# SinOncology/BreakID

Hardware: AMD Instinct MI355X
Metric: M reads/s clustered+split-scanned (higher is better)
Workload: dtype int32/u8 (+f64 sd replay)

## Files before the change

breakid_amd/csrc/api.hip:

```cpp
#include <algorithm>
#include <cmath>
#include <limits>
#include <cstring>
#include <numeric>

#include "bk_common.h"
#include "prims.h"
#include "stream.h"
#include "join.h"
#include "cluster.h"
#include "bp.h"
#include "normal.h"
#include "genotype.h"
#include "clip.h"
#include "junction.h"
#include "evidence.h"
#include "unique.h"
#include "consensus.h"
#include "jfit.h"
#include "locsim.h"
#include "coverage.h"
#include "frame.h"
#include "exclude.h"
#include "ahc.h"
#include "lanes.h"
#include "bgzf_gpu.h"

namespace
{
thread_local std::string g_init_error;

uint64_t fnv64(const std::string &s)
{
  uint64_t h = 0xCBF29CE484222325ull;
  for (unsigned char c : s)
  {
    h ^= c;
    h *= 0x100000001B3ull;
  }
  return h;
}
std::string chrom_id_to_name(int tid)
{
  if (tid == 23) return "chrY";
  if (tid == 22) return "chrX";
  if (tid >= 0 && tid < 22) return "chr" + std::to_string(tid + 1);
  return "";
}

struct StageTimer
{
  std::string name;
  hipEvent_t a = nullptr, b = nullptr;
  uint64_t bytes = 0;
  uint64_t touched = 0;
};
}

struct bk_ctx
{
  int device = 0;
  hipStream_t st = nullptr;
  bool own_stream = true;
  std::string err;
  int nt = 0;
  std::vector<uint32_t> tlen;
  std::vector<std::string> tname;
  std::vector<int32_t> hdr_id_host;
  DevBuf d_tprefix, d_nhash, d_nid, d_own, d_hdr;
  NameTableDev names{};

  bk_soa rec{};
  DevBuf col[13];
  DevBuf d_side;
  DevBuf xcol[13];
  bool have_records = false;
  bool streamed = false;

  DevBuf d_counters, d_sd, d_cand, d_split_raw, d_split, d_sa_list;
  StreamCounters hc{};
  SdState hsd{};
  bool stream_done = false, splits_sorted = false;
  int mapq_min = 20;
  int stream_mapq = -1;
  uint64_t cand_cap = 0, split_cap = 0, sa_cap = 0;
  uint64_t rec_base = 0;
  std::vector<uint64_t> route_counts;
  JoinBufs jb2;
  const Cand *ext_cand = nullptr;
  const bk_split *ext_split = nullptr;
  bk_cluster *ext_clusters = nullptr;
  std::vector<uint8_t> own_groups;
  const Cand *cand_ptr() const { return ext_cand ? ext_cand : d_cand.get<Cand>(); }
  const bk_split *split_raw_ptr() const { return ext_split ? ext_split : d_split_raw.get<bk_split>(); }
  bk_cluster *clusters_ptr() const { return ext_clusters ? ext_clusters : d_clusters.get<bk_cluster>(); }
  SdBufs sdb;
  double mean = 0, sd = 0;
  bool stats_done = false;

  JoinBufs jb;
  JoinResult jr;
  std::vector<uint32_t> gkey_host, glex_host, lex_to_num;
  std::vector<uint64_t> gstart_host;
  DevBuf d_glex, d_lex_to_num;

  ClusterStage stage;
  bool clustered = false;

  BpBufs bb;
  DevBuf d_clusters;
  uint64_t n_clusters = 0;

  bool joined = false, bp_done = false, shard = false;
  double join_w = 0;
  NormalBufs nb;
  std::vector<struct bk_normal_support> f_normal;
  RefBufs rb;
  std::vector<struct bk_ref_support> f_ref;
  ClipBufs cb;
  std::vector<struct bk_clip_support> f_clip;
  DevBuf d_bd_tid, d_bd_pos, d_bd_out, d_bd_samp;
  std::vector<uint32_t> f_base_depth;
  ClipReadBufs crb;
  std::vector<uint32_t> f_cr_counts;
  std::vector<struct bk_clip_read> f_cr_rows;
  std::vector<uint64_t> f_cr_off;
  JunctionBufs jnb;
  std::vector<struct bk_junction> f_junction;
  bool summary_map = false;
  EvidenceBufs evb;
  std::vector<struct bk_evidence> f_evidence;
  std::vector<uint64_t> f_ev_off;
  UniqueBufs uqb;
  std::vector<struct bk_unique_support> f_unique;
  std::vector<uint64_t> f_uq_first;
  ConsensusBufs cnb;
  std::vector<struct bk_consensus> f_cons;
  std::vector<uint8_t> f_cons_bases;
  std::vector<uint32_t> f_cons_depth;
  JfitBufs jfb;
  std::vector<struct bk_junction_fit> f_jfit;
  LocsimBufs lsb;
  std::vector<struct bk_locus_sim> f_locsim;
  CovBufs cvb;
  std::vector<struct bk_window_cov> f_wincov;
  FrameBufs frb;
  std::vector<struct bk_frame_call> f_frame;

  prims::RadixBufs dbg_radix;
  DevBuf dbg_in, dbg_out, dbg_vals;

  std::vector<bk_pair> f_pairs[3];
  std::vector<uint64_t> f_off[3];
  std::vector<bk_split> f_splits;
  std::vector<bk_cluster> f_clusters;
  std::vector<int32_t> f_gkeys;
  std::vector<bk_group_stat> f_gstats;

  bool timing = false;
  std::vector<StageTimer> timers;
  Timing tout;

  void tick(const char *name, uint64_t bytes, bool begin, uint64_t touched = 0)
  {
    if (!timing) return;
    if (begin)
    {
      StageTimer t;
      t.name = name;
      t.bytes = bytes;
      t.touched = touched;
      HIP_CHECK(hipEventCreate(&t.a));
      HIP_CHECK(hipEventCreate(&t.b));
      HIP_CHECK(hipEventRecord(t.a, st));
      timers.push_back(t);
    }
    else
      HIP_CHECK(hipEventRecord(timers.back().b, st));
  }
};

static RecView rec_view(const bk_ctx *ctx)
{
  RecView r;
  r.n = ctx->rec.n;
  r.tid = ctx->rec.tid; r.pos = ctx->rec.pos; r.flag = ctx->rec.flag; r.mapq = ctx->rec.mapq;
  r.cigar_off = ctx->rec.cigar_off; r.cigar = ctx->rec.cigar;
  r.isize = ctx->rec.isize; r.aux_off = ctx->rec.aux_off;
  return r;
}

namespace
{
struct Scope
{
  bk_ctx *c;
  Scope(bk_ctx *c, const char *name, uint64_t bytes = 0, uint64_t touched = 0) : c(c) { c->tick(name, bytes, true, touched); }
  ~Scope()
  {
    try
    {
      c->tick("", 0, false);
    }
    catch (...)
    {
    }
  }
};

template <class F> int guarded(bk_ctx *ctx, F &&f)
{
  if (!ctx) return BK_ERR_ARG;
  try
  {
    HIP_CHECK(hipSetDevice(ctx->device));
    f();
    return BK_OK;
  }
  catch (const bk_error &e)
  {
    ctx->err = e.msg;
    return e.code;
  }
  catch (const std::exception &e)
  {
    ctx->err = e.what();
    return BK_ERR_HIP;
  }
}

template <class T> void rows_to_host(bk_ctx *ctx, const T *d_rows, uint64_t n, std::vector<T> &out)
{
  out.resize(n);
  if (n) HIP_CHECK(hipMemcpyAsync(out.data(), d_rows, n * sizeof(T), hipMemcpyDeviceToHost, ctx->st));
  HIP_CHECK(hipStreamSynchronize(ctx->st));
}

void build_name_tables(bk_ctx *c)
{
  const int nt = c->nt;
  std::map<std::string, int> ids;
  for (int i = 0; i < nt; ++i)
    if (!ids.count(c->tname[i])) ids[c->tname[i]] = i;
  if (!ids.count("")) ids[""] = nt;
  if (!ids.count("*")) ids["*"] = nt + 1;
  for (int t = 0; t < 24; ++t)
  {
    std::string s = chrom_id_to_name(t);
    if (!ids.count(s)) ids[s] = nt + 2 + t;
  }
  uint32_t cap = 64;
  while (cap < ids.size() * 4) cap <<= 1;
  std::vector<uint64_t> hash(cap, 0);
  std::vector<int32_t> idv(cap, -1);
  for (auto &kv : ids)
  {
    uint64_t h = fnv64(kv.first);
    if (h == 0) h = 1;
    uint32_t slot = (uint32_t) h & (cap - 1);
    while (hash[slot] != 0 && hash[slot] != h) slot = (slot + 1) & (cap - 1);
    if (hash[slot] == 0)
    {
      hash[slot] = h;
      idv[slot] = kv.second;
    }
  }
  std::vector<int32_t> own(std::max(nt, 1));
  for (int t = 0; t < nt; ++t) own[t] = ids[chrom_id_to_name(t)];
  c->hdr_id_host.assign(nt + 1, 0);
  c->hdr_id_host[0] = ids["*"];
  for (int t = 0; t < nt; ++t) c->hdr_id_host[t + 1] = ids[c->tname[t]];
  std::vector<uint32_t> prefix(nt + 1, 0);
  for (int t = 0; t < nt; ++t) prefix[t + 1] = prefix[t] + c->tlen[t];
  HIP_CHECK(hipMemcpy(c->d_nhash.as<uint64_t>(cap), hash.data(), cap * 8, hipMemcpyHostToDevice));
  HIP_CHECK(hipMemcpy(c->d_nid.as<int32_t>(cap), idv.data(), cap * 4, hipMemcpyHostToDevice));
  HIP_CHECK(hipMemcpy(c->d_own.as<int32_t>(own.size()), own.data(), own.size() * 4, hipMemcpyHostToDevice));
  HIP_CHECK(hipMemcpy(c->d_hdr.as<int32_t>(nt + 1), c->hdr_id_host.data(), (nt + 1) * 4, hipMemcpyHostToDevice));
  HIP_CHECK(hipMemcpy(c->d_tprefix.as<uint32_t>(nt + 1), prefix.data(), (nt + 1) * 4, hipMemcpyHostToDevice));
  c->names.hash = c->d_nhash.get<uint64_t>();
  c->names.id = c->d_nid.get<int32_t>();
  c->names.mask = cap - 1;
  c->names.own_id = c->d_own.get<int32_t>();
  c->names.n_targets = nt;
  c->names.empty_id = ids[""];
}

std::string rname(const bk_ctx *c, int tid) { return tid < 0 ? "*" : c->tname[tid]; }

StreamArgs stream_args(bk_ctx *c, uint64_t n)
{
  StreamArgs a{};
  a.n = n;
  a.q_begin = 0;
  a.rec_base = c->rec_base;
  a.tid = c->rec.tid; a.pos = c->rec.pos; a.mtid = c->rec.mtid; a.mpos = c->rec.mpos; a.isize = c->rec.isize;
  a.flag = c->rec.flag; a.mapq = c->rec.mapq; a.qhash = c->rec.qhash; a.qcheck = c->rec.qcheck;
  static const bool no_side = getenv("BREAKID_NO_SIDE") != nullptr;
  a.side = no_side && c->rec.qhash ? nullptr : c->rec.side;
  a.cigar_off = c->rec.cigar_off; a.cigar = c->rec.cigar; a.aux_off = c->rec.aux_off; a.aux = c->rec.aux;
  a.mapq_min = c->mapq_min;
  a.names = c->names;
  a.counters = c->d_counters.get<StreamCounters>();
  a.sd = c->d_sd.get<SdState>();
  a.cand = c->d_cand.get<Cand>();
  a.cand_cap = c->cand_cap;
  a.split = c->d_split_raw.get<bk_split>();
  a.split_cap = c->split_cap;
  a.sa_list = c->d_sa_list.get<uint32_t>();
  a.sa_cap = c->sa_cap;
  return a;
}
void stream_prepare(bk_ctx *c, uint64_t n_expected)
{
  c->streamed = true;
  c->cand_cap = std::max<uint64_t>(c->cand_cap, std::max<uint64_t>(1u << 16, n_expected / 8 + 1024));
  c->split_cap = std::max<uint64_t>(c->split_cap, std::max<uint64_t>(1u << 14, n_expected / 32 + 1024));
  c->sa_cap = std::max<uint64_t>(c->sa_cap, std::max<uint64_t>(1u << 14, n_expected / 16 + 1024));
  StreamCounters *dc = c->d_counters.as<StreamCounters>(1);
  SdState *dsd = c->d_sd.as<SdState>(1);
  HIP_CHECK(hipMemsetAsync(dc, 0, sizeof(StreamCounters), c->st));
  HIP_CHECK(hipMemsetAsync(dsd, 0, sizeof(SdState), c->st));
  (void) c->d_cand.as<Cand>(c->cand_cap);
  (void) c->d_split_raw.as<bk_split>(c->split_cap);
  (void) c->d_sa_list.as<uint32_t>(c->sa_cap);
}
bool stream_finish(bk_ctx *c)
{
  HIP_CHECK(hipMemcpyAsync(&c->hc, c->d_counters.get<StreamCounters>(), sizeof(StreamCounters), hipMemcpyDeviceToHost, c->st));
  HIP_CHECK(hipMemcpyAsync(&c->hsd, c->d_sd.get<SdState>(), sizeof(SdState), hipMemcpyDeviceToHost, c->st));
  HIP_CHECK(hipStreamSynchronize(c->st));
  if (c->hc.n_cand > c->cand_cap || c->hc.n_sa > c->sa_cap)
  {
    c->cand_cap = std::max<uint64_t>(c->cand_cap, c->hc.n_cand + 1024);
    c->sa_cap = std::max<uint64_t>(c->sa_cap, c->hc.n_sa + 1024);
    return false;
  }
  return true;
}
void stream_rare_path(bk_ctx *c)
{
  const uint64_t n = c->rec.n;
  if (c->timing && !c->timers.empty())
  {
    c->timers.back().bytes += 32ull * c->hc.n_cand + 4ull * c->hc.n_sa;
    c->timers.back().touched = 23ull * n + 4ull * c->rec.n_cigar_words + (c->rec.qcheck ? 60ull : 56ull) * c->hc.n_cand + 4ull * c->hc.n_sa;
  }
  if (c->hc.unsorted) throw bk_error(BK_ERR_UNSORTED, "records are not coordinate sorted (the reference requires an indexed, sorted BAM)");
  if (c->hc.n_sa > c->split_cap)
  {
    c->split_cap = c->hc.n_sa + 1024;
    (void) c->d_split_raw.as<bk_split>(c->split_cap);
  }
  StreamArgs a = stream_args(c, n);
  {
    Scope s(c, "k_split_records", c->rec.n_aux_bytes + 4ull * c->hc.n_sa);
    launch_split_records(a, c->hc.n_sa, c->st);
  }
  HIP_CHECK(hipMemcpyAsync(&c->hc, c->d_counters.get<StreamCounters>(), sizeof(StreamCounters), hipMemcpyDeviceToHost, c->st));
  HIP_CHECK(hipStreamSynchronize(c->st));
  if (c->timing && !c->timers.empty())
  {
    c->timers.back().bytes += 48ull * c->hc.n_split;
    c->timers.back().touched = c->timers.back().bytes + 40ull * c->hc.n_sa + 32ull * c->hc.n_split;
  }
  c->stream_done = true;
  c->stream_mapq = c->mapq_min;
  c->splits_sorted = false;
  c->stats_done = false;
}

void run_stream(bk_ctx *c)
{
  if (!c->have_records) throw bk_error(BK_ERR_ARG, "no records uploaded");
  const uint64_t n = c->rec.n;
  for (int attempt = 0; attempt < 3; ++attempt)
  {
    stream_prepare(c, n);
    {
      Scope s(c, "k_stream", 39ull * n + 4ull * c->rec.n_cigar_words);
      launch_stream(stream_args(c, n), c->st);
    }
    if (stream_finish(c)) break;
    if (c->timing && !c->timers.empty()) c->timers.pop_back();
    if (attempt == 2) throw bk_error(BK_ERR_LIMIT, "stream pass: output capacity");
  }
  stream_rare_path(c);
}

void ensure_splits_sorted(bk_ctx *c)
{
  if (c->splits_sorted) return;
  Scope s(c, "split_sort");
  bk_split *sorted = c->d_split.as<bk_split>(c->hc.n_split + 1);
  int bits = 0;
  if (!c->ext_split && c->rec_base == 0)
  {
    bits = 1;
    while (bits < 32 && (1ull << bits) < c->rec.n) ++bits;
  }
  sort_splits(const_cast<bk_split *>(c->split_raw_ptr()), c->hc.n_split, sorted, c->bb, c->st, bits);
  c->splits_sorted = true;
}
}

extern "C" {

void bk_prepare_process()
{
  static std::once_flag once;
  std::call_once(once, [] {
    const char *q = getenv("GPU_MAX_HW_QUEUES");
    stage_set_hw_queues(q ? atoi(q) : 4);
  });
}

int bk_init(int device, const uint32_t *target_len, const char *const *target_name, int n_targets, bk_ctx **out)
{
  {
    bk_prepare_process();
  }
  if (!out || n_targets < 0 || (n_targets && (!target_len || !target_name)))
  {
    g_init_error = "bk_init: bad arguments";
    return BK_ERR_ARG;
  }
  *out = nullptr;
  int ndev = 0;
  if (hipGetDeviceCount(&ndev) != hipSuccess || ndev <= 0 || device < 0 || device >= ndev)
  {
    g_init_error = "bk_init: no HIP device " + std::to_string(device) + " (this library has no CPU path)";
    return BK_ERR_NO_DEVICE;
  }
  hipDeviceProp_t prop;
  if (hipGetDeviceProperties(&prop, device) != hipSuccess || std::string(prop.gcnArchName).rfind("gfx950", 0) != 0)
  {
    g_init_error = std::string("bk_init: device is not gfx950 (") + prop.gcnArchName + "); kernels are built for MI355X only";
    return BK_ERR_NO_DEVICE;
  }
  bk_ctx *c = new bk_ctx();
  c->device = device;
  c->nt = n_targets;
  for (int i = 0; i < n_targets; ++i)
  {
    c->tlen.push_back(target_len[i]);
    c->tname.push_back(target_name[i]);
  }
  int rc = guarded(c, [&] {
    HIP_CHECK(hipStreamCreate(&c->st));
    build_name_tables(c);
  });
  if (rc != BK_OK)
  {
    g_init_error = c->err;
    delete c;
    return rc;
  }
  *out = c;
  return BK_OK;
}

void bk_free(bk_ctx *ctx)
{
  if (!ctx) return;
  (void) hipSetDevice(ctx->device);
  (void) hipStreamSynchronize(ctx->st);
  for (auto &t : ctx->timers)
  {
    if (t.a) (void) hipEventDestroy(t.a);
    if (t.b) (void) hipEventDestroy(t.b);
  }
  if (ctx->own_stream && ctx->st) (void) hipStreamDestroy(ctx->st);
  delete ctx;
}

const char *bk_last_error(const bk_ctx *ctx) { return ctx ? ctx->err.c_str() : g_init_error.c_str(); }

int bk_set_stream(bk_ctx *ctx, void *hip_stream)
{
  return guarded(ctx, [&] {
    if (ctx->own_stream && ctx->st) HIP_CHECK(hipStreamDestroy(ctx->st));
    ctx->st = (hipStream_t) hip_stream;
    ctx->own_stream = false;
  });
}
int bk_get_stream(bk_ctx *ctx, void **hip_stream)
{
  return guarded(ctx, [&] {
    if (!hip_stream) throw bk_error(BK_ERR_ARG, "bk_get_stream: null output");
    *hip_stream = (void *) ctx->st;
  });
}
int bk_sync(bk_ctx *ctx)
{
  return guarded(ctx, [&] { HIP_CHECK(hipStreamSynchronize(ctx->st)); });
}

int bk_records(bk_ctx *ctx, bk_soa *cols)
{
  return guarded(ctx, [&] {
    if (!cols) throw bk_error(BK_ERR_ARG, "bk_records: null output");
    if (!ctx->have_records) throw bk_error(BK_ERR_ARG, "bk_records: the context holds no record table");
    HIP_CHECK(hipStreamSynchronize(ctx->st));
    *cols = ctx->rec;
  });
}

int bk_upload_records(bk_ctx *ctx, const bk_soa *s, int mem_space)
{
  return guarded(ctx, [&] {
    if (!s) throw bk_error(BK_ERR_ARG, "bk_upload_records: null table");
    if (s->n > 0xFFFFFFF0ull) throw bk_error(BK_ERR_LIMIT, "more than 2^32 records in one context (shard across GPUs)");
    ctx->stream_done = ctx->stats_done = ctx->clustered = false;
    ctx->joined = ctx->bp_done = ctx->shard = false;
    ctx->ext_cand = nullptr;
    ctx->ext_split = nullptr;
    ctx->ext_clusters = nullptr;
    ctx->own_groups.clear();
    ctx->rec_base = 0;
    ctx->streamed = false;
    if (mem_space == BK_MEM_DEVICE)
    {
      hipPointerAttribute_t at;
      if (s->n && s->tid && hipPointerGetAttributes(&at, s->tid) == hipSuccess && at.type == hipMemoryTypeDevice && at.device != ctx->device)
        throw bk_error(BK_ERR_ARG, "bk_upload_records: BK_MEM_DEVICE table lives on device " + std::to_string(at.device) + ", context on device " +
                                       std::to_string(ctx->device));
      (void) hipGetLastError();
      for (const void *p : {(const void *) s->tid, (const void *) s->pos, (const void *) s->isize, (const void *) s->flag, (const void *) s->mapq, (const void *) s->cigar_off,
                            (const void *) s->aux_off})
        if (s->n && ((uintptr_t) p & 15u)) throw bk_error(BK_ERR_ARG, "bk_upload_records: BK_MEM_DEVICE columns must be 16-byte aligned");
      if (s->n && s->side && ((uintptr_t) s->side & 15u)) throw bk_error(BK_ERR_ARG, "bk_upload_records: BK_MEM_DEVICE side rows must be 16-byte aligned");
      ctx->rec = *s;
    }
    else
    {
      const uint64_t n = s->n;
      const void *src[13] = {s->tid, s->pos, s->mtid, s->mpos, s->isize, s->flag, s->mapq, s->qhash, s->cigar_off, s->cigar, s->aux_off, s->aux, s->qcheck};
      const size_t bytes[13] = {n * 4, n * 4, n * 4, n * 4, n * 4, n * 2, n, n * 8, (n + 1) * 4, s->n_cigar_words * 4, (n + 1) * 4, s->n_aux_bytes,
                                s->qcheck ? n * 4 : 0};
      void *dst[13];
      for (int k = 0; k < 13; ++k)
      {
        dst[k] = ctx->col[k].ensure(bytes[k] + 16);
        if (bytes[k]) HIP_CHECK(hipMemcpyAsync(dst[k], src[k], bytes[k], hipMemcpyHostToDevice, ctx->st));
      }
      HIP_CHECK(hipStreamSynchronize(ctx->st));
      bk_soa d = *s;
      d.tid = (const int32_t *) dst[0]; d.pos = (const int32_t *) dst[1]; d.mtid = (const int32_t *) dst[2]; d.mpos = (const int32_t *) dst[3];
      d.isize = (const int32_t *) dst[4]; d.flag = (const uint16_t *) dst[5]; d.mapq = (const uint8_t *) dst[6]; d.qhash = (const uint64_t *) dst[7];
      d.cigar_off = (const uint32_t *) dst[8]; d.cigar = (const uint32_t *) dst[9]; d.aux_off = (const uint32_t *) dst[10]; d.aux = (const uint8_t *) dst[11];
      d.qcheck = s->qcheck ? (const uint32_t *) dst[12] : nullptr;
      bk_side *side = ctx->d_side.as<bk_side>(n + 1);
      launch_make_side(d.qhash, d.mtid, d.mpos, d.qcheck, n, side, ctx->st);
      d.side = side;
      ctx->rec = d;
    }
    ctx->have_records = true;
  });
}

int bk_exclude_regions(bk_ctx *ctx, const bk_regions *r, uint64_t *n_removed)
{
  return guarded(ctx, [&] {
    if (!ctx->have_records || ctx->streamed || ctx->shard)
      throw bk_error(BK_ERR_ARG, "bk_exclude_regions: call it after bk_upload_records and before the stream pass (bk_isize_stats, bk_shard_begin, "
                                 "or a context of bk_bam_decode_device_ctx)");
    if (!r || (r->n && (!r->tid || !r->beg || !r->end))) throw bk_error(BK_ERR_ARG, "bk_exclude_regions: null interval list");
    const bk_soa &s = ctx->rec;
    if (s.n && (!s.tid || !s.pos || !s.mtid || !s.mpos || !s.isize || !s.flag || !s.mapq || !s.qhash || !s.cigar_off || !s.aux_off))
      throw bk_error(BK_ERR_ARG, "bk_exclude_regions: the table lacks a column");
    std::vector<std::vector<std::pair<int32_t, int32_t>>> by(ctx->nt);
    for (uint64_t k = 0; k < r->n; ++k)
    {
      const int32_t t = r->tid[k], b = r->beg[k], e = r->end[k];
      if (t < 0 || t >= ctx->nt || b < 0 || e <= b)
        throw bk_error(BK_ERR_ARG, "bk_exclude_regions: interval " + std::to_string(k) + " (tid " + std::to_string(t) + ", [" + std::to_string(b) + ", " +
                                       std::to_string(e) + ")): needs 0 <= tid < n_targets, 0 <= beg < end");
      by[t].emplace_back(b, e);
    }
    std::vector<uint32_t> off(ctx->nt + 1, 0);
    std::vector<int32_t> beg, end;
    for (int t = 0; t < ctx->nt; ++t)
    {
      auto &v = by[t];
      std::sort(v.begin(), v.end());
      for (auto &iv : v)
        if (beg.size() > off[t] && iv.first <= end.back())
          end.back() = std::max(end.back(), iv.second);
        else
        {
          beg.push_back(iv.first);
          end.push_back(iv.second);
        }
      off[t + 1] = (uint32_t) beg.size();
    }
    const bool owned = s.tid && s.tid == ctx->col[0].get<int32_t>();
    if (beg.empty() && owned)
    {
      if (n_removed) *n_removed = 0;
      return;
    }
    DevBuf d_off, d_beg, d_end;
    ExclRegions rg;
    rg.n_targets = ctx->nt;
    rg.off = d_off.as<uint32_t>(off.size());
    rg.beg = d_beg.as<int32_t>(beg.size() + 1);
    rg.end = d_end.as<int32_t>(end.size() + 1);
    HIP_CHECK(hipMemcpyAsync((void *) rg.off, off.data(), off.size() * 4, hipMemcpyHostToDevice, ctx->st));
    if (!beg.empty())
    {
      HIP_CHECK(hipMemcpyAsync((void *) rg.beg, beg.data(), beg.size() * 4, hipMemcpyHostToDevice, ctx->st));
      HIP_CHECK(hipMemcpyAsync((void *) rg.end, end.data(), end.size() * 4, hipMemcpyHostToDevice, ctx->st));
    }
    bk_soa out;
    const uint64_t n_before = s.n;
    exclude_compact(s, rg, ctx->xcol, out, ctx->st, [&](const char *name, uint64_t bytes, bool begin) { ctx->tick(name ? name : "", bytes, begin, bytes); });
    for (int k = 0; k < 13; ++k)
    {
      std::swap(ctx->col[k], ctx->xcol[k]);
      ctx->xcol[k].release();
    }
    {
      Scope sc(ctx, "make_side", (out.qcheck ? 56ull : 52ull) * out.n, (out.qcheck ? 56ull : 52ull) * out.n);
      bk_side *side = ctx->d_side.as<bk_side>(out.n + 1);
      launch_make_side(out.qhash, out.mtid, out.mpos, out.qcheck, out.n, side, ctx->st);
      out.side = side;
    }
    HIP_CHECK(hipStreamSynchronize(ctx->st));
    ctx->rec = out;
    if (n_removed) *n_removed = n_before - out.n;
  });
}

int bk_isize_stats(bk_ctx *ctx, double *mean, double *sd)
{
  return guarded(ctx, [&] {
    if (!ctx->stream_done) run_stream(ctx);
    if (!ctx->stats_done)
    {
      const double n = (double) ctx->hc.isize_n;
      const double m = (double) (long long) ctx->hc.isize_sum / n;
      ctx->mean = m;
      if (ctx->hc.isize_n == 0)
        ctx->sd = std::nan("");
      else
      {
        double sum_d = ctx->hsd.sumsq - 2.0 * m * (double) ctx->hc.isize_sum + n * m * m;
        if (!(sum_d > 0)) sum_d = 0;
        double da = (double) ctx->hsd.vmax - m, dmax = da * da + m * m;
        double bound = 2.0 * sum_d + 2.0 * n + 2.0 * dmax + 4.0;
        int k = std::ilogb(bound) + 1;
        double thr = k >= 51 ? 1.0e300 : std::ldexp(1.0, k - 53);
        {
          Scope s(ctx, "isize_sd", 0, 6ull * ctx->rec.n);
          launch_sd(ctx->rec.flag, ctx->rec.isize, ctx->rec.n, m, thr, ctx->d_sd.get<SdState>(), ctx->sdb, ctx->st);
        }
        HIP_CHECK(hipMemcpyAsync(&ctx->hsd, ctx->d_sd.get<SdState>(), sizeof(SdState), hipMemcpyDeviceToHost, ctx->st));
        HIP_CHECK(hipStreamSynchronize(ctx->st));
        ctx->sd = std::sqrt((double) ctx->hsd.t_final / n);
      }
      ctx->stats_done = true;
    }
    if (mean) *mean = ctx->mean;
    if (sd) *sd = ctx->sd;
  });
}

static void finish_groups(bk_ctx *ctx, const std::vector<uint32_t> *all_keys)
{
  const uint32_t ng = ctx->jr.n_groups;
  ctx->gkey_host.assign(ng, 0);
  ctx->gstart_host.assign(ng + 1, 0);
  if (ng)
  {
    HIP_CHECK(hipMemcpyAsync(ctx->gkey_host.data(), ctx->jr.gkey, ng * 4, hipMemcpyDeviceToHost, ctx->st));
    HIP_CHECK(hipMemcpyAsync(ctx->gstart_host.data(), ctx->jr.gstart, (ng + 1) * 8, hipMemcpyDeviceToHost, ctx->st));
    HIP_CHECK(hipStreamSynchronize(ctx->st));
  }
  auto key_name = [&](uint32_t k) {
    int t1 = (int) (k / (uint32_t) (ctx->nt + 1)) - 1, t2 = (int) (k % (uint32_t) (ctx->nt + 1)) - 1;
    return rname(ctx, t1) + "_" + rname(ctx, t2);
  };
  std::vector<std::string> keys(ng);
  for (uint32_t g = 0; g < ng; ++g) keys[g] = key_name(ctx->gkey_host[g]);
  ctx->lex_to_num.resize(ng);
  std::iota(ctx->lex_to_num.begin(), ctx->lex_to_num.end(), 0u);
  std::sort(ctx->lex_to_num.begin(), ctx->lex_to_num.end(), [&](uint32_t a, uint32_t b) { return keys[a] < keys[b]; });
  ctx->glex_host.assign(ng, 0);
  if (!all_keys)
    for (uint32_t l = 0; l < ng; ++l) ctx->glex_host[ctx->lex_to_num[l]] = l;
  else
  {
    std::vector<std::string> names;
    names.reserve(all_keys->size());
    for (uint32_t k : *all_keys) names.push_back(key_name(k));
    std::sort(names.begin(), names.end());
    names.erase(std::unique(names.begin(), names.end()), names.end());
    for (uint32_t g = 0; g < ng; ++g)
    {
      auto it = std::lower_bound(names.begin(), names.end(), keys[g]);
      if (it == names.end() || *it != keys[g]) throw bk_error(BK_ERR_ARG, "bk_shard_group_pairs: a local group is missing from the global key list");
      ctx->glex_host[g] = (uint32_t) (it - names.begin());
    }
  }
  uint32_t *dg = ctx->d_glex.as<uint32_t>((uint64_t) ng + 1), *dl = ctx->d_lex_to_num.as<uint32_t>((uint64_t) ng + 1);
  if (ng) HIP_CHECK(hipMemcpyAsync(dg, ctx->glex_host.data(), ng * 4, hipMemcpyHostToDevice, ctx->st));
  if (ng) HIP_CHECK(hipMemcpyAsync(dl, ctx->lex_to_num.data(), ng * 4, hipMemcpyHostToDevice, ctx->st));
  join_assign_ids(ctx->jr, dg, ctx->st);
}

int bk_discordant_pairs(bk_ctx *ctx, int mapq_min, double w, uint64_t *n_pairs, uint32_t *n_groups)
{
  return guarded(ctx, [&] {
    if (!ctx->stream_done || mapq_min != ctx->stream_mapq)
    {
      ctx->mapq_min = mapq_min;
      run_stream(ctx);
    }
    {
      Scope s(ctx, "mate_join");
      ctx->jb.rec_bits = -1;
      if (!ctx->ext_cand && ctx->rec_base == 0)
      {
        int bits = 1;
        while (bits < 32 && (1ull << bits) < ctx->rec.n) ++bits;
        ctx->jb.rec_bits = bits;
      }
      join_candidates(ctx->cand_ptr(), ctx->hc.n_cand, w, ctx->d_tprefix.get<uint32_t>(), ctx->nt, ctx->jb, ctx->st, ctx->jr);
    }
    finish_groups(ctx, nullptr);
    ctx->clustered = false;
    ctx->joined = true;
    ctx->bp_done = false;
    ctx->join_w = w;
    if (n_pairs) *n_pairs = ctx->jr.n_pairs;
    if (n_groups) *n_groups = ctx->jr.n_groups;
  });
}

int bk_mask_and_cluster(bk_ctx *ctx, double w, int fast, uint64_t *n_clustered)
{
  return guarded(ctx, [&] {
    const StageInput in{ctx->device, ctx->st, ctx->jr, ctx->gstart_host, ctx->own_groups,
                        [&](const char *name, const std::function<void()> &body) { Scope s(ctx, name); body(); }};
    ctx->summary_map = false;
    ctx->stage.run(in, w, fast);
    ctx->clustered = true;
    if (n_clustered) *n_clustered = ctx->stage.list.n;
  });
}

int bk_split_evidence(bk_ctx *ctx, uint64_t *n_tuples)
{
  return guarded(ctx, [&] {
    if (!ctx->stream_done) run_stream(ctx);
    ensure_splits_sorted(ctx);
    if (n_tuples) *n_tuples = ctx->hc.n_split;
  });
}

int bk_cluster_summary(bk_ctx *ctx, double w, uint64_t *n_clusters)
{
  return guarded(ctx, [&] {
    if (!ctx->clustered) throw bk_error(BK_ERR_ARG, "bk_cluster_summary: call bk_mask_and_cluster first");
    ctx->bp_done = false;
    if (ctx->stage.list.ng != ctx->jr.n_groups) throw bk_error(BK_ERR_HIP, "bk_cluster_summary: the clustered list and the join disagree on the groups (internal error)");
    Scope s(ctx, "cluster_summary");
    ctx->n_clusters = cluster_summary(ctx->jr.pairs, ctx->stage.list.idx.get<uint32_t>(), ctx->stage.list.gof.get<uint32_t>(), ctx->stage.d_cluster.get<uint32_t>(), ctx->stage.list.n,
                                      ctx->stage.list.ng, ctx->jr.gkey, ctx->d_glex.get<uint32_t>(), ctx->d_lex_to_num.get<uint32_t>(), ctx->nt, w, ctx->d_clusters, ctx->bb, ctx->st);
    ctx->summary_map = true;
    if (n_clusters) *n_clusters = ctx->n_clusters;
  });
}

int bk_split_breakpoints(bk_ctx *ctx, double w, uint64_t *n_valid)
{
  return guarded(ctx, [&] {
    ensure_splits_sorted(ctx);
    RecView r;
    r.n = ctx->rec.n;
    r.tid = ctx->rec.tid; r.pos = ctx->rec.pos; r.flag = ctx->rec.flag; r.mapq = ctx->rec.mapq;
    r.cigar_off = ctx->rec.cigar_off; r.cigar = ctx->rec.cigar;
    {
      Scope s(ctx, "split_breakpoints");
      split_breakpoints(r, ctx->d_split.get<bk_split>(), ctx->hc.n_split, ctx->clusters_ptr(), ctx->n_clusters, w, (int) ctx->hc.max_span,
                        ctx->d_hdr.get<int32_t>(), ctx->bb, ctx->st);
    }
    ctx->bp_done = true;
    if (n_valid) *n_valid = count_valid_clusters(ctx->clusters_ptr(), ctx->n_clusters, ctx->bb, ctx->st);
  });
}

static TupleTable tuple_table(const bk_ctx *ctx)
{
  return TupleTable{ctx->d_split.get<bk_split>(), ctx->hc.n_split, (int) ctx->hc.max_span, ctx->d_hdr.get<int32_t>(), ctx->names.own_id, ctx->nt, ctx->names.empty_id};
}
static JunctionPairs junction_pairs(const bk_ctx *ctx)
{
  JunctionPairs jp{};
  if (ctx->n_clusters)
  {
    jp.pairs = ctx->jr.pairs;
    jp.idx = ctx->stage.list.idx.get<uint32_t>();
    jp.gof = ctx->stage.list.gof.get<uint32_t>();
    jp.cl = ctx->stage.d_cluster.get<uint32_t>();
    jp.n = ctx->stage.list.n;
    jp.ng = ctx->stage.list.ng;
    jp.slotbase = ctx->bb.slotbase.get<uint32_t>();
    jp.keep = ctx->bb.keep.get<uint32_t>();
    jp.off = ctx->bb.off.get<uint32_t>();
  }
  return jp;
}
static void require_same_reference(const std::string &who, const char *role_a, const bk_ctx *a, const char *role_b, const bk_ctx *b)
{
  if (b->device != a->device)
    throw bk_error(BK_ERR_ARG, who + ": " + role_a + " (device " + std::to_string(a->device) + ") and " + role_b + " (device " + std::to_string(b->device) +
                                   ") contexts are on different devices");
  if (b != a && (b->nt != a->nt || b->tname != a->tname || b->tlen != a->tlen))
    throw bk_error(BK_ERR_ARG, who + ": " + role_a + " and " + role_b + " reference lists differ (names or lengths)");
}

int bk_normal_support(bk_ctx *tumor, bk_ctx *normal, double w, const struct bk_normal_support **out, uint64_t *count)
{
  if (!normal) return guarded(tumor, [&] { throw bk_error(BK_ERR_ARG, "bk_normal_support: null normal context"); });
  return guarded(tumor, [&] {
    if (!out || !count) throw bk_error(BK_ERR_ARG, "bk_normal_support: null output");
    if (tumor->shard || normal->shard) throw bk_error(BK_ERR_ARG, "bk_normal_support: sharded contexts (bk_shard_*) are not supported");
    if (!tumor->bp_done) throw bk_error(BK_ERR_ARG, "bk_normal_support: call bk_split_breakpoints on the tumour context first");
    if (!normal->stats_done || !normal->joined || !normal->splits_sorted)
      throw bk_error(BK_ERR_ARG, "bk_normal_support: call bk_isize_stats, bk_discordant_pairs and bk_split_evidence on the normal context first");
    if (tumor->join_w != w) throw bk_error(BK_ERR_ARG, "bk_normal_support: w is not the tumour's distance (its bk_discordant_pairs w)");
    if (normal->stream_mapq != tumor->stream_mapq || normal->join_w != w)
      throw bk_error(BK_ERR_ARG, "bk_normal_support: the normal's bk_discordant_pairs must use the tumour's mapq_min and w");
    require_same_reference("bk_normal_support", "tumour", tumor, "normal", normal);
    Scope s(tumor, "normal_support");
    HIP_CHECK(hipStreamSynchronize(normal->st));
    const NormalSide ns{normal->jr.pairs, normal->jr.n_pairs, tuple_table(normal), rec_view(normal)};
    const uint64_t ncl = tumor->n_clusters;
    struct bk_normal_support *d_res;
    normal_support(ns, tumor->clusters_ptr(), ncl, w, tumor->nb, tumor->st, &d_res);
    rows_to_host(tumor, d_res, ncl, tumor->f_normal);
    *out = tumor->f_normal.data();
    *count = ncl;
  });
}

int bk_ref_support(bk_ctx *calls, bk_ctx *records, int mapq_min, int anchor, double w, const struct bk_ref_support **out, uint64_t *count)
{
  if (!records) return guarded(calls, [&] { throw bk_error(BK_ERR_ARG, "bk_ref_support: null records context"); });
  return guarded(calls, [&] {
    if (!out || !count) throw bk_error(BK_ERR_ARG, "bk_ref_support: null output");
    if (calls->shard || records->shard) throw bk_error(BK_ERR_ARG, "bk_ref_support: sharded contexts (bk_shard_*) are not supported");
    if (!calls->bp_done) throw bk_error(BK_ERR_ARG, "bk_ref_support: call bk_split_breakpoints on the calls context first");
    if (!records->have_records || !records->stats_done) throw bk_error(BK_ERR_ARG, "bk_ref_support: call bk_isize_stats on the records context first");
    if (anchor < 0) throw bk_error(BK_ERR_ARG, "bk_ref_support: anchor must not be negative");
    if (mapq_min < 0) throw bk_error(BK_ERR_ARG, "bk_ref_support: mapq_min must not be negative");
    if (!(w >= 0.0 && w < 2147483648.0)) throw bk_error(BK_ERR_ARG, "bk_ref_support: w is out of range");
    require_same_reference("bk_ref_support", "calls", calls, "records", records);
    const bk_soa &t = records->rec;
    if (t.n && (!t.tid || !t.pos || !t.isize || !t.flag || !t.mapq || !t.cigar_off || !t.aux_off))
      throw bk_error(BK_ERR_ARG, "bk_ref_support: the record table lacks a column");
    const uint64_t ncl = calls->n_clusters;
    if (records != calls) HIP_CHECK(hipStreamSynchronize(records->st));
    struct bk_ref_support *d_res;
    RefStat *d_stat = nullptr;
    {
      Scope s(calls, "ref_support");
      ref_support(rec_view(records), (int) records->hc.max_span, calls->clusters_ptr(), ncl, mapq_min, anchor, w, calls->rb, calls->st, &d_res,
                  calls->timing ? &d_stat : nullptr);
    }
    std::vector<RefStat> stat(d_stat ? 2 * ncl : 0);
    if (!stat.empty()) HIP_CHECK(hipMemcpyAsync(stat.data(), d_stat, 2 * ncl * sizeof(RefStat), hipMemcpyDeviceToHost, calls->st));
    rows_to_host(calls, d_res, ncl, calls->f_ref);
    if (calls->timing && !calls->timers.empty())
    {
      uint64_t visited = 0, words = 0;
      for (const RefStat &x : stat)
      {
        visited += x.visited;
        words += x.words;
      }
      calls->timers.back().bytes = 19ull * visited;
      calls->timers.back().touched = 19ull * visited + 4ull * words + ncl * (2ull * sizeof(bk_cluster) + sizeof(struct bk_ref_support));
    }
    *out = calls->f_ref.data();
    *count = ncl;
  });
}

int bk_clip_support(bk_ctx *calls, bk_ctx *records, int mapq_min, int min_clip, double w, const struct bk_clip_support **out, uint64_t *count)
{
  if (!records) return guarded(calls, [&] { throw bk_error(BK_ERR_ARG, "bk_clip_support: null records context"); });
  return guarded(calls, [&] {
    if (!out || !count) throw bk_error(BK_ERR_ARG, "bk_clip_support: null output");
    if (calls->shard || records->shard) throw bk_error(BK_ERR_ARG, "bk_clip_support: sharded contexts (bk_shard_*) are not supported");
    if (!calls->bp_done) throw bk_error(BK_ERR_ARG, "bk_clip_support: call bk_split_breakpoints on the calls context first");
    if (!records->have_records || !records->stats_done) throw bk_error(BK_ERR_ARG, "bk_clip_support: call bk_isize_stats on the records context first");
    if (min_clip < 1) throw bk_error(BK_ERR_ARG, "bk_clip_support: min_clip must be at least 1");
    if (mapq_min < 0) throw bk_error(BK_ERR_ARG, "bk_clip_support: mapq_min must not be negative");
    if (!(w >= 0.0 && w < 2147483648.0)) throw bk_error(BK_ERR_ARG, "bk_clip_support: w is out of range");
    require_same_reference("bk_clip_support", "calls", calls, "records", records);
    const bk_soa &t = records->rec;
    if (t.n && (!t.tid || !t.pos || !t.flag || !t.mapq || !t.cigar_off || !t.aux_off)) throw bk_error(BK_ERR_ARG, "bk_clip_support: the record table lacks a column");
    const uint64_t ncl = calls->n_clusters;
    if (records != calls) HIP_CHECK(hipStreamSynchronize(records->st));
    struct bk_clip_support *d_res;
    ClipStat *d_stat = nullptr;
    {
      Scope s(calls, "clip_support");
      clip_support(rec_view(records), (int) records->hc.max_span, calls->clusters_ptr(), ncl, mapq_min, min_clip, w, calls->cb, calls->st, &d_res,
                   calls->timing ? &d_stat : nullptr);
    }
    std::vector<ClipStat> stat(d_stat ? 2 * ncl : 0);
    if (!stat.empty()) HIP_CHECK(hipMemcpyAsync(stat.data(), d_stat, 2 * ncl * sizeof(ClipStat), hipMemcpyDeviceToHost, calls->st));
    rows_to_host(calls, d_res, ncl, calls->f_clip);
    if (calls->timing && !calls->timers.empty())
    {
      uint64_t visited = 0, words = 0;
      for (const ClipStat &x : stat)
      {
        visited += x.visited;
        words += x.words;
      }
      calls->timers.back().bytes = 15ull * visited;
      calls->timers.back().touched = 15ull * visited + 4ull * words + ncl * (2ull * sizeof(bk_cluster) + sizeof(struct bk_clip_support));
    }
    *out = calls->f_clip.data();
    *count = ncl;
  });
}

int bk_clip_reads(bk_ctx *records, const struct bk_clip_site *sites, uint64_t n_sites, int mapq_min, int min_clip, const uint32_t **counts,
                  const struct bk_clip_read **rows, const uint64_t **site_off)
{
  return guarded(records, [&] {
    if (!counts) throw bk_error(BK_ERR_ARG, "bk_clip_reads: null counts");
    if ((rows == nullptr) != (site_off == nullptr)) throw bk_error(BK_ERR_ARG, "bk_clip_reads: rows and site_off go together (both, or neither for the counts only)");
    if (n_sites && !sites) throw bk_error(BK_ERR_ARG, "bk_clip_reads: null sites");
    if (records->shard) throw bk_error(BK_ERR_ARG, "bk_clip_reads: sharded contexts (bk_shard_*) are not supported");
    if (!records->have_records || !records->stats_done) throw bk_error(BK_ERR_ARG, "bk_clip_reads: call bk_isize_stats first");
    if (min_clip < 1) throw bk_error(BK_ERR_ARG, "bk_clip_reads: min_clip must be at least 1");
    if (mapq_min < 0) throw bk_error(BK_ERR_ARG, "bk_clip_reads: mapq_min must not be negative");
    if (n_sites > 0x40000000ull) throw bk_error(BK_ERR_LIMIT, "bk_clip_reads: more than 2^30 sites");
    for (uint64_t k = 0; k < n_sites; ++k)
      if (sites[k].dir > 1u) throw bk_error(BK_ERR_ARG, "bk_clip_reads: site " + std::to_string(k) + " has a dir above 1 (0 = LEFT, 1 = RIGHT)");
    const bool listing = rows != nullptr;
    const bk_soa &t = records->rec;
    if (t.n && (!t.tid || !t.pos || !t.flag || !t.mapq || !t.cigar_off || !t.aux_off)) throw bk_error(BK_ERR_ARG, "bk_clip_reads: the record table lacks a column");
    if (listing && t.n && !t.side && !t.qhash) throw bk_error(BK_ERR_ARG, "bk_clip_reads: a listing needs the read-name hashes: the record table has neither qhash nor side");
    const ClipNames nm{listing ? t.side : nullptr, listing ? t.qhash : nullptr, listing ? t.qcheck : nullptr};
    ClipReadsOut o{};
    {
      Scope s(records, "clip_reads");
      clip_reads(rec_view(records), nm, (int) records->hc.max_span, sites, n_sites, mapq_min, min_clip, listing, records->timing, records->crb, records->st, o);
    }
    if (o.bad) throw bk_error(BK_ERR_HIP, "bk_clip_reads: the listing and the counts disagree (internal error)");
    std::vector<ClipStat> stat(o.stat ? n_sites : 0);
    if (!stat.empty()) HIP_CHECK(hipMemcpyAsync(stat.data(), o.stat, n_sites * sizeof(ClipStat), hipMemcpyDeviceToHost, records->st));
    records->f_cr_off.assign(listing ? n_sites + 1 : 0, 0);
    if (listing) HIP_CHECK(hipMemcpyAsync(records->f_cr_off.data(), o.site_off, (n_sites + 1) * 8, hipMemcpyDeviceToHost, records->st));
    records->f_cr_rows.resize(o.n_rows);
    if (o.n_rows) HIP_CHECK(hipMemcpyAsync(records->f_cr_rows.data(), o.rows, o.n_rows * sizeof(struct bk_clip_read), hipMemcpyDeviceToHost, records->st));
    rows_to_host(records, o.counts, n_sites, records->f_cr_counts);
    if (records->timing && !records->timers.empty())
    {
      uint64_t visited = 0, words = 0;
      for (const ClipStat &x : stat)
      {
        visited += x.visited;
        words += x.words;
      }
      const uint64_t passes = listing && o.n_rows ? 2 : 1;
      records->timers.back().bytes = passes * 15ull * visited;
      records->timers.back().touched = passes * (15ull * visited + 4ull * words + n_sites * sizeof(struct bk_clip_site)) + n_sites * 12ull +
                                       (listing ? n_sites * 16ull + o.n_rows * (32ull + sizeof(struct bk_clip_read)) : 0ull);
    }
    *counts = records->f_cr_counts.data();
    if (listing)
    {
      *rows = records->f_cr_rows.data();
      *site_off = records->f_cr_off.data();
    }
  });
}

int bk_base_depth(bk_ctx *records, const int32_t *tid, const uint32_t *pos, uint64_t n, const uint32_t **out)
{
  return guarded(records, [&] {
    if (!out || (n && (!tid || !pos))) throw bk_error(BK_ERR_ARG, "bk_base_depth: null argument");
    if (records->shard) throw bk_error(BK_ERR_ARG, "bk_base_depth: sharded contexts (bk_shard_*) are not supported");
    if (!records->have_records || !records->stats_done) throw bk_error(BK_ERR_ARG, "bk_base_depth: call bk_isize_stats first");
    const bk_soa &t = records->rec;
    if (t.n && (!t.tid || !t.pos || !t.flag || !t.mapq || !t.cigar_off)) throw bk_error(BK_ERR_ARG, "bk_base_depth: the record table lacks a column");
    records->f_base_depth.assign(n, 0u);
    if (n)
    {
      int32_t *d_tid = records->d_bd_tid.as<int32_t>(n);
      uint32_t *d_pos = records->d_bd_pos.as<uint32_t>(n), *d_out = records->d_bd_out.as<uint32_t>(n);
      HIP_CHECK(hipMemcpyAsync(d_tid, tid, n * 4, hipMemcpyHostToDevice, records->st));
      HIP_CHECK(hipMemcpyAsync(d_pos, pos, n * 4, hipMemcpyHostToDevice, records->st));
      {
        Scope s(records, "base_depth");
        base_depth_at(rec_view(records), d_tid, d_pos, n, (int) records->hc.max_span, records->d_bd_samp, records->st, d_out);
      }
      HIP_CHECK(hipMemcpyAsync(records->f_base_depth.data(), d_out, n * 4, hipMemcpyDeviceToHost, records->st));
      HIP_CHECK(hipStreamSynchronize(records->st));
    }
    *out = records->f_base_depth.data();
  });
}

int bk_genotype_call(uint32_t alt, uint32_t ref, uint8_t *gt, uint8_t *gq, float *vaf)
{
  if (!gt || !gq || !vaf) return BK_ERR_ARG;
  if ((uint64_t) alt + ref == 0)
  {
    *gt = 255;
    *gq = 0;
    *vaf = std::numeric_limits<float>::quiet_NaN();
    return BK_OK;
  }
  static const double c[3] = {-0x1.4d104d427de80p+0, -0x1.34413509f79ffp-2, -0x1.6cf9f8b075bd8p-6};
  const double k = (double) alt, r = (double) ref;
  double L[3];
  for (int g = 0; g < 3; ++g)
  {
    const double a = k * c[g], b = r * c[2 - g];
    L[g] = a + b;
  }
  int best = 0;
  for (int g = 1; g < 3; ++g)
    if (L[g] > L[best]) best = g;
  int second = -1;
  for (int g = 0; g < 3; ++g)
    if (g != best && (second < 0 || L[g] > L[second])) second = g;
  const double q = std::floor(10.0 * (L[best] - L[second]) + 0.5);
  *gt = (uint8_t) best;
  *gq = (uint8_t) (q < 99.0 ? q : 99.0);
  *vaf = (float) alt / (float) ((uint64_t) alt + ref);
  return BK_OK;
}

int bk_junctions(bk_ctx *ctx, const struct bk_junction **out, uint64_t *count)
{
  return guarded(ctx, [&] {
    if (!out || !count) throw bk_error(BK_ERR_ARG, "bk_junctions: null output");
    if (ctx->shard) throw bk_error(BK_ERR_ARG, "bk_junctions: sharded contexts (bk_shard_*) are not supported");
    if (!ctx->bp_done || !ctx->clustered || !ctx->summary_map) throw bk_error(BK_ERR_ARG, "bk_junctions: call bk_split_breakpoints first");
    const uint64_t ncl = ctx->n_clusters;
    const JunctionPairs jp = junction_pairs(ctx);
    struct bk_junction *d_res;
    uint32_t *d_vis;
    {
      Scope s(ctx, "junctions", jp.n * (12ull + 4ull));
      junctions(jp, tuple_table(ctx), ctx->clusters_ptr(), ncl, ctx->jnb, ctx->st, &d_res, &d_vis);
    }
    std::vector<uint32_t> vis(ctx->timing ? ncl : 0);
    if (!vis.empty()) HIP_CHECK(hipMemcpyAsync(vis.data(), d_vis, ncl * 4, hipMemcpyDeviceToHost, ctx->st));
    rows_to_host(ctx, d_res, ncl, ctx->f_junction);
    if (ctx->timing && !ctx->timers.empty())
    {
      uint64_t visited = 0;
      for (uint32_t v : vis) visited += v;
      ctx->timers.back().touched = jp.n * (12ull + 32ull) + visited * sizeof(bk_split) + ncl * (sizeof(bk_cluster) + 2ull * sizeof(struct bk_junction) + 4ull);
    }
    *out = ctx->f_junction.data();
    *count = ncl;
  });
}

int bk_evidence(bk_ctx *ctx, const struct bk_evidence **out, uint64_t *count, const uint64_t **call_off)
{
  return guarded(ctx, [&] {
    if (!out || !count || !call_off) throw bk_error(BK_ERR_ARG, "bk_evidence: null output");
    if (ctx->shard) throw bk_error(BK_ERR_ARG, "bk_evidence: sharded contexts (bk_shard_*) are not supported");
    if (!ctx->bp_done || !ctx->clustered || !ctx->summary_map) throw bk_error(BK_ERR_ARG, "bk_evidence: call bk_split_breakpoints first");
    const uint64_t ncl = ctx->n_clusters;
    const bk_soa &t = ctx->rec;
    if (ncl && (!ctx->have_records || !t.mapq || (!t.side && !t.qhash))) throw bk_error(BK_ERR_ARG, "bk_evidence: the record table lacks a column");
    const JunctionPairs jp = junction_pairs(ctx);
    EvidenceRecs er{t.n, t.side, t.qhash, t.qcheck, t.mapq};
    struct bk_evidence *d_rows;
    uint64_t *d_off;
    EvidenceStat *d_stat;
    {
      Scope s(ctx, "evidence", jp.n * (12ull + 4ull + 2ull * 12ull));
      evidence(jp, tuple_table(ctx), ctx->clusters_ptr(), ncl, er, ctx->evb, ctx->st, &d_rows, &d_off, &d_stat);
    }
    ctx->f_ev_off.assign(ncl + 1, 0);
    EvidenceStat stat{};
    HIP_CHECK(hipMemcpyAsync(ctx->f_ev_off.data(), d_off, (ncl + 1) * 8, hipMemcpyDeviceToHost, ctx->st));
    HIP_CHECK(hipMemcpyAsync(&stat, d_stat, sizeof stat, hipMemcpyDeviceToHost, ctx->st));
    HIP_CHECK(hipStreamSynchronize(ctx->st));
    if (stat.bad) throw bk_error(BK_ERR_HIP, "bk_evidence: the listing and the counts of bk_junctions disagree (internal error)");
    const uint64_t n = ctx->f_ev_off[ncl];
    rows_to_host(ctx, d_rows, n, ctx->f_evidence);
    if (ctx->timing && !ctx->timers.empty())
    {
      uint64_t n_pair_rows = 0;
      for (uint64_t i = 0; i < n; ++i) n_pair_rows += ctx->f_evidence[i].kind == BK_EV_PAIR;
      int bits = 1;
      while ((ncl >> bits) != 0) ++bits;
      const uint64_t passes = (uint64_t) (bits + 7) / 8;
      ctx->timers.back().touched = jp.n * (12ull + 32ull) + 2ull * stat.visited * sizeof(bk_split) + ncl * (2ull * sizeof(bk_cluster) + 2ull * sizeof(struct bk_junction) + 20ull) +
                                   jp.n * (12ull + 12ull + passes * 32ull + 12ull) + n_pair_rows * (64ull + 32ull) + (n - n_pair_rows) * 32ull +
                                   n * sizeof(struct bk_evidence);
    }
    *out = ctx->f_evidence.data();
    *count = n;
    *call_off = ctx->f_ev_off.data();
  });
}

int bk_unique_support(bk_ctx *ctx, const struct bk_unique_support **out, uint64_t *count, const uint64_t **first, uint64_t *n_rows)
{
  return guarded(ctx, [&] {
    if (!out || !count) throw bk_error(BK_ERR_ARG, "bk_unique_support: null output");
    if (!first != !n_rows) throw bk_error(BK_ERR_ARG, "bk_unique_support: first and n_rows go together (both, or both null for the counts alone)");
    if (ctx->shard) throw bk_error(BK_ERR_ARG, "bk_unique_support: sharded contexts (bk_shard_*) are not supported");
    if (!ctx->bp_done || !ctx->clustered || !ctx->summary_map) throw bk_error(BK_ERR_ARG, "bk_unique_support: call bk_split_breakpoints first");
    const uint64_t ncl = ctx->n_clusters;
    const bk_soa &t = ctx->rec;
    if (ncl && (!ctx->have_records || !t.mapq || (!t.side && (!t.qhash || !t.mtid || !t.mpos))))
      throw bk_error(BK_ERR_ARG, "bk_unique_support: the record table lacks a column (mtid and mpos, or bk_side rows)");
    const JunctionPairs jp = junction_pairs(ctx);
    EvidenceRecs er{t.n, t.side, t.qhash, t.qcheck, t.mapq, t.mtid, t.mpos};
    const bool listing = first != nullptr;
    struct bk_unique_support *d_res;
    uint64_t *d_first;
    EvidenceStat *d_stat;
    UniqueStat us;
    {
      Scope s(ctx, "unique", jp.n * (12ull + 4ull + 2ull * 12ull));
      unique_support(jp, tuple_table(ctx), ctx->clusters_ptr(), ncl, er, listing, ctx->uqb, ctx->st, &d_res, &d_first, &d_stat, &us);
    }
    EvidenceStat stat{};
    HIP_CHECK(hipMemcpyAsync(&stat, d_stat, sizeof stat, hipMemcpyDeviceToHost, ctx->st));
    if (listing)
    {
      ctx->f_uq_first.resize(us.n_rows);
      if (us.n_rows) HIP_CHECK(hipMemcpyAsync(ctx->f_uq_first.data(), d_first, us.n_rows * 8, hipMemcpyDeviceToHost, ctx->st));
    }
    rows_to_host(ctx, d_res, ncl, ctx->f_unique);
    if (stat.bad) throw bk_error(BK_ERR_HIP, "bk_unique_support: the listing and the counts of bk_junctions disagree (internal error)");
    if (ctx->timing && !ctx->timers.empty())
    {
      int bits = 1;
      while ((ncl >> bits) != 0) ++bits;
      const uint64_t ev_passes = (uint64_t) (bits + 7) / 8, n = us.n_rows;
      ctx->timers.back().bytes += n * 64ull;
      ctx->timers.back().touched = jp.n * (12ull + 32ull) + 2ull * stat.visited * sizeof(bk_split) + ncl * (2ull * sizeof(bk_cluster) + 2ull * sizeof(struct bk_junction) + 20ull) +
                                   jp.n * (12ull + 12ull + ev_passes * 32ull + 12ull) + n * (64ull + 32ull) +
                                   n * (64ull + us.gathers * 20ull + us.passes * 36ull + 68ull + (listing ? 8ull : 0ull)) + ncl * (32ull + sizeof(struct bk_unique_support));
    }
    *out = ctx->f_unique.data();
    *count = ncl;
    if (listing)
    {
      *first = ctx->f_uq_first.data();
      *n_rows = us.n_rows;
    }
  });
}

int bk_clip_consensus(bk_ctx *ctx, const bk_reads *reads, const struct bk_clip_site *sites, uint64_t n_sites, int mapq_min, int min_clip, uint32_t max_len,
                      uint32_t min_depth, const struct bk_consensus **out, const uint8_t **bases, const uint32_t **col_depth)
{
  return guarded(ctx, [&] {
    if (!reads || !out || !bases) throw bk_error(BK_ERR_ARG, "bk_clip_consensus: null reads, out or bases");
    if (n_sites && !sites) throw bk_error(BK_ERR_ARG, "bk_clip_consensus: null sites");
    if (ctx->shard) throw bk_error(BK_ERR_ARG, "bk_clip_consensus: sharded contexts (bk_shard_*) are not supported");
    if (max_len < 1 || max_len > 256) throw bk_error(BK_ERR_ARG, "bk_clip_consensus: max_len must be 1..256");
    if (min_depth == 0) throw bk_error(BK_ERR_ARG, "bk_clip_consensus: min_depth must be at least 1");
    if (min_clip < 1) throw bk_error(BK_ERR_ARG, "bk_clip_consensus: min_clip must be at least 1");
    if (mapq_min < 0) throw bk_error(BK_ERR_ARG, "bk_clip_consensus: mapq_min must not be negative");
    if (reads->n > 0x100000000ull) throw bk_error(BK_ERR_LIMIT, "bk_clip_consensus: more than 2^32 reads");
    if (n_sites > 0x40000000ull) throw bk_error(BK_ERR_LIMIT, "bk_clip_consensus: more than 2^30 sites");
    for (uint64_t k = 0; k < n_sites; ++k)
    {
      if (sites[k].dir > 1u) throw bk_error(BK_ERR_ARG, "bk_clip_consensus: site " + std::to_string(k) + " has a dir above 1 (0 = LEFT, 1 = RIGHT)");
      if (sites[k].tol != 0u) throw bk_error(BK_ERR_ARG, "bk_clip_consensus: site " + std::to_string(k) + " has a tol other than 0");
    }
    const bk_reads &t = *reads;
    if (t.n && (!t.tid || !t.pos || !t.flag || !t.mapq || !t.cigar_off || !t.l_seq || !t.seq_off)) throw bk_error(BK_ERR_ARG, "bk_clip_consensus: the reads table lacks a column");
    for (uint64_t i = 0; i < t.n; ++i)
    {
      if (t.cigar_off[i + 1] < t.cigar_off[i]) throw bk_error(BK_ERR_ARG, "bk_clip_consensus: cigar_off does not ascend at read " + std::to_string(i));
      if (t.seq_off[i + 1] < t.seq_off[i]) throw bk_error(BK_ERR_ARG, "bk_clip_consensus: seq_off does not ascend at read " + std::to_string(i));
      if (t.seq_off[i + 1] - t.seq_off[i] < ((uint64_t) t.l_seq[i] + 1) / 2)
        throw bk_error(BK_ERR_ARG, "bk_clip_consensus: read " + std::to_string(i) + " has fewer seq bytes than (l_seq + 1) / 2");
    }
    if (t.n && ((t.cigar_off[t.n] && !t.cigar) || (t.seq_off[t.n] && !t.seq))) throw bk_error(BK_ERR_ARG, "bk_clip_consensus: the reads table lacks a column");
    struct bk_consensus *d_res;
    uint8_t *d_bases;
    uint32_t *d_depth;
    ConsensusStat *d_stat;
    consensus_upload(t, ctx->cnb, ctx->st);
    {
      const uint64_t words = t.n ? t.cigar_off[t.n] : 0, sbytes = t.n ? t.seq_off[t.n] : 0;
      Scope s(ctx, "consensus", t.n * 27ull + 12ull + words * 4ull + sbytes + n_sites * (16ull + sizeof(struct bk_consensus) + 5ull * max_len));
      clip_consensus(sites, n_sites, mapq_min, min_clip, max_len, min_depth, ctx->cnb, ctx->st, &d_res, &d_bases, &d_depth, &d_stat);
    }
    ConsensusStat stat{};
    HIP_CHECK(hipMemcpyAsync(&stat, d_stat, sizeof stat, hipMemcpyDeviceToHost, ctx->st));
    const uint64_t cols = n_sites * max_len;
    ctx->f_cons_bases.resize(cols);
    if (cols) HIP_CHECK(hipMemcpyAsync(ctx->f_cons_bases.data(), d_bases, cols, hipMemcpyDeviceToHost, ctx->st));
    if (col_depth)
    {
      ctx->f_cons_depth.resize(cols);
      if (cols) HIP_CHECK(hipMemcpyAsync(ctx->f_cons_depth.data(), d_depth, cols * 4, hipMemcpyDeviceToHost, ctx->st));
    }
    rows_to_host(ctx, d_res, n_sites, ctx->f_cons);
    if (ctx->timing && !ctx->timers.empty())
    {
      ctx->timers.back().touched = 2ull * t.n * 19ull + stat.words * 4ull + stat.contributions * 24ull + stat.seq_bytes +
                                   n_sites * (4ull + 8ull + 16ull + sizeof(struct bk_consensus) + 5ull * max_len);
    }
    *out = ctx->f_cons.data();
    *bases = ctx->f_cons_bases.data();
    if (col_depth) *col_depth = ctx->f_cons_depth.data();
  });
}

static void check_refseq(const bk_refseq &t, const std::string &who)
{
  if (t.n_segs > 0x100000ull) throw bk_error(BK_ERR_LIMIT, who +": more than 2^20 segments");
  if (t.n_segs && (!t.tid || !t.start || !t.len || !t.off)) throw bk_error(BK_ERR_ARG, who + ": the reference table lacks a column");
  for (uint64_t g = 0; g < t.n_segs; ++g)
  {
    if (t.off[g + 1] < t.off[g]) throw bk_error(BK_ERR_ARG, who + ": off does not ascend at segment " + std::to_string(g));
    if (t.off[g + 1] - t.off[g] < ((uint64_t) t.len[g] + 1) / 2)
      throw bk_error(BK_ERR_ARG, who + ": segment " + std::to_string(g) + " has fewer bytes than (len + 1) / 2");
    if (g + 1 < t.n_segs)
    {
      if (t.tid[g + 1] < t.tid[g] || (t.tid[g + 1] == t.tid[g] && t.start[g + 1] < t.start[g]))
        throw bk_error(BK_ERR_ARG, who + ": segment " + std::to_string(g + 1) + " is out of order (the segments ascend by tid, then start)");
      if (t.tid[g + 1] == t.tid[g] && (long long) t.start[g] + (long long) t.len[g] > (long long) t.start[g + 1])
        throw bk_error(BK_ERR_ARG, who + ": segment " + std::to_string(g + 1) + " overlaps the one before it");
    }
  }
  if (t.n_segs && t.off[t.n_segs] && !t.bases) throw bk_error(BK_ERR_ARG, who + ": the reference table lacks a column");
}

int bk_junction_fit(bk_ctx *ctx, const bk_refseq *ref, const struct bk_junction_probe *probes, uint64_t n, const uint8_t *query, uint32_t max_len, uint32_t max_shift,
                    uint32_t max_ins, uint32_t max_hom, const struct bk_junction_fit **out)
{
  return guarded(ctx, [&] {
    if (!ref || !out) throw bk_error(BK_ERR_ARG, "bk_junction_fit: null ref or out");
    if (n && (!probes || !query)) throw bk_error(BK_ERR_ARG, "bk_junction_fit: null probes or query");
    if (ctx->shard) throw bk_error(BK_ERR_ARG, "bk_junction_fit: sharded contexts (bk_shard_*) are not supported");
    if (max_len < 1 || max_len > 256) throw bk_error(BK_ERR_ARG, "bk_junction_fit: max_len must be 1..256");
    if (max_shift > 64) throw bk_error(BK_ERR_ARG, "bk_junction_fit: max_shift must be 0..64");
    if (max_ins > 64) throw bk_error(BK_ERR_ARG, "bk_junction_fit: max_ins must be 0..64");
    if (max_hom > 64) throw bk_error(BK_ERR_ARG, "bk_junction_fit: max_hom must be 0..64");
    if (n > 0x40000000ull) throw bk_error(BK_ERR_LIMIT, "bk_junction_fit: more than 2^30 probes");
    const bk_refseq &t = *ref;
    check_refseq(t, "bk_junction_fit");
    uint64_t qbytes = 0, walk_bases = 0;
    for (uint64_t k = 0; k < n; ++k)
    {
      const struct bk_junction_probe &p = probes[k];
      if (p.dir_own > 1u || p.dir_mate > 1u) throw bk_error(BK_ERR_ARG, "bk_junction_fit: probe " + std::to_string(k) + " has a dir above 1 (0 = LEFT, 1 = RIGHT)");
      if (p.qlen > max_len) throw bk_error(BK_ERR_ARG, "bk_junction_fit: probe " + std::to_string(k) + " has a qlen above max_len");
      const uint8_t *q = query + k * max_len;
      for (uint32_t j = 0; j < p.qlen; ++j)
        if (q[j] != 'A' && q[j] != 'C' && q[j] != 'G' && q[j] != 'T' && q[j] != 'N')
          throw bk_error(BK_ERR_ARG, "bk_junction_fit: probe " + std::to_string(k) + " has a query byte outside ACGTN in column " + std::to_string(j));
      if (p.qlen >= 1 && p.tid_own >= 0 && p.tid_mate >= 0)
      {
        qbytes += p.qlen;
        walk_bases += 2ull * p.qlen + 2ull * max_shift + 2ull * max_hom;
      }
    }
    struct bk_junction_fit *d_res;
    jfit_upload(t, probes, n, query, max_len, ctx->jfb, ctx->st);
    {
      Scope s(ctx, "junction_fit", n * (sizeof(struct bk_junction_probe) + sizeof(struct bk_junction_fit) + (uint64_t) max_len) + t.n_segs * 24ull +
                                       (t.n_segs ? t.off[t.n_segs] : 0));
      junction_fit(n, max_len, max_shift, max_ins, max_hom, ctx->jfb, ctx->st, &d_res);
    }
    rows_to_host(ctx, d_res, n, ctx->f_jfit);
    if (ctx->timing && !ctx->timers.empty()) ctx->timers.back().touched = n * (sizeof(struct bk_junction_probe) + sizeof(struct bk_junction_fit)) + qbytes + (walk_bases + 1) / 2;
    *out = ctx->f_jfit.data();
  });
}

int bk_locus_similarity(bk_ctx *ctx, const bk_refseq *ref, const struct bk_locus_pair *pairs, uint64_t n, uint32_t flank, const struct bk_locus_sim **out)
{
  return guarded(ctx, [&] {
    if (!ref || !out) throw bk_error(BK_ERR_ARG, "bk_locus_similarity: null ref or out");
    if (n && !pairs) throw bk_error(BK_ERR_ARG, "bk_locus_similarity: null pairs");
    if (ctx->shard) throw bk_error(BK_ERR_ARG, "bk_locus_similarity: sharded contexts (bk_shard_*) are not supported");
    if (flank < 1 || flank > 255) throw bk_error(BK_ERR_ARG, "bk_locus_similarity: flank must be 1..255");
    if (n > 0x40000000ull) throw bk_error(BK_ERR_LIMIT, "bk_locus_similarity: more than 2^30 pairs");
    const bk_refseq &t = *ref;
    check_refseq(t, "bk_locus_similarity");
    const uint64_t L = 2ull * flank + 1;
    struct bk_locus_sim *d_res;
    locsim_upload(t, pairs, n, ctx->lsb, ctx->st);
    {
      Scope s(ctx, "locus_similarity", n * (sizeof(struct bk_locus_pair) + sizeof(struct bk_locus_sim)) + t.n_segs * 24ull + (t.n_segs ? t.off[t.n_segs] : 0));
      locus_similarity(n, flank, ctx->lsb, ctx->st, &d_res);
    }
    rows_to_host(ctx, d_res, n, ctx->f_locsim);
    if (ctx->timing && !ctx->timers.empty()) ctx->timers.back().touched = n * (sizeof(struct bk_locus_pair) + sizeof(struct bk_locus_sim) + L);
    *out = ctx->f_locsim.data();
  });
}

int bk_window_coverage(bk_ctx *records, const struct bk_cov_window *windows, uint64_t n, int mapq_min, const struct bk_window_cov **out)
{
  return guarded(records, [&] {
    if (!out || (n && !windows)) throw bk_error(BK_ERR_ARG, "bk_window_coverage: null argument");
    if (records->shard) throw bk_error(BK_ERR_ARG, "bk_window_coverage: sharded contexts (bk_shard_*) are not supported");
    if (!records->have_records || !records->stats_done) throw bk_error(BK_ERR_ARG, "bk_window_coverage: call bk_isize_stats first");
    if (mapq_min < 0) throw bk_error(BK_ERR_ARG, "bk_window_coverage: mapq_min must be >= 0");
    if (n > 0x40000000ull) throw bk_error(BK_ERR_LIMIT, "bk_window_coverage: more than 2^30 windows");
    for (uint64_t k = 0; k < n; ++k)
      if (windows[k].reserved) throw bk_error(BK_ERR_ARG, "bk_window_coverage: window " + std::to_string(k) + " has a non-zero reserved field");
    const bk_soa &t = records->rec;
    if (t.n && (!t.tid || !t.pos || !t.flag || !t.mapq || !t.cigar_off)) throw bk_error(BK_ERR_ARG, "bk_window_coverage: the record table lacks a column");
    if (t.n_cigar_words && !t.cigar) throw bk_error(BK_ERR_ARG, "bk_window_coverage: the record table lacks a column");
    CovBufs &b = records->cvb;
    struct bk_window_cov *d_res = nullptr;
    if (n) HIP_CHECK(hipMemcpyAsync(b.win.as<struct bk_cov_window>(n), windows, n * sizeof(struct bk_cov_window), hipMemcpyHostToDevice, records->st));
    {
      const uint64_t bytes = t.n * 11ull + t.n_cigar_words * 4ull + cov_tiles(t.n) * 16ull + n * 32ull;
      struct Whole
      {
        bk_ctx *c;
        size_t at;
        ~Whole()
        {
          if (c->timing && at < c->timers.size()) (void) hipEventRecord(c->timers[at].b, c->st);
        }
      } whole{records, records->timers.size()};
      records->tick("window_coverage", bytes, true, bytes);
      {
        Scope s(records, "window_coverage_tiles", 0, t.n * 11ull + t.n_cigar_words * 4ull + cov_tiles(t.n) * 16ull);
        cov_tiles_build(rec_view(records), mapq_min, b, records->st);
      }
      {
        Scope s(records, "window_coverage_windows", 0, n * 32ull);
        window_coverage(rec_view(records), records->nt, (int) records->hc.max_span, n, mapq_min, b, records->st, &d_res);
      }
    }
    rows_to_host(records, d_res, n, records->f_wincov);
    *out = records->f_wincov.data();
  });
}

static void check_txmodel(const bk_txmodel &t)
{
  const std::string who = "bk_fusion_frame: ";
  if (t.n_tx > 0x1000000ull) throw bk_error(BK_ERR_LIMIT, who + "more than 2^24 transcripts");
  if (t.n_parts > 0x10000000ull) throw bk_error(BK_ERR_LIMIT, who + "more than 2^28 coding parts");
  if (!t.n_tx) return;
  if (!t.tid || !t.tx_start || !t.tx_end || !t.strand || !t.ex_off || (t.n_parts && (!t.ex_start || !t.ex_end))) throw bk_error(BK_ERR_ARG, who + "the model lacks a column");
  if (t.ex_off[0] != 0 || t.ex_off[t.n_tx] != t.n_parts) throw bk_error(BK_ERR_ARG, who + "ex_off does not run from 0 to n_parts");
  for (uint64_t i = 0; i < t.n_tx; ++i)
  {
    const std::string at = "transcript " + std::to_string(i);
    if (t.tid[i] < 0) throw bk_error(BK_ERR_ARG, who + at + " has a negative tid");
    if (t.strand[i] > 1) throw bk_error(BK_ERR_ARG, who + at + " has a strand above 1 (0 = '+', 1 = '-')");
    if (t.tx_end[i] < t.tx_start[i]) throw bk_error(BK_ERR_ARG, who + at + " ends in front of its start");
    if (i + 1 < t.n_tx && (t.tid[i + 1] < t.tid[i] || (t.tid[i + 1] == t.tid[i] && t.tx_start[i + 1] < t.tx_start[i])))
      throw bk_error(BK_ERR_ARG, who + "transcript " + std::to_string(i + 1) + " is out of order (the rows ascend by tid, then tx_start)");
    if (t.ex_off[i + 1] < t.ex_off[i] || t.ex_off[i + 1] > t.n_parts) throw bk_error(BK_ERR_ARG, who + "ex_off does not ascend at " + at);
    for (uint64_t g = t.ex_off[i]; g < t.ex_off[i + 1]; ++g)
    {
      if (t.ex_end[g] <= t.ex_start[g]) throw bk_error(BK_ERR_ARG, who + at + " has an empty or descending coding part");
      if (g > t.ex_off[i] && t.ex_start[g] < t.ex_end[g - 1]) throw bk_error(BK_ERR_ARG, who + at + " has coding parts that descend or overlap");
      if (t.ex_start[g] < t.tx_start[i] || t.ex_end[g] > t.tx_end[i]) throw bk_error(BK_ERR_ARG, who + at + " has a coding part outside [tx_start, tx_end)");
    }
  }
}

int bk_fusion_frame(bk_ctx *ctx, const bk_txmodel *model, const struct bk_frame_site *sites, uint64_t n, const struct bk_frame_call **out)
{
  return guarded(ctx, [&] {
    if (!model || !out) throw bk_error(BK_ERR_ARG, "bk_fusion_frame: null model or out");
    if (n && !sites) throw bk_error(BK_ERR_ARG, "bk_fusion_frame: null sites");
    if (ctx->shard) throw bk_error(BK_ERR_ARG, "bk_fusion_frame: sharded contexts (bk_shard_*) are not supported");
    if (n > 0x40000000ull) throw bk_error(BK_ERR_LIMIT, "bk_fusion_frame: more than 2^30 sites");
    const bk_txmodel &t = *model;
    check_txmodel(t);
    for (uint64_t k = 0; k < n; ++k)
      if (sites[k].right1 > 1u || sites[k].right2 > 1u) throw bk_error(BK_ERR_ARG, "bk_fusion_frame: site " + std::to_string(k) + " has a right above 1 (0 = LEFT, 1 = RIGHT)");
    struct bk_frame_call *d_res;
    frame_upload(t, sites, n, ctx->frb, ctx->st);
    {
      const uint64_t bytes = t.n_tx * 21ull + (t.n_tx ? t.n_parts : 0) * 16ull + n * (sizeof(struct bk_frame_site) + sizeof(struct bk_frame_call));
      Scope s(ctx, "fusion_frame", bytes, bytes);
      frame_derive(t, ctx->frb, ctx->st);
      fusion_frame(n, ctx->frb, ctx->st, &d_res);
    }
    rows_to_host(ctx, d_res, n, ctx->f_frame);
    *out = ctx->f_frame.data();
  });
}

int bk_junction_sides(const struct bk_junction *j, uint8_t *right1, uint8_t *right2, uint8_t *source)
{
  if (!j || !right1 || !right2 || !source) return BK_ERR_ARG;
  auto largest = [](const uint32_t *v) {
    int best = 0;
    for (int i = 1; i < 4; ++i)
      if (v[i] > v[best]) best = i;
    return v[best] ? best : -1;
  };
  int idx = largest(j->splits);
  *source = 2;
  if (idx < 0)
  {
    idx = largest(j->pairs);
    *source = 1;
  }
  if (idx < 0)
  {
    idx = 1;
    *source = 0;
  }
  *right1 = (uint8_t) (idx >> 1);
  *right2 = (uint8_t) (idx & 1);
  return BK_OK;
}

int bk_call_windows(const bk_cluster *c, int right1, int right2, uint32_t flank, const uint32_t *target_len, struct bk_cov_window out[5])
{
  if (!c || !target_len || !out || flank == 0) return BK_ERR_ARG;
  const int32_t tid[2] = {c->p1_tid, c->p2_tid};
  const long long cut[2] = {(long long) c->p1_exact - (right1 ? 1 : 0), (long long) c->p2_exact - (right2 ? 1 : 0)};
  auto window = [&](int32_t t, long long a, long long b) {
    struct bk_cov_window w = {t, 0u, 0u, 0u};
    if (t < 0) return w;
    const long long len = (long long) target_len[t];
    a = a < 0 ? 0 : a;
    b = b > len ? len : b;
    if (b > a)
    {
      w.beg = (uint32_t) a;
      w.end = (uint32_t) b;
    }
    return w;
  };
  for (int s = 0; s < 2; ++s)
  {
    out[2 * s] = window(tid[s], cut[s] - (long long) flank, cut[s]);
    out[2 * s + 1] = window(tid[s], cut[s], cut[s] + (long long) flank);
  }
  out[4] = tid[0] == tid[1] && tid[0] >= 0 ? window(tid[0], std::min(cut[0], cut[1]), std::max(cut[0], cut[1])) : window(-1, 0, 0);
  return BK_OK;
}

int bk_clip_rescue(const bk_cluster *c, const struct bk_junction *j, const struct bk_clip_support *s, uint32_t min_support, uint32_t *pos1, uint32_t *pos2, uint32_t *n1,
                   uint32_t *n2)
{
  if (!c || !j || !s || !pos1 || !pos2 || !n1 || !n2 || min_support == 0) return BK_ERR_ARG;
  if ((c->flags & 2u) || c->p1_tid < 0 || c->p2_tid < 0) return 0;
  uint8_t d1 = 0, d2 = 1, source = 0;
  bk_junction_sides(j, &d1, &d2, &source);
  if (s->peak_n[0][d1] < min_support || s->peak_n[1][d2] < min_support) return 0;
  *pos1 = s->peak_pos[0][d1];
  *pos2 = s->peak_pos[1][d2];
  *n1 = s->peak_n[0][d1];
  *n2 = s->peak_n[1][d2];
  return 1;
}

int bk_vcf_breakend_alt(char ref_base, int own_right, const char *mate_chr, uint32_t mate_pos, int mate_right, char *buf, size_t cap)
{
  if (!mate_chr || !buf) return BK_ERR_ARG;
  const char br = mate_right ? '[' : ']';
  const std::string mate = br + std::string(mate_chr) + ":" + std::to_string(mate_pos) + br;
  const std::string alt = own_right ? mate + ref_base : ref_base + mate;
  if (alt.size() + 1 > cap) return BK_ERR_ARG;
  std::memcpy(buf, alt.c_str(), alt.size() + 1);
  return BK_OK;
}

int bk_run(bk_ctx *ctx, int mapq_min, int fast, double *w_out, uint64_t *n_valid)
{
  if (!ctx) return BK_ERR_ARG;
  if (ctx->stream_done && mapq_min != ctx->stream_mapq) ctx->stream_done = false;
  ctx->mapq_min = mapq_min;
  double mean, sd;
  int rc = bk_isize_stats(ctx, &mean, &sd);
  if (rc) return rc;
  const int times = 2;
  const double w = times * std::sqrt(times) * (mean + 3 * sd);
  if (w_out) *w_out = w;
  if ((rc = bk_discordant_pairs(ctx, mapq_min, w, nullptr, nullptr))) return rc;
  if ((rc = bk_mask_and_cluster(ctx, w, fast, nullptr))) return rc;
  if ((rc = bk_split_evidence(ctx, nullptr))) return rc;
  if ((rc = bk_cluster_summary(ctx, w, nullptr))) return rc;
  if ((rc = bk_split_breakpoints(ctx, w, n_valid))) return rc;
  return BK_OK;
}

int bk_fetch(bk_ctx *ctx, int stage, const void **data, uint64_t *count, const uint64_t **group_off, uint32_t *n_groups)
{
  return guarded(ctx, [&] {
    if (!data || !count) throw bk_error(BK_ERR_ARG, "bk_fetch: null output");
    const uint32_t ng = ctx->jr.n_groups;
    if (group_off) *group_off = nullptr;
    if (n_groups) *n_groups = 0;
    auto fetch_list = [&](int slot, const uint32_t *d_idx, const uint64_t *d_goff, const uint32_t *d_cl, uint64_t n) {
      std::vector<bk_pair> all(ctx->jr.n_pairs);
      if (!all.empty()) HIP_CHECK(hipMemcpyAsync(all.data(), ctx->jr.pairs, all.size() * sizeof(bk_pair), hipMemcpyDeviceToHost, ctx->st));
      std::vector<uint32_t> idx(n), cl(d_cl ? n : 0);
      std::vector<uint64_t> goff(ng + 1, 0);
      if (n && d_idx) HIP_CHECK(hipMemcpyAsync(idx.data(), d_idx, n * 4, hipMemcpyDeviceToHost, ctx->st));
      if (n && d_cl) HIP_CHECK(hipMemcpyAsync(cl.data(), d_cl, n * 4, hipMemcpyDeviceToHost, ctx->st));
      if (ng && d_goff) HIP_CHECK(hipMemcpyAsync(goff.data(), d_goff, (ng + 1) * 8, hipMemcpyDeviceToHost, ctx->st));
      HIP_CHECK(hipStreamSynchronize(ctx->st));
      auto &out = ctx->f_pairs[slot];
      auto &off = ctx->f_off[slot];
      out.clear();
      off.assign(1, 0);
      for (uint32_t l = 0; l < ng; ++l)
      {
        uint32_t g = ctx->lex_to_num[l];
        for (uint64_t p = goff[g]; p < goff[g + 1]; ++p)
        {
          bk_pair pr = all[d_idx ? idx[p] : p];
          if (d_cl) pr.cluster = (int32_t) cl[p];
          out.push_back(pr);
        }
        off.push_back(out.size());
      }
      *data = out.data();
      *count = out.size();
      if (group_off) *group_off = off.data();
      if (n_groups) *n_groups = ng;
    };
    switch (stage)
    {
    case BK_STAGE_SCAN:
      fetch_list(0, nullptr, ctx->jr.gstart, nullptr, ctx->jr.n_pairs);
      break;
    case BK_STAGE_ISO:
      fetch_list(1, ctx->stage.iso_idx.get<uint32_t>(), ctx->stage.iso_goff.get<uint64_t>(), nullptr, ctx->stage.iso_n);
      break;
    case BK_STAGE_CLUSTERED:
      if (!ctx->clustered) throw bk_error(BK_ERR_ARG, "bk_fetch: not clustered yet");
      fetch_list(2, ctx->stage.list.idx.get<uint32_t>(), ctx->stage.list.goff.get<uint64_t>(), ctx->stage.d_cluster.get<uint32_t>(), ctx->stage.list.n);
      break;
    case BK_STAGE_SPLITS:
      ensure_splits_sorted(ctx);
      ctx->f_splits.resize(ctx->hc.n_split);
      if (ctx->hc.n_split)
        HIP_CHECK(hipMemcpyAsync(ctx->f_splits.data(), ctx->d_split.get<bk_split>(), ctx->hc.n_split * sizeof(bk_split), hipMemcpyDeviceToHost, ctx->st));
      HIP_CHECK(hipStreamSynchronize(ctx->st));
      *data = ctx->f_splits.data();
      *count = ctx->f_splits.size();
      break;
    case BK_STAGE_CLUSTERS:
      rows_to_host(ctx, ctx->clusters_ptr(), ctx->n_clusters, ctx->f_clusters);
      {
        auto by_group = [](const bk_cluster &a, const bk_cluster &b) { return a.group < b.group; };
        if (ctx->ext_clusters)
          std::stable_sort(ctx->f_clusters.begin(), ctx->f_clusters.end(), by_group);
        else if (!std::is_sorted(ctx->f_clusters.begin(), ctx->f_clusters.end(), by_group))
          throw bk_error(BK_ERR_HIP, "bk_fetch: the cluster table is not in group order (internal error)");
      }
      *data = ctx->f_clusters.data();
      *count = ctx->f_clusters.size();
      break;
    case BK_STAGE_GROUP_KEYS:
      ctx->f_gkeys.clear();
      for (uint32_t l = 0; l < ng; ++l)
      {
        uint32_t k = ctx->gkey_host[ctx->lex_to_num[l]];
        ctx->f_gkeys.push_back((int32_t) (k / (uint32_t) (ctx->nt + 1)) - 1);
        ctx->f_gkeys.push_back((int32_t) (k % (uint32_t) (ctx->nt + 1)) - 1);
      }
      *data = ctx->f_gkeys.data();
      *count = ng;
      break;
    default:
      throw bk_error(BK_ERR_ARG, "bk_fetch: unknown stage");
    }
  });
}

int bk_shard_begin(bk_ctx *ctx, uint64_t rec_base, int mapq_min)
{
  return guarded(ctx, [&] {
    ctx->rec_base = rec_base;
    ctx->shard = true;
    ctx->streamed = true;
    ctx->mapq_min = mapq_min;
    ctx->ext_cand = nullptr;
    ctx->ext_split = nullptr;
    ctx->ext_clusters = nullptr;
    run_stream(ctx);
  });
}

int bk_shard_get_stats(bk_ctx *ctx, bk_shard_stats *out)
{
  return guarded(ctx, [&] {
    if (!ctx->stream_done || !out) throw bk_error(BK_ERR_ARG, "bk_shard_get_stats: call bk_shard_begin first");
    out->isize_sum = ctx->hc.isize_sum;
    out->isize_n = ctx->hc.isize_n;
    out->sumsq = ctx->hsd.sumsq;
    out->vmax = ctx->hsd.vmax;
    out->max_span = ctx->hc.max_span;
    out->n_cand = ctx->hc.n_cand;
    out->n_split = ctx->hc.n_split;
  });
}

int bk_shard_set_stats(bk_ctx *ctx, const bk_shard_stats *total)
{
  return guarded(ctx, [&] {
    if (!ctx->stream_done || !total) throw bk_error(BK_ERR_ARG, "bk_shard_set_stats: call bk_shard_begin first");
    ctx->hc.isize_sum = total->isize_sum;
    ctx->hc.isize_n = total->isize_n;
    ctx->hsd.sumsq = total->sumsq;
    ctx->hsd.vmax = total->vmax;
    ctx->hc.max_span = total->max_span;
    ctx->stats_done = false;
  });
}

static void sd_mean_thr(bk_ctx *ctx, double &m, double &thr)
{
  const double n = (double) ctx->hc.isize_n;
  m = (double) (long long) ctx->hc.isize_sum / n;
  if (ctx->hc.isize_n == 0)
  {
    thr = 0;
    return;
  }
  double sum_d = ctx->hsd.sumsq - 2.0 * m * (double) ctx->hc.isize_sum + n * m * m;
  if (!(sum_d > 0)) sum_d = 0;
  double da = (double) ctx->hsd.vmax - m, dmax = da * da + m * m;
  double bound = 2.0 * sum_d + 2.0 * n + 2.0 * dmax + 4.0;
  int k = std::ilogb(bound) + 1;
  thr = k >= 51 ? 1.0e300 : std::ldexp(1.0, k - 53);
}

int bk_shard_sd_local(bk_ctx *ctx, uint64_t *l_total, void **ex_dev, uint64_t *n_ex)
{
  return guarded(ctx, [&] {
    if (!ctx->stream_done) throw bk_error(BK_ERR_ARG, "bk_shard_sd_local: call bk_shard_begin / bk_shard_set_stats first");
    double m, thr;
    sd_mean_thr(ctx, m, thr);
    unsigned long long lt = 0, ne = 0;
    launch_sd_local(ctx->rec.flag, ctx->rec.isize, ctx->rec.n, m, thr, ctx->sdb, ctx->st, &lt, &ne);
    HIP_CHECK(hipStreamSynchronize(ctx->st));
    if (l_total) *l_total = lt;
    if (n_ex) *n_ex = ne;
    if (ex_dev) *ex_dev = ctx->sdb.exceptions.p;
  });
}

int bk_shard_sd_finish(bk_ctx *ctx, const void *all_ex_dev, uint64_t n_all, uint64_t l_grand, double *mean, double *sd)
{
  return guarded(ctx, [&] {
    double m, thr;
    sd_mean_thr(ctx, m, thr);
    launch_sd_walk((const SdException *) all_ex_dev, n_all, l_grand, ctx->d_sd.get<SdState>(), ctx->st);
    HIP_CHECK(hipMemcpyAsync(&ctx->hsd.t_final, &ctx->d_sd.get<SdState>()->t_final, 8, hipMemcpyDeviceToHost, ctx->st));
    HIP_CHECK(hipStreamSynchronize(ctx->st));
    ctx->mean = m;
    ctx->sd = std::sqrt((double) ctx->hsd.t_final / (double) ctx->hc.isize_n);
    ctx->stats_done = true;
    if (mean) *mean = ctx->mean;
    if (sd) *sd = ctx->sd;
  });
}

int bk_shard_buffer(bk_ctx *ctx, int which, void **dev, uint64_t *count, uint32_t *elem_bytes)
{
  return guarded(ctx, [&] {
    if (!dev || !count || !elem_bytes) throw bk_error(BK_ERR_ARG, "bk_shard_buffer: null output");
    switch (which)
    {
    case BK_BUF_CANDIDATES: *dev = ctx->d_cand.p; *count = ctx->ext_cand ? 0 : ctx->hc.n_cand; *elem_bytes = sizeof(Cand); break;
    case BK_BUF_TUPLES: *dev = ctx->d_split_raw.p; *count = ctx->ext_split ? 0 : ctx->hc.n_split; *elem_bytes = sizeof(bk_split); break;
    case BK_BUF_CLUSTERS: *dev = ctx->d_clusters.p; *count = ctx->ext_clusters ? 0 : ctx->n_clusters; *elem_bytes = sizeof(bk_cluster); break;
    default: throw bk_error(BK_ERR_ARG, "bk_shard_buffer: unknown buffer");
    }
  });
}

int bk_shard_set_buffer(bk_ctx *ctx, int which, const void *dev, uint64_t count)
{
  return guarded(ctx, [&] {
    switch (which)
    {
    case BK_BUF_CANDIDATES: ctx->ext_cand = (const Cand *) dev; ctx->hc.n_cand = count; break;
    case BK_BUF_TUPLES: ctx->ext_split = (const bk_split *) dev; ctx->hc.n_split = count; ctx->splits_sorted = false; break;
    case BK_BUF_CLUSTERS: ctx->ext_clusters = (bk_cluster *) dev; ctx->n_clusters = count; break;
    default: throw bk_error(BK_ERR_ARG, "bk_shard_set_buffer: unknown buffer");
    }
  });
}

int bk_shard_group_sizes(bk_ctx *ctx, const uint64_t **starts, uint32_t *n_groups)
{
  return guarded(ctx, [&] {
    if (starts) *starts = ctx->gstart_host.data();
    if (n_groups) *n_groups = ctx->jr.n_groups;
  });
}

int bk_shard_own_groups(bk_ctx *ctx, const uint8_t *own, uint32_t n_groups)
{
  return guarded(ctx, [&] {
    if (n_groups != ctx->jr.n_groups) throw bk_error(BK_ERR_ARG, "bk_shard_own_groups: wrong group count");
    ctx->own_groups.assign(own, own + n_groups);
  });
}

int bk_shard_route_candidates(bk_ctx *ctx, uint32_t world, void **dev, const uint64_t **counts)
{
  return guarded(ctx, [&] {
    if (!ctx->stream_done || ctx->ext_cand) throw bk_error(BK_ERR_ARG, "bk_shard_route_candidates: needs this shard's own candidates (after bk_shard_begin)");
    if (!world || world > 4096 || !dev || !counts) throw bk_error(BK_ERR_ARG, "bk_shard_route_candidates: bad arguments");
    *dev = route_candidates(ctx->d_cand.get<Cand>(), ctx->hc.n_cand, world, ctx->jb, ctx->st, ctx->route_counts);
    *counts = ctx->route_counts.data();
  });
}

int bk_shard_group_keys(bk_ctx *ctx, const uint32_t **keys, uint32_t *n_groups)
{
  return guarded(ctx, [&] {
    if (keys) *keys = ctx->gkey_host.data();
    if (n_groups) *n_groups = ctx->jr.n_groups;
  });
}

int bk_shard_route_pairs(bk_ctx *ctx, const uint32_t *dest_of_group, uint32_t n_groups, uint32_t world, void **dev, const uint64_t **counts)
{
  return guarded(ctx, [&] {
    if (n_groups != ctx->jr.n_groups || !world || !dev || !counts || (n_groups && !dest_of_group)) throw bk_error(BK_ERR_ARG, "bk_shard_route_pairs: bad arguments");
    ctx->route_counts.assign(world, 0);
    for (uint32_t g = 0; g < n_groups; ++g)
    {
      if (dest_of_group[g] >= world) throw bk_error(BK_ERR_ARG, "bk_shard_route_pairs: destination out of range");
      ctx->route_counts[dest_of_group[g]] += ctx->gstart_host[g + 1] - ctx->gstart_host[g];
    }
    std::vector<uint64_t> base(world, 0), off(n_groups, 0);
    for (uint32_t d = 1; d < world; ++d) base[d] = base[d - 1] + ctx->route_counts[d - 1];
    for (uint32_t g = 0; g < n_groups; ++g)
    {
      off[g] = base[dest_of_group[g]];
      base[dest_of_group[g]] += ctx->gstart_host[g + 1] - ctx->gstart_host[g];
    }
    *dev = route_pairs(ctx->jr, off, ctx->jb, ctx->st);
    *counts = ctx->route_counts.data();
  });
}

int bk_shard_group_pairs(bk_ctx *ctx, const void *pairs_dev, uint64_t n, const uint32_t *all_keys, uint32_t n_all_keys)
{
  return guarded(ctx, [&] {
    if ((n && !pairs_dev) || (n_all_keys && !all_keys)) throw bk_error(BK_ERR_ARG, "bk_shard_group_pairs: null input");
    {
      Scope s(ctx, "group_pairs");
      ctx->jb2.rec_bits = -1;
      group_pairs((const bk_pair *) pairs_dev, n, ctx->nt, ctx->jb2, ctx->st, ctx->jr);
    }
    std::vector<uint32_t> keys(all_keys, all_keys + n_all_keys);
    finish_groups(ctx, &keys);
    ctx->own_groups.clear();
    ctx->clustered = false;
  });
}

int bk_shard_bp_cov(bk_ctx *ctx, double w, void **cov_dev, uint64_t *n)
{
  return guarded(ctx, [&] {
    uint32_t *cov = bp_cov_partial(rec_view(ctx), ctx->clusters_ptr(), ctx->n_clusters, w, (int) ctx->hc.max_span, ctx->bb, ctx->st);
    HIP_CHECK(hipStreamSynchronize(ctx->st));
    if (cov_dev) *cov_dev = cov;
    if (n) *n = 2 * ctx->n_clusters;
  });
}

int bk_shard_bp_vote(bk_ctx *ctx, double w, const void *cov_total_dev)
{
  return guarded(ctx, [&] {
    ensure_splits_sorted(ctx);
    bp_vote(ctx->d_split.get<bk_split>(), ctx->hc.n_split, ctx->clusters_ptr(), ctx->n_clusters, w, (int) ctx->hc.max_span, (const uint32_t *) cov_total_dev,
            ctx->d_hdr.get<int32_t>(), ctx->bb, ctx->st);
    HIP_CHECK(hipStreamSynchronize(ctx->st));
  });
}

int bk_shard_bp_vote_slice(bk_ctx *ctx, double w, const void *cov_total_dev, uint64_t lo, uint64_t hi, void **clusters_dev, void **voted_dev)
{
  return guarded(ctx, [&] {
    if (lo > hi || hi > ctx->n_clusters || !clusters_dev || !voted_dev) throw bk_error(BK_ERR_ARG, "bk_shard_bp_vote_slice: bad range");
    ensure_splits_sorted(ctx);
    bp_vote(ctx->d_split.get<bk_split>(), ctx->hc.n_split, ctx->clusters_ptr() + lo, hi - lo, w, (int) ctx->hc.max_span,
            cov_total_dev ? (const uint32_t *) cov_total_dev + 2 * lo : nullptr, ctx->d_hdr.get<int32_t>(), ctx->bb, ctx->st);
    HIP_CHECK(hipStreamSynchronize(ctx->st));
    *clusters_dev = ctx->clusters_ptr() + lo;
    *voted_dev = ctx->bb.voted.p;
  });
}

int bk_shard_bp_set_voted(bk_ctx *ctx, const void *voted_all_dev)
{
  return guarded(ctx, [&] {
    uint32_t *v = ctx->bb.voted.as<uint32_t>(ctx->n_clusters + 1);
    if (ctx->n_clusters && voted_all_dev != v)
      HIP_CHECK(hipMemcpyAsync(v, voted_all_dev, ctx->n_clusters * 4, hipMemcpyDeviceToDevice, ctx->st));
    HIP_CHECK(hipStreamSynchronize(ctx->st));
  });
}

int bk_shard_bp_depth(bk_ctx *ctx, void **depth_dev, uint64_t *n)
{
  return guarded(ctx, [&] {
    uint32_t *d = bp_depth_partial(rec_view(ctx), ctx->clusters_ptr(), ctx->n_clusters, (int) ctx->hc.max_span, ctx->bb, ctx->st);
    HIP_CHECK(hipStreamSynchronize(ctx->st));
    if (depth_dev) *depth_dev = d;
    if (n) *n = 2 * ctx->n_clusters;
  });
}

int bk_shard_bp_finish(bk_ctx *ctx, const void *depth_total_dev)
{
  return guarded(ctx, [&] {
    bp_finish(ctx->clusters_ptr(), ctx->n_clusters, (const uint32_t *) depth_total_dev, ctx->bb, ctx->st);
    HIP_CHECK(hipStreamSynchronize(ctx->st));
  });
}

int bk_debug_std_sort(bk_ctx *ctx, const uint32_t *key, const uint64_t *group_off, uint32_t n_groups, uint32_t *perm_out)
{
  return guarded(ctx, [&] {
    if (!key || !group_off || !perm_out) throw bk_error(BK_ERR_ARG, "bk_debug_std_sort: null argument");
    const uint64_t n = group_off[n_groups];
    DevBuf dk, dp, dgof, dgoff;
    std::vector<uint32_t> gof(n), iota(n);
    for (uint32_t g = 0; g < n_groups; ++g)
      for (uint64_t p = group_off[g]; p < group_off[g + 1]; ++p) gof[p] = g;
    std::iota(iota.begin(), iota.end(), 0u);
    HIP_CHECK(hipMemcpy(dk.as<uint32_t>(n + 1), key, n * 4, hipMemcpyHostToDevice));
    HIP_CHECK(hipMemcpy(dp.as<uint32_t>(n + 1), iota.data(), n * 4, hipMemcpyHostToDevice));
    HIP_CHECK(hipMemcpy(dgof.as<uint32_t>(n + 1), gof.data(), n * 4, hipMemcpyHostToDevice));
    HIP_CHECK(hipMemcpy(dgoff.as<uint64_t>((uint64_t) n_groups + 1), group_off, ((uint64_t) n_groups + 1) * 8, hipMemcpyHostToDevice));
    uint64_t max_group = 0;
    for (uint32_t g = 0; g < n_groups; ++g) max_group = std::max<uint64_t>(max_group, group_off[g + 1] - group_off[g]);
    ctx->stage.debug_sort(ctx->device, ctx->st, dk.get<uint32_t>(), dp.get<uint32_t>(), dgof.get<uint32_t>(), dgoff.get<uint64_t>(), n_groups, n, max_group);
    HIP_CHECK(hipMemcpyAsync(perm_out, dp.get<uint32_t>(), n * 4, hipMemcpyDeviceToHost, ctx->st));
    HIP_CHECK(hipStreamSynchronize(ctx->st));
  });
}

int bk_debug_scan(bk_ctx *ctx, int elem_bytes, const void *in, uint64_t n, int in_place, void *out)
{
  return guarded(ctx, [&] {
    if (elem_bytes != 4 && elem_bytes != 8) throw bk_error(BK_ERR_ARG, "bk_debug_scan: elem_bytes must be 4 or 8");
    if (!out || (n && !in)) throw bk_error(BK_ERR_ARG, "bk_debug_scan: null argument");
    auto run = [&](auto zero) {
      using T = decltype(zero);
      T *d_in = ctx->dbg_in.as<T>(n + 1);
      T *d_out = in_place ? d_in : ctx->dbg_out.as<T>(n + 1);
      HIP_CHECK(hipMemsetAsync(d_out, 0xA5, (n + 1) * sizeof(T), ctx->st));
      if (n) HIP_CHECK(hipMemcpyAsync(d_in, in, n * sizeof(T), hipMemcpyHostToDevice, ctx->st));
      prims::exclusive_scan<T>(d_in, d_out, n, ctx->dbg_radix.scan_tmp, ctx->st);
      HIP_CHECK(hipMemcpyAsync(out, d_out, (n + 1) * sizeof(T), hipMemcpyDeviceToHost, ctx->st));
      HIP_CHECK(hipStreamSynchronize(ctx->st));
    };
    if (elem_bytes == 4)
      run(uint32_t(0));
    else
      run(uint64_t(0));
  });
}

int bk_debug_radix_sort(bk_ctx *ctx, const uint64_t *keys, const uint32_t *vals, uint64_t n, int begin_bit, int end_bit, uint64_t *keys_out, uint32_t *vals_out)
{
  return guarded(ctx, [&] {
    if (n && (!keys || !vals || !keys_out || !vals_out)) throw bk_error(BK_ERR_ARG, "bk_debug_radix_sort: null argument");
    if (begin_bit < 0 || end_bit > 64) throw bk_error(BK_ERR_ARG, "bk_debug_radix_sort: bits outside [0, 64]");
    prims::radix_check_count(n);
    if (!n) return;
    prims::RadixBufs &rb = ctx->dbg_radix;
    uint64_t *dk = ctx->dbg_in.as<uint64_t>(n);
    uint32_t *dv = ctx->dbg_vals.as<uint32_t>(n);
    HIP_CHECK(hipMemsetAsync(rb.keys_alt.as<uint64_t>(n), 0xA5, n * 8, ctx->st));
    HIP_CHECK(hipMemsetAsync(rb.vals_alt.as<uint32_t>(n), 0xA5, n * 4, ctx->st));
    HIP_CHECK(hipMemcpyAsync(dk, keys, n * 8, hipMemcpyHostToDevice, ctx->st));
    HIP_CHECK(hipMemcpyAsync(dv, vals, n * 4, hipMemcpyHostToDevice, ctx->st));
    uint64_t *ko = nullptr;
    uint32_t *vo = nullptr;
    prims::radix_sort_pairs(dk, dv, n, begin_bit, end_bit, rb, ctx->st, &ko, &vo);
    HIP_CHECK(hipMemcpyAsync(keys_out, ko, n * 8, hipMemcpyDeviceToHost, ctx->st));
    HIP_CHECK(hipMemcpyAsync(vals_out, vo, n * 4, hipMemcpyDeviceToHost, ctx->st));
    HIP_CHECK(hipStreamSynchronize(ctx->st));
  });
}

int bk_debug_prims_info(uint64_t out[4])
{
  if (!out) return BK_ERR_ARG;
  out[0] = prims::BLOCK;
  out[1] = prims::SCAN_TILE;
  out[2] = prims::SCAN_ONE_MAX;
  out[3] = prims::RS_TILE;
  return BK_OK;
}

int bk_sort_forms(bk_ctx *ctx, uint64_t out[3])
{
  return guarded(ctx, [&] {
    if (!out) throw bk_error(BK_ERR_ARG, "bk_sort_forms: null output");
    ctx->stage.sort_forms(out);
  });
}

int bk_debug_ahc(bk_ctx *ctx, const uint32_t *x, const uint32_t *y, uint32_t n, double w, uint32_t *idx_out, int32_t *cluster_out, uint32_t *n_out)
{
  return guarded(ctx, [&] {
    if (!x || !y || !idx_out || !cluster_out || !n_out) throw bk_error(BK_ERR_ARG, "bk_debug_ahc: null argument");
    std::vector<bk_pair> hp(n);
    for (uint32_t i = 0; i < n; ++i)
    {
      memset(&hp[i], 0, sizeof(bk_pair));
      hp[i].x = x[i];
      hp[i].y = y[i];
    }
    DevBuf dp, dcl;
    PairList L;
    L.n = n;
    L.ng = 1;
    std::vector<uint32_t> iota(n), gof(n, 0);
    std::iota(iota.begin(), iota.end(), 0u);
    uint64_t goff[2] = {0, n};
    HIP_CHECK(hipMemcpy(dp.as<bk_pair>(n + 1), hp.data(), n * sizeof(bk_pair), hipMemcpyHostToDevice));
    HIP_CHECK(hipMemcpy(L.idx.as<uint32_t>(n + 1), iota.data(), n * 4, hipMemcpyHostToDevice));
    HIP_CHECK(hipMemcpy(L.gof.as<uint32_t>(n + 1), gof.data(), n * 4, hipMemcpyHostToDevice));
    HIP_CHECK(hipMemcpy(L.goff.as<uint64_t>(2), goff, 16, hipMemcpyHostToDevice));
    ahc_cluster_all(dp.get<bk_pair>(), L, w, dcl, ctx->stage.ab, ctx->stage.cb(), ctx->st);
    *n_out = (uint32_t) L.n;
    if (L.n)
    {
      HIP_CHECK(hipMemcpyAsync(idx_out, L.idx.get<uint32_t>(), L.n * 4, hipMemcpyDeviceToHost, ctx->st));
      HIP_CHECK(hipMemcpyAsync(cluster_out, dcl.get<uint32_t>(), L.n * 4, hipMemcpyDeviceToHost, ctx->st));
    }
    HIP_CHECK(hipStreamSynchronize(ctx->st));
  });
}

}

namespace
{
struct FeedLink
{
  int device = 0, mapq_min = 20;
  bk_ctx *ctx = nullptr;
  int rc = BK_OK;
  std::string err;
  uint64_t done = 0;
  bool prepared = false, overflow = false;
  hipEvent_t t0 = nullptr, t1 = nullptr;
  template <class F> void guard(F &&f)
  {
    if (rc != BK_OK) return;
    try
    {
      f();
    }
    catch (const bk_error &e)
    {
      rc = e.code;
      err = e.msg;
    }
  }
};
void link_header(void *u, int nt, const char *const *names, const uint32_t *lens)
{
  FeedLink *L = (FeedLink *) u;
  if (L->ctx || L->rc != BK_OK) return;
  L->rc = bk_init(L->device, lens, names, nt, &L->ctx);
  if (L->rc != BK_OK) L->err = bk_last_error(nullptr);
}
void link_reset(void *u)
{
  FeedLink *L = (FeedLink *) u;
  L->guard([&] {
    if (L->ctx) HIP_CHECK(hipStreamSynchronize(L->ctx->st));
    L->done = 0;
    L->prepared = false;
    L->overflow = false;
  });
}
void link_before_move(void *u)
{
  FeedLink *L = (FeedLink *) u;
  L->guard([&] {
    if (L->ctx) HIP_CHECK(hipStreamSynchronize(L->ctx->st));
  });
}
void link_chunk(void *u, const bk_soa *cols, uint64_t n_ready, uint64_t n_est, hipEvent_t ready)
{
  FeedLink *L = (FeedLink *) u;
  L->guard([&] {
    bk_ctx *c = L->ctx;
    if (!c || n_ready < (uint64_t) STREAM_V + 1) return;
    c->rec = *cols;
    c->have_records = true;
    c->mapq_min = L->mapq_min;
    if (!L->prepared)
    {
      stream_prepare(c, n_est + n_est / 4);
      L->prepared = true;
    }
    const uint64_t lim = (n_ready - 1) / STREAM_V * STREAM_V;
    if (lim <= L->done) return;
    HIP_CHECK(hipStreamWaitEvent(c->st, ready, 0));
    StreamArgs a = stream_args(c, lim);
    a.q_begin = L->done / STREAM_V;
    launch_stream(a, c->st);
    L->done = lim;
  });
}
}


extern "C" {

int bk_bam_decode_device_ctx(const char *path, int device, int mapq_min, bk_bam_dev **bam_out, bk_ctx **ctx_out, int *n_targets, const char *const **names,
                             const uint32_t **lens, char *err, size_t errlen)
{
  auto fail = [&](int code, const std::string &m) {
    if (err && errlen) snprintf(err, errlen, "%s", m.c_str());
    return code;
  };
  if (!path || !bam_out || !ctx_out) return fail(BK_ERR_ARG, "bk_bam_decode_device_ctx: null argument");
  *bam_out = nullptr;
  *ctx_out = nullptr;
  FeedLink L;
  L.device = device;
  L.mapq_min = mapq_min;
  FeedConsumer fc;
  fc.user = &L;
  fc.on_header = link_header;
  fc.on_chunk = link_chunk;
  fc.before_move = link_before_move;
  fc.on_reset = link_reset;
  bk_soa cols;
  bk_bam_dev *bam = nullptr;
  int rc = bam_decode_device_impl(path, device, &bam, &cols, n_targets, names, lens, err, errlen, &fc);
  if (rc == BK_OK && L.rc != BK_OK) rc = fail(L.rc, L.err);
  if (rc == BK_OK && !L.ctx) rc = fail(BK_ERR_IO, "bk_bam_decode_device_ctx: no header");
  if (rc != BK_OK)
  {
    if (L.ctx) bk_free(L.ctx);
    if (bam) bk_bam_dev_free(bam);
    return rc;
  }
  bk_ctx *c = L.ctx;
  rc = guarded(c, [&] {
    const uint64_t done = L.prepared ? L.done : 0;
    c->stream_done = c->stats_done = c->clustered = false;
    c->rec = cols;
    c->have_records = true;
    c->mapq_min = mapq_min;
    c->rec_base = 0;
    bool ok = false;
    if (L.prepared)
    {
      Scope s(c, "k_stream", 39ull * cols.n + 4ull * cols.n_cigar_words);
      StreamArgs a = stream_args(c, cols.n);
      a.q_begin = done / STREAM_V;
      launch_stream(a, c->st);
      ok = stream_finish(c);
    }
    if (ok)
      stream_rare_path(c);
    else
      run_stream(c);
    if (bk_debug("feed"))
      fprintf(stderr, "[feed/stream] stream pass %s: %llu of %llu records went through k_stream while the file was still arriving\n", ok ? "overlapped" : "after the feed",
              (unsigned long long) (ok ? done : 0), (unsigned long long) cols.n);
  });
  if (rc != BK_OK)
  {
    fail(rc, c->err);
    bk_free(c);
    bk_bam_dev_free(bam);
    return rc;
  }
  *bam_out = bam;
  *ctx_out = c;
  return BK_OK;
}

int bk_group_stats(bk_ctx *ctx, const bk_group_stat **out, uint32_t *n_groups)
{
  return guarded(ctx, [&] {
    if (!out || !n_groups) throw bk_error(BK_ERR_ARG, "bk_group_stats: null output");
    if (!ctx->clustered) throw bk_error(BK_ERR_ARG, "bk_group_stats: call bk_mask_and_cluster (and bk_cluster_summary) first");
    const uint32_t ng = ctx->jr.n_groups;
    std::vector<uint64_t> iso(ng + 1, 0), clu(ng + 1, 0);
    std::vector<uint32_t> kmax(ng + 1, 0);
    if (ng)
    {
      HIP_CHECK(hipMemcpyAsync(iso.data(), ctx->stage.iso_goff.get<uint64_t>(), ((uint64_t) ng + 1) * 8, hipMemcpyDeviceToHost, ctx->st));
      HIP_CHECK(hipMemcpyAsync(clu.data(), ctx->stage.list.goff.get<uint64_t>(), ((uint64_t) ng + 1) * 8, hipMemcpyDeviceToHost, ctx->st));
      if (ctx->stage.list.n && ctx->bb.kmax.p) HIP_CHECK(hipMemcpyAsync(kmax.data(), ctx->bb.kmax.get<uint32_t>(), (uint64_t) ng * 4, hipMemcpyDeviceToHost, ctx->st));
      HIP_CHECK(hipStreamSynchronize(ctx->st));
    }
    ctx->f_gstats.assign(ng, bk_group_stat{});
    for (uint32_t l = 0; l < ng; ++l)
    {
      const uint32_t g = ctx->lex_to_num[l];
      bk_group_stat &o = ctx->f_gstats[l];
      const uint32_t k = ctx->gkey_host[g];
      o.p1_tid = (int32_t) (k / (uint32_t) (ctx->nt + 1)) - 1;
      o.p2_tid = (int32_t) (k % (uint32_t) (ctx->nt + 1)) - 1;
      o.n_scan = ctx->gstart_host[g + 1] - ctx->gstart_host[g];
      o.n_isolated_removed = iso[g + 1] - iso[g];
      o.n_clustered = clu[g + 1] - clu[g];
      o.cluster_id_end = o.n_clustered ? kmax[g] : 0;
      o.ordinal = ctx->glex_host[g];
    }
    *out = ctx->f_gstats.data();
    *n_groups = ng;
  });
}

int bk_debug_points(bk_ctx *ctx, int mode, const uint32_t *x, const uint32_t *y, uint32_t n, double w, uint32_t *idx_out, int32_t *cluster_out, uint32_t *n_out)
{
  return guarded(ctx, [&] {
    if ((n && (!x || !y)) || !idx_out || !n_out || mode < 0 || mode > 2) throw bk_error(BK_ERR_ARG, "bk_debug_points: bad argument");
    std::vector<bk_pair> hp(n);
    for (uint32_t i = 0; i < n; ++i)
    {
      memset(&hp[i], 0, sizeof(bk_pair));
      hp[i].x = x[i];
      hp[i].y = y[i];
    }
    DevBuf dp, dcl, dgof, dgoff;
    PairList L;
    std::vector<uint32_t> gof(n, 0);
    uint64_t goff[2] = {0, n};
    if (n) HIP_CHECK(hipMemcpy(dp.as<bk_pair>(n + 1), hp.data(), n * sizeof(bk_pair), hipMemcpyHostToDevice));
    if (n) HIP_CHECK(hipMemcpy(dgof.as<uint32_t>(n + 1), gof.data(), n * 4, hipMemcpyHostToDevice));
    HIP_CHECK(hipMemcpy(dgoff.as<uint64_t>(2), goff, 16, hipMemcpyHostToDevice));
    const bk_pair *pairs = dp.as<bk_pair>(n + 1);
    remove_isolated_all(pairs, dgof.get<uint32_t>(), dgoff.get<uint64_t>(), 1, mode == 1 ? n : 0, w, L, ctx->stage.cb(), ctx->st);
    if (mode != 1)
    {
      L.n = n;
      L.ng = 1;
      std::vector<uint32_t> iota(n);
      std::iota(iota.begin(), iota.end(), 0u);
      if (n) HIP_CHECK(hipMemcpy(L.idx.as<uint32_t>(n + 1), iota.data(), n * 4, hipMemcpyHostToDevice));
      if (n) HIP_CHECK(hipMemcpy(L.gof.as<uint32_t>(n + 1), gof.data(), n * 4, hipMemcpyHostToDevice));
      HIP_CHECK(hipMemcpy(L.goff.as<uint64_t>(2), goff, 16, hipMemcpyHostToDevice));
      if (mode == 0)
        debug_mask_list(pairs, L, (long) w, ctx->stage.cb(), ctx->st);
      else
        fast_cluster_all(pairs, L, w, dcl, ctx->stage.cb(), ctx->st);
    }
    *n_out = (uint32_t) L.n;
    if (L.n)
    {
      HIP_CHECK(hipMemcpyAsync(idx_out, L.idx.get<uint32_t>(), L.n * 4, hipMemcpyDeviceToHost, ctx->st));
      if (mode == 2 && cluster_out) HIP_CHECK(hipMemcpyAsync(cluster_out, dcl.get<uint32_t>(), L.n * 4, hipMemcpyDeviceToHost, ctx->st));
    }
    HIP_CHECK(hipStreamSynchronize(ctx->st));
  });
}

int bk_debug_cigar(bk_ctx *ctx, uint32_t n, const uint8_t *kind, const uint32_t *c1_off, const uint8_t *c1, const uint32_t *c2_off, const uint8_t *c2, const int32_t *e,
                   int32_t *out6)
{
  return guarded(ctx, [&] {
    if (!n) return;
    if (!kind || !c1_off || !c1 || !c2_off || !c2 || !e || !out6) throw bk_error(BK_ERR_ARG, "bk_debug_cigar: null argument");
    DevBuf dk, d1o, d1, d2o, d2, de, dout;
    HIP_CHECK(hipMemcpy(dk.as<uint8_t>(n), kind, n, hipMemcpyHostToDevice));
    HIP_CHECK(hipMemcpy(d1o.as<uint32_t>(n + 1), c1_off, (n + 1) * 4, hipMemcpyHostToDevice));
    HIP_CHECK(hipMemcpy(d1.as<uint8_t>(c1_off[n] + 16), c1, c1_off[n], hipMemcpyHostToDevice));
    HIP_CHECK(hipMemcpy(d2o.as<uint32_t>(n + 1), c2_off, (n + 1) * 4, hipMemcpyHostToDevice));
    HIP_CHECK(hipMemcpy(d2.as<uint8_t>(c2_off[n] + 16), c2, c2_off[n], hipMemcpyHostToDevice));
    HIP_CHECK(hipMemcpy(de.as<int32_t>(n), e, n * 4, hipMemcpyHostToDevice));
    int32_t *o = dout.as<int32_t>(6ull * n);
    debug_cigar(dk.get<uint8_t>(), d1o.get<uint32_t>(), d1.get<uint8_t>(), d2o.get<uint32_t>(), d2.get<uint8_t>(), de.get<int32_t>(), n, o, ctx->st);
    HIP_CHECK(hipMemcpyAsync(out6, o, 24ull * n, hipMemcpyDeviceToHost, ctx->st));
    HIP_CHECK(hipStreamSynchronize(ctx->st));
  });
}

int bk_debug_vote(bk_ctx *ctx, const bk_split *side1, uint32_t n1, const bk_split *side2, uint32_t n2, int32_t p1_tid, int32_t p2_tid, int32_t *out3)
{
  return guarded(ctx, [&] {
    if ((n1 && !side1) || (n2 && !side2) || !out3) throw bk_error(BK_ERR_ARG, "bk_debug_vote: null argument");
    const uint32_t pos1 = 100000, pos2 = 300000;
    std::vector<bk_split> t;
    auto put = [&](const bk_split *src, uint32_t n, int32_t tid, uint32_t pos, uint64_t salt) {
      for (uint32_t i = 0; i < n + 2; ++i)
      {
        bk_split s;
        if (i < n)
          s = src[i];
        else
        {
          memset(&s, 0, sizeof s);
          s.qhash = 0xD00D000000000000ull + salt + i;
          s.prim_chr = s.sec_chr = -7;
        }
        s.tid = tid;
        s.pos = (int32_t) pos;
        s.endpos = (int32_t) pos + 50;
        t.push_back(s);
      }
    };
    put(side1, n1, p1_tid, pos1, 0);
    put(side2, n2, p2_tid, pos2, 1000);
    std::stable_sort(t.begin(), t.end(), [](const bk_split &a, const bk_split &b) { return (uint32_t) a.tid != (uint32_t) b.tid ? (uint32_t) a.tid < (uint32_t) b.tid : a.pos < b.pos; });
    for (size_t i = 0; i < t.size(); ++i) t[i].rec = i;
    bk_cluster c;
    memset(&c, 0, sizeof c);
    c.p1_tid = p1_tid;
    c.p2_tid = p2_tid;
    c.p1_mean = pos1 + 10;
    c.p2_mean = pos2 + 10;
    c.p1_exact = 0xFFFFFFFFu;
    c.p2_exact = -1;
    DevBuf dt, dc, dcov;
    HIP_CHECK(hipMemcpy(dt.as<bk_split>(t.size() + 1), t.data(), t.size() * sizeof(bk_split), hipMemcpyHostToDevice));
    HIP_CHECK(hipMemcpy(dc.as<bk_cluster>(2), &c, sizeof c, hipMemcpyHostToDevice));
    const uint32_t cov[2] = {5, 5};
    HIP_CHECK(hipMemcpy(dcov.as<uint32_t>(4), cov, 8, hipMemcpyHostToDevice));
    bp_vote(dt.get<bk_split>(), t.size(), dc.get<bk_cluster>(), 1, 1000.0, 200, dcov.get<uint32_t>(), ctx->d_hdr.get<int32_t>(), ctx->bb, ctx->st);
    uint32_t voted = 0;
    HIP_CHECK(hipMemcpyAsync(&voted, ctx->bb.voted.get<uint32_t>(), 4, hipMemcpyDeviceToHost, ctx->st));
    HIP_CHECK(hipMemcpyAsync(&c, dc.get<bk_cluster>(), sizeof c, hipMemcpyDeviceToHost, ctx->st));
    HIP_CHECK(hipStreamSynchronize(ctx->st));
    out3[0] = voted ? (int32_t) c.p1_exact : -1;
    out3[1] = voted ? c.p2_exact : -1;
    out3[2] = voted ? (int32_t) c.n_sr : 0;
  });
}

int bk_debug_region(bk_ctx *ctx, int32_t tid, uint32_t start, uint32_t end, uint64_t depth_pos, bk_split *out, uint32_t cap, uint32_t *n_out, uint32_t *cov_out,
                    uint32_t *depth_out)
{
  return guarded(ctx, [&] {
    if (!ctx->stream_done) run_stream(ctx);
    ensure_splits_sorted(ctx);
    DevBuf dout, dres;
    bk_split *o = dout.as<bk_split>((uint64_t) cap + 1);
    uint32_t *res = dres.as<uint32_t>(4);
    debug_region(rec_view(ctx), ctx->d_split.get<bk_split>(), ctx->hc.n_split, tid, start, end, (int) ctx->hc.max_span, depth_pos, o, cap, res, ctx->st);
    uint32_t h[4] = {0, 0, 0, 0};
    HIP_CHECK(hipMemcpyAsync(h, res, 16, hipMemcpyDeviceToHost, ctx->st));
    HIP_CHECK(hipStreamSynchronize(ctx->st));
    const uint32_t n = h[0] < cap ? h[0] : cap;
    if (n && out) HIP_CHECK(hipMemcpy(out, o, n * sizeof(bk_split), hipMemcpyDeviceToHost));
    if (n_out) *n_out = h[0];
    if (cov_out) *cov_out = h[1];
    if (depth_out) *depth_out = h[2];
  });
}

int bk_timing_enable(bk_ctx *ctx, int on)
{
  return guarded(ctx, [&] {
    ctx->timing = on != 0;
    for (auto &t : ctx->timers)
    {
      if (t.a) (void) hipEventDestroy(t.a);
      if (t.b) (void) hipEventDestroy(t.b);
    }
    ctx->timers.clear();
  });
}

int bk_timing(bk_ctx *ctx, const char *const **names, const float **ms, const uint64_t **bytes, int *n)
{
  return guarded(ctx, [&] {
    HIP_CHECK(hipStreamSynchronize(ctx->st));
    Timing &t = ctx->tout;
    t.names.clear(); t.ms.clear(); t.bytes.clear(); t.touched.clear(); t.cnames.clear();
    for (auto &s : ctx->timers)
    {
      float v = 0;
      HIP_CHECK(hipEventElapsedTime(&v, s.a, s.b));
      t.names.push_back(s.name);
      t.ms.push_back(v);
      t.bytes.push_back(s.bytes);
      t.touched.push_back(s.touched);
    }
    for (auto &s : t.names) t.cnames.push_back(s.c_str());
    if (names) *names = t.cnames.data();
    if (ms) *ms = t.ms.data();
    if (bytes) *bytes = t.bytes.data();
    if (n) *n = (int) t.names.size();
  });
}

int bk_timing_touched(bk_ctx *ctx, const uint64_t **touched, int *n)
{
  return guarded(ctx, [&] {
    if (touched) *touched = ctx->tout.touched.data();
    if (n) *n = (int) ctx->tout.touched.size();
  });
}

}
```

breakid_amd/csrc/bp.h:

```cpp
#pragma once
#include "bk_common.h"
#include "prims.h"

template <class Less> __device__ __forceinline__ uint64_t wave_lower(uint64_t lo, uint64_t hi, Less less)
{
  const uint32_t lane = threadIdx.x & 63;
  while (hi - lo > 64)
  {
    const uint64_t width = hi - lo;
    const uint64_t p = lo + width * (lane + 1) / 65;
    const uint32_t c = (uint32_t) __popcll(__ballot(less(p)));
    const uint64_t nlo = c ? lo + width * c / 65 + 1 : lo;
    const uint64_t nhi = c < 64 ? lo + width * (c + 1) / 65 : hi;
    lo = nlo;
    hi = nhi;
  }
  const uint64_t i = lo + lane;
  return lo + (uint64_t) __popcll(__ballot(i < hi && less(i)));
}
__device__ __forceinline__ uint32_t wave_sum_u32(uint32_t v)
{
  for (int d = 32; d; d >>= 1) v += (uint32_t) __shfl_xor((int) v, d, 64);
  return v;
}

struct ClusterAcc
{
  uint32_t *n;
  unsigned long long *sum1, *sum2;
  uint32_t *min1, *max1, *min2, *max2, *type;
};

struct RecView
{
  uint64_t n;
  const int32_t *tid, *pos;
  const uint16_t *flag;
  const uint8_t *mapq;
  const uint32_t *cigar_off, *cigar;
  const unsigned long long *samp = nullptr;
  uint64_t n_samp = 0;
  const int32_t *isize = nullptr;
  const uint32_t *aux_off = nullptr;
};

constexpr uint32_t REC_SAMPLE_SHIFT = 10;
__device__ __forceinline__ unsigned long long rec_key(int32_t tid, long long pos) { return ((unsigned long long) (uint32_t) tid << 32) | (uint32_t) (pos + 0x80000000ll); }
__device__ inline uint64_t rec_lower(const RecView &r, int32_t T, long long P)
{
  uint64_t lo = 0, hi = r.n;
  if (r.samp)
  {
    const unsigned long long want = rec_key(T, P < -0x80000000ll ? -0x80000000ll : P);
    const unsigned long long *__restrict__ samp = r.samp;
    const uint64_t a = wave_lower(0, r.n_samp, [&](uint64_t m) { return samp[m] < want; });
    lo = a ? ((a - 1) << REC_SAMPLE_SHIFT) + 1 : 0;
    hi = a < r.n_samp ? (a << REC_SAMPLE_SHIFT) : r.n;
  }
  const uint32_t Tu = (uint32_t) T;
  return wave_lower(lo, hi, [&](uint64_t m) {
    const uint32_t t = (uint32_t) r.tid[m];
    return t != Tu ? (t < Tu) : ((long long) r.pos[m] < P);
  });
}

struct BpWork
{
  uint64_t t1lo, t1hi, t2lo, t2hi;
  uint32_t ok, pad;
};

struct BpBufs
{
  DevBuf samp, key, val, kmax, lexbase, slotbase, an, as1, as2, amin1, amax1, amin2, amax2, atype, keep, off, tmpc, work, nmatch, moff, err, emit, ecount, scan_tmp, cov, depth, voted, nvalid, maxrec;
  prims::RadixBufs radix;
};

uint64_t count_valid_clusters(const bk_cluster *cl, uint64_t ncl, BpBufs &b, hipStream_t st);
void sort_splits(bk_split *unsorted, uint64_t n, bk_split *sorted, BpBufs &b, hipStream_t st, int rec_bits);
uint64_t cluster_summary(const bk_pair *pairs, const uint32_t *idx, const uint32_t *gof, const uint32_t *cl, uint64_t n, uint32_t ng, const uint32_t *gkey,
                         const uint32_t *glex, const uint32_t *lex_to_num, int32_t nt, double w, DevBuf &clusters_out, BpBufs &b, hipStream_t st);
RecView rec_sampled(const RecView &r, DevBuf &samp, hipStream_t st);
uint32_t *bp_cov_partial(const RecView &r, const bk_cluster *cl, uint64_t ncl, double w, int maxspan, BpBufs &b, hipStream_t st);
void bp_vote(const bk_split *sp, uint64_t nsp, bk_cluster *cl, uint64_t ncl, double w, int maxspan, const uint32_t *cov, const int32_t *hdr_id, BpBufs &b, hipStream_t st);
uint32_t *bp_depth_partial(const RecView &r, const bk_cluster *cl, uint64_t ncl, int maxspan, BpBufs &b, hipStream_t st);
void base_depth_at(const RecView &r, const int32_t *tid, const uint32_t *pos, uint64_t n, int maxspan, DevBuf &samp, hipStream_t st, uint32_t *depth);
void bp_finish(bk_cluster *cl, uint64_t ncl, const uint32_t *depth, BpBufs &b, hipStream_t st);
void split_breakpoints(const RecView &r, const bk_split *sp, uint64_t nsp, bk_cluster *cl, uint64_t ncl, double w, int maxspan, const int32_t *hdr_id, BpBufs &b,
                       hipStream_t st);
void debug_region(const RecView &r, const bk_split *sp, uint64_t nsp, int32_t tid, uint32_t start, uint32_t end, int maxspan, unsigned long long depth_pos, bk_split *out,
                  uint32_t cap, uint32_t *res, hipStream_t st);
```

breakid_amd/csrc/bp.hip:

```cpp
#include "bk_common.h"
#include "prims.h"
#include "bp.h"
#include <algorithm>
#include <vector>

namespace
{
__global__ __launch_bounds__(256) void k_group_kmax(const uint32_t *__restrict__ gof, const uint32_t *__restrict__ cl, uint64_t n, uint32_t *__restrict__ kmax)
{
  uint64_t p = (uint64_t) blockIdx.x * blockDim.x + threadIdx.x;
  const bool live = p < n;
  uint32_t g = live ? gof[p] : 0xFFFFFFFFu;
  uint32_t v = live ? cl[p] + 1 : 0u;
  __shared__ uint32_t s_g[4], s_v[4];
  const uint32_t g0 = __shfl(g, 0, 64);
  const bool wave_uniform = __ballot(live && g != g0) == 0ull;
  if (wave_uniform)
    for (int d = 32; d; d >>= 1) v = max(v, (uint32_t) __shfl_xor((int) v, d, 64));
  if ((threadIdx.x & 63) == 0)
  {
    s_g[threadIdx.x >> 6] = wave_uniform ? g0 : 0xFFFFFFFEu;
    s_v[threadIdx.x >> 6] = v;
  }
  __syncthreads();
  const bool block_uniform = s_g[0] == s_g[1] && s_g[1] == s_g[2] && s_g[2] == s_g[3] && s_g[0] < 0xFFFFFFFEu;
  if (block_uniform)
  {
    if (threadIdx.x == 0) atomicMax(&kmax[s_g[0]], max(max(s_v[0], s_v[1]), max(s_v[2], s_v[3])));
  }
  else if (wave_uniform)
  {
    if ((threadIdx.x & 63) == 0 && g0 != 0xFFFFFFFFu) atomicMax(&kmax[g0], v);
  }
  else if (live)
    atomicMax(&kmax[g], v);
}
__global__ __launch_bounds__(256) void k_accumulate(const bk_pair *__restrict__ pairs, const uint32_t *__restrict__ idx, const uint32_t *__restrict__ gof,
                                                    const uint32_t *__restrict__ cl, const uint32_t *__restrict__ slotbase, uint64_t n, ClusterAcc acc)
{
  const uint64_t p = (uint64_t) blockIdx.x * blockDim.x + threadIdx.x;
  const int lane = threadIdx.x & 63;
  const bool live = p < n;
  uint32_t s = 0xFFFFFFFFu, cnt = 0, mn1 = 0xFFFFFFFFu, mx1 = 0, mn2 = 0xFFFFFFFFu, mx2 = 0, type = 0;
  unsigned long long s1 = 0, s2 = 0;
  if (live)
  {
    const bk_pair pr = pairs[idx[p]];
    s = slotbase[gof[p]] + cl[p];
    cnt = 1;
    s1 = pr.p1_pos;
    s2 = pr.p2_pos;
    mn1 = mx1 = pr.p1_pos;
    mn2 = mx2 = pr.p2_pos;
    if (pr.p1_tid != pr.p2_tid)
      type = BK_TYPE_DIFF_CHR;
    else
    {
      if (pr.p1_rev && !pr.p2_rev) type |= BK_TYPE_ABS_REVERSE;
      if (pr.p1_rev == pr.p2_rev) type |= BK_TYPE_SAME_ORIENT;
      if (!pr.p1_rev && pr.p2_rev) type |= BK_TYPE_DEFAULT_ORIENT;
    }
  }
  const uint32_t s_prev = __shfl_up(s, 1, 64), s_next = __shfl_down(s, 1, 64);
  bool head = lane == 0 || s_prev != s;
  const bool tail = lane == 63 || s_next != s;
  for (int d = 1; d < 64; d <<= 1)
  {
    const uint32_t o_cnt = __shfl_up(cnt, d, 64), o_mn1 = __shfl_up(mn1, d, 64), o_mx1 = __shfl_up(mx1, d, 64), o_mn2 = __shfl_up(mn2, d, 64),
                   o_mx2 = __shfl_up(mx2, d, 64), o_type = __shfl_up(type, d, 64);
    const unsigned long long o_s1 = __shfl_up(s1, d, 64), o_s2 = __shfl_up(s2, d, 64);
    const int o_head = __shfl_up((int) head, d, 64);
    if (lane >= d && !head)
    {
      cnt += o_cnt;
      s1 += o_s1;
      s2 += o_s2;
      mn1 = min(mn1, o_mn1);
      mx1 = max(mx1, o_mx1);
      mn2 = min(mn2, o_mn2);
      mx2 = max(mx2, o_mx2);
      type |= o_type;
      head = o_head != 0;
    }
  }
  if (!live || !tail) return;
  atomicAdd(&acc.n[s], cnt);
  atomicAdd(&acc.sum1[s], s1);
  atomicAdd(&acc.sum2[s], s2);
  atomicMin(&acc.min1[s], mn1);
  atomicMax(&acc.max1[s], mx1);
  atomicMin(&acc.min2[s], mn2);
  atomicMax(&acc.max2[s], mx2);
  atomicOr(&acc.type[s], type);
}
__global__ __launch_bounds__(prims::BLOCK) void k_slot_bases(const uint32_t *__restrict__ kmax, const uint32_t *__restrict__ lex_to_num, uint32_t ng,
                                                             uint32_t *__restrict__ lexbase, uint32_t *__restrict__ slotbase)
{
  __shared__ uint32_t lds[prims::WAVES];
  uint32_t carry = 0;
  for (uint32_t base = 0; base < ng; base += prims::BLOCK)
  {
    const uint32_t l = base + threadIdx.x;
    const uint32_t g = l < ng ? lex_to_num[l] : 0u;
    const uint32_t v = l < ng ? kmax[g] : 0u;
    uint32_t tot;
    const uint32_t ex = prims::block_exclusive_scan(v, lds, tot);
    if (l < ng) lexbase[l] = slotbase[g] = carry + ex;
    carry += tot;
  }
  if (threadIdx.x == 0) lexbase[ng] = slotbase[ng] = carry;
}
__global__ __launch_bounds__(256) void k_finalize(ClusterAcc acc, const uint32_t *__restrict__ lexbase, const uint32_t *__restrict__ lex_to_num, uint32_t ng, uint32_t nslots,
                                                  const uint32_t *__restrict__ gkey, const uint32_t *__restrict__ glex, int32_t nt, double w, uint32_t *__restrict__ keep,
                                                  bk_cluster *__restrict__ tmp)
{
  uint32_t s = blockIdx.x * blockDim.x + threadIdx.x;
  if (s >= nslots) return;
  uint32_t k = 0;
  uint32_t n = acc.n[s];
  if (n)
  {
    uint32_t lo = 0, hi = ng;
    while (lo < hi)
    {
      uint32_t m = (lo + hi) >> 1;
      if (lexbase[m] <= s) lo = m + 1; else hi = m;
    }
    const uint32_t g = lex_to_num[lo - 1];
    bk_cluster c;
    c.group = glex[g];
    c.id = (int32_t) (s - lexbase[lo - 1]);
    c.p1_tid = (int32_t) (gkey[g] / (uint32_t) (nt + 1)) - 1;
    c.p2_tid = (int32_t) (gkey[g] % (uint32_t) (nt + 1)) - 1;
    unsigned long long m1 = (uint32_t) ((double) acc.sum1[s] / (double) n);
    unsigned long long m2 = (uint32_t) ((double) acc.sum2[s] / (double) n);
    c.p1_mean = (uint32_t) m1;
    c.p2_mean = (uint32_t) m2;
    c.p1_min = acc.min1[s];
    c.p1_max = acc.max1[s];
    c.p2_min = acc.min2[s];
    c.p2_max = acc.max2[s];
    c.p1_exact = 0xFFFFFFFFu;
    c.p2_exact = -1;
    c.n_drp = n;
    c.n_sr = 0;
    c.depth1 = c.depth2 = 0;
    c.type_mask = acc.type[s];
    long long dist = (long long) (m1 - m2);
    bool same = c.p1_tid == c.p2_tid;
    bool near = same && (double) dist <= 2 * w && (double) dist >= -2 * w;
    c.flags = near ? 0u : 1u;
    k = near ? 0u : 1u;
    tmp[s] = c;
  }
  keep[s] = k;
}
__global__ __launch_bounds__(256) void k_compact_clusters(const uint32_t *__restrict__ keep, const uint32_t *__restrict__ off, uint32_t nslots, const bk_cluster *__restrict__ tmp,
                                                          bk_cluster *__restrict__ out)
{
  uint32_t s = blockIdx.x * blockDim.x + threadIdx.x;
  if (s < nslots && keep[s]) out[off[s]] = tmp[s];
}

__device__ __forceinline__ int32_t rec_endpos(const RecView &r, uint64_t i)
{
  return bam_endpos_hts(r.flag[i], r.pos[i], r.cigar, r.cigar_off[i], r.cigar_off[i + 1]);
}
__global__ __launch_bounds__(256) void k_rec_sample(const int32_t *__restrict__ tid, const int32_t *__restrict__ pos, uint64_t n_samp, unsigned long long *__restrict__ samp)
{
  const uint64_t j = (uint64_t) blockIdx.x * blockDim.x + threadIdx.x;
  if (j < n_samp) samp[j] = rec_key(tid[j << REC_SAMPLE_SHIFT], (long long) pos[j << REC_SAMPLE_SHIFT]);
}
__device__ uint64_t split_lower(const bk_split *__restrict__ sp, uint64_t ns, uint64_t rec)
{
  uint64_t lo = 0, hi = ns;
  while (lo < hi)
  {
    uint64_t m = (lo + hi) >> 1;
    if ((uint64_t) sp[m].rec < rec) lo = m + 1; else hi = m;
  }
  return lo;
}
__device__ __forceinline__ long long wave_sum(long long v)
{
  for (int d = 32; d; d >>= 1) v += __shfl_xor(v, d, 64);
  return v;
}

struct Region
{
  int32_t tid;
  int beg, end;
  bool valid;
};
__device__ __forceinline__ Region make_region(int32_t tid, uint32_t mean, int wi)
{
  Region r;
  uint32_t rs = (uint32_t) ((unsigned long long) mean - (unsigned long long) (long long) wi);
  uint32_t re = (uint32_t) ((unsigned long long) mean + (unsigned long long) (long long) wi);
  r.tid = tid;
  r.beg = (int) rs;
  r.end = (int) re;
  if (r.beg < 0) r.beg = 0;
  r.valid = !(r.end < r.beg || tid < 0);
  return r;
}
__device__ __forceinline__ bool in_region(const Region &rg, int32_t tid, int32_t pos, int32_t endpos) { return tid == rg.tid && pos < rg.end && endpos > rg.beg; }

__device__ uint64_t split_lower_pos(const bk_split *__restrict__ sp, uint64_t ns, int32_t T, long long P)
{
  const uint32_t Tu = (uint32_t) T;
  return wave_lower(0, ns, [&](uint64_t m) {
    const uint32_t t = (uint32_t) sp[m].tid;
    return t != Tu ? (t < Tu) : ((long long) sp[m].pos < P);
  });
}

constexpr uint32_t COV_ENOUGH = 5;
__device__ uint32_t region_cov(const RecView &r, const Region &rg, int maxspan)
{
  if (!rg.valid) return 0;
  const int lane = threadIdx.x & 63;
  const uint64_t lo = rec_lower(r, rg.tid, (long long) rg.beg - maxspan);
  uint32_t cov = 0;
  for (uint64_t base = lo; base < r.n && cov < COV_ENOUGH; base += 64)
  {
    const uint64_t i = base + lane;
    bool hit = false, past = true;
    if (i < r.n)
    {
      const int32_t t = r.tid[i], p = r.pos[i];
      past = t != rg.tid || p >= rg.end;
      hit = !past && in_region(rg, t, p, rec_endpos(r, i));
    }
    cov += (uint32_t) __popcll(__ballot(hit));
    if (__ballot(past)) break;
  }
  return cov < COV_ENOUGH ? cov : COV_ENOUGH;
}

__global__ __launch_bounds__(256) void k_bp_cov(RecView r, const bk_cluster *__restrict__ cl, uint32_t ncl, int wi, int maxspan, uint32_t *__restrict__ cov)
{
  const uint32_t c = blockIdx.x * 4 + (threadIdx.x >> 6);
  if (c >= ncl) return;
  const bk_cluster k = cl[c];
  uint32_t c1 = region_cov(r, make_region(k.p1_tid, k.p1_mean, wi), maxspan);
  uint32_t c2 = region_cov(r, make_region(k.p2_tid, k.p2_mean, wi), maxspan);
  if ((threadIdx.x & 63) == 0)
  {
    cov[2 * c] = c1;
    cov[2 * c + 1] = c2;
  }
}

__device__ bool side_verdict(const bk_split *__restrict__ sp, uint64_t nsp, const Region &rg, int maxspan, uint32_t cov, uint64_t &tlo, uint64_t &thi, bool &poison)
{
  tlo = thi = 0;
  if (!rg.valid) return false;
  const int lane = threadIdx.x & 63;
  tlo = split_lower_pos(sp, nsp, rg.tid, (long long) rg.beg - maxspan);
  thi = split_lower_pos(sp, nsp, rg.tid, (long long) rg.end);
  long long ev = 0, bad = 0;
  for (uint64_t t = tlo + lane; t < thi; t += 64)
  {
    const bk_split s = sp[t];
    if (in_region(rg, s.tid, s.pos, s.endpos))
    {
      ++ev;
      if (s.flags & 2u) ++bad;
    }
  }
  ev = wave_sum(ev);
  bad = wave_sum(bad);
  if (bad) poison = true;
  return !(cov < 5 || ev < 2);
}

__device__ __forceinline__ bool tuples_match_at(const bk_split *__restrict__ pa, const bk_split *__restrict__ pb, uint32_t *__restrict__ err)
{
  if (pa->qhash != pb->qhash) return false;
  const bk_split a = *pa, b = *pb;
  if (a.qcheck != b.qcheck)
  {
    if (err) atomicOr(err, 2u);
    return false;
  }
  return ((a.flags ^ b.flags) & 1u) && a.prim_chr == b.prim_chr && a.sec_chr == b.sec_chr && a.reserved == b.reserved && a.prim_start == b.prim_start && a.sec_start == b.sec_start &&
         a.prim_end == b.prim_end && a.sec_end == b.sec_end && a.prim_cigar == b.prim_cigar && a.sec_cigar == b.sec_cigar && a.prim_bp == b.prim_bp && a.sec_bp == b.sec_bp;
}

__device__ __forceinline__ bool tuples_match(const bk_split &a, const bk_split &b)
{
  return a.qhash == b.qhash && ((a.flags ^ b.flags) & 1u) && a.prim_chr == b.prim_chr && a.sec_chr == b.sec_chr && a.reserved == b.reserved && a.prim_start == b.prim_start &&
         a.sec_start == b.sec_start && a.prim_end == b.prim_end && a.sec_end == b.sec_end && a.prim_cigar == b.prim_cigar && a.sec_cigar == b.sec_cigar &&
         a.prim_bp == b.prim_bp && a.sec_bp == b.sec_bp;
}

__global__ __launch_bounds__(256) void k_bp_regions(const bk_split *__restrict__ sp, uint64_t nsp, const bk_cluster *__restrict__ cl, uint32_t ncl, int wi, int maxspan,
                                                    const uint32_t *__restrict__ cov, BpWork *__restrict__ work, uint32_t *__restrict__ nmatch, uint32_t *__restrict__ err)
{
  const uint32_t c = blockIdx.x * 4 + (threadIdx.x >> 6);
  const int lane = threadIdx.x & 63;
  if (c >= ncl) return;
  const bk_cluster k = cl[c];
  BpWork wk;
  wk.ok = 0;
  wk.pad = 0;
  wk.t1lo = wk.t1hi = wk.t2lo = wk.t2hi = 0;
  bool poison = false;
  Region r1 = make_region(k.p1_tid, k.p1_mean, wi), r2 = make_region(k.p2_tid, k.p2_mean, wi);
  bool ok1 = side_verdict(sp, nsp, r1, maxspan, cov[2 * c], wk.t1lo, wk.t1hi, poison);
  bool ok2 = false;
  if (ok1) ok2 = side_verdict(sp, nsp, r2, maxspan, cov[2 * c + 1], wk.t2lo, wk.t2hi, poison);
  long long m = 0;
  if (ok1 && ok2)
  {
    wk.ok = 1;
    const uint64_t n2 = wk.t2hi - wk.t2lo, total = (wk.t1hi - wk.t1lo) * n2;
    for (uint64_t q = lane; q < total; q += 64)
    {
      const uint64_t qi = total <= 0xFFFFFFFFull ? (uint64_t) ((uint32_t) q / (uint32_t) n2) : q / n2;
      const bk_split *pa = sp + wk.t1lo + qi, *pb = sp + wk.t2lo + (q - qi * n2);
      if (!tuples_match_at(pa, pb, err)) continue;
      if (in_region(r1, pa->tid, pa->pos, pa->endpos) && in_region(r2, pb->tid, pb->pos, pb->endpos)) ++m;
    }
    m = wave_sum(m);
  }
  if (lane == 0)
  {
    work[c] = wk;
    nmatch[c] = (uint32_t) m;
    if (poison) atomicOr(err, 1u);
  }
}

__device__ int key_text(int32_t a, int32_t b, char *out)
{
  int n = 0;
  for (int part = 0; part < 2; ++part)
  {
    long long v = part ? b : a;
    char tmp[12];
    int t = 0;
    bool neg = v < 0;
    if (neg) v = -v;
    do
    {
      tmp[t++] = (char) ('0' + v % 10);
      v /= 10;
    } while (v);
    if (neg) out[n++] = '-';
    while (t) out[n++] = tmp[--t];
    if (!part) out[n++] = ',';
  }
  return n;
}
__device__ bool key_less(int32_t a1, int32_t a2, int32_t b1, int32_t b2)
{
  char sa[28], sb[28];
  int la = key_text(a1, a2, sa), lb = key_text(b1, b2, sb);
  int l = la < lb ? la : lb;
  for (int i = 0; i < l; ++i)
  {
    unsigned char x = (unsigned char) sa[i], y = (unsigned char) sb[i];
    if (x != y) return x < y;
  }
  return la < lb;
}

__device__ __forceinline__ unsigned long long key_code(int32_t v, unsigned long long pad)
{
  const bool neg = v < 0;
  uint32_t u = neg ? (uint32_t) (-(long long) v) : (uint32_t) v;
  unsigned long long code = 0;
  int len = 0;
  do
  {
    code |= (unsigned long long) (3u + u % 10u) << (4 * len);
    u /= 10u;
    ++len;
  } while (u);
  if (neg) code |= 2ull << (4 * len++);
  const int sh = 4 * (11 - len);
  return (code << sh) | ((0x11111111111ull * pad) & ((1ull << sh) - 1ull));
}

constexpr uint32_t VOTE_LDS = 256;
__global__ __launch_bounds__(256) void k_bp_vote(const bk_split *__restrict__ sp, bk_cluster *__restrict__ cl, uint32_t ncl, int wi, const BpWork *__restrict__ work,
                                                 const uint32_t *__restrict__ moff, int2 *__restrict__ emit, uint32_t *__restrict__ ecount,
                                                 const int32_t *__restrict__ hdr_id, uint32_t *__restrict__ voted)
{
  const uint32_t c = blockIdx.x * 4 + (threadIdx.x >> 6);
  const int lane = threadIdx.x & 63;
  __shared__ int2 s_emit[4][VOTE_LDS];
  __shared__ unsigned int s_ecount[4];
  if (c >= ncl) return;
  if (lane == 0) voted[c] = 0;
  const BpWork wk = work[c];
  bk_cluster k = cl[c];
  const uint32_t m0 = moff[c], m1 = moff[c + 1];
  if (!wk.ok) return;
  const uint32_t K = m1 - m0;
  if (K == 0) return;
  Region r1 = make_region(k.p1_tid, k.p1_mean, wi), r2 = make_region(k.p2_tid, k.p2_mean, wi);
  const int32_t p1_chr = hdr_id[k.p1_tid + 1];
  const bool in_lds = K <= VOTE_LDS;
  const int wv = threadIdx.x >> 6;
  int2 *E = in_lds ? s_emit[wv] : emit + m0;
  if (in_lds && lane == 0) s_ecount[wv] = 0;
  __builtin_amdgcn_wave_barrier();
  const uint64_t n1 = wk.t1hi - wk.t1lo, n2 = wk.t2hi - wk.t2lo, total = n1 * n2;
  for (uint64_t q = lane; q < total; q += 64)
  {
    const uint64_t qi = total <= 0xFFFFFFFFull ? (uint64_t) ((uint32_t) q / (uint32_t) n2) : q / n2;
    const uint64_t i = wk.t1lo + qi, j = wk.t2lo + (q - qi * n2);
    const bk_split *pa = sp + i, *pb = sp + j;
    if (!tuples_match_at(pa, pb, nullptr)) continue;
    {
      const bk_split a = *pa, b = *pb;
      if (in_region(r1, a.tid, a.pos, a.endpos) && in_region(r2, b.tid, b.pos, b.endpos))
      {
        uint32_t slot = in_lds ? atomicAdd(&s_ecount[wv], 1u) : atomicAdd(&ecount[c], 1u);
        int2 e;
        if (a.prim_chr == p1_chr)
        {
          e.x = (int32_t) a.prim_bp;
          e.y = (int32_t) a.sec_bp;
        }
        else
        {
          e.x = (int32_t) a.sec_bp;
          e.y = (int32_t) a.prim_bp;
        }
        if (slot < K) E[slot] = e;
      }
    }
  }
  if (in_lds)
    __builtin_amdgcn_fence(__ATOMIC_SEQ_CST, "wavefront");
  else
    __builtin_amdgcn_fence(__ATOMIC_SEQ_CST, "agent");
  __builtin_amdgcn_wave_barrier();
  int best_cnt = 0;
  int32_t best1 = 0, best2 = 0;
  unsigned long long bk1 = 0, bk2 = 0;
  for (uint32_t q = lane; q < K; q += 64)
  {
    const int2 e = E[q];
    const uint32_t t1 = (uint32_t) e.x, t2 = (uint32_t) e.y;
    int cnt = 0;
    for (uint32_t m = 0; m < K; ++m)
    {
      const int2 u = E[m];
      if (((uint32_t) u.x <= t1 + 2u && (uint32_t) u.x >= t1 - 2u) && ((uint32_t) u.y <= t2 + 2u && (uint32_t) u.y >= t2 - 2u)) ++cnt;
    }
    if (cnt >= best_cnt && cnt > 0)
    {
      const unsigned long long k1 = key_code(e.x, 1ull), k2 = key_code(e.y, 0ull);
      if (cnt > best_cnt || k1 < bk1 || (k1 == bk1 && k2 < bk2))
      {
        best_cnt = cnt;
        best1 = e.x;
        best2 = e.y;
        bk1 = k1;
        bk2 = k2;
      }
    }
  }
  for (int d = 32; d; d >>= 1)
  {
    const int oc = __shfl_xor(best_cnt, d, 64);
    const int32_t o1 = __shfl_xor(best1, d, 64), o2 = __shfl_xor(best2, d, 64);
    const unsigned long long ok1 = __shfl_xor(bk1, d, 64), ok2 = __shfl_xor(bk2, d, 64);
    if (oc > best_cnt || (oc == best_cnt && oc > 0 && (ok1 < bk1 || (ok1 == bk1 && ok2 < bk2))))
    {
      best_cnt = oc;
      best1 = o1;
      best2 = o2;
      bk1 = ok1;
      bk2 = ok2;
    }
  }
  if (best_cnt >= 2 && lane == 0)
  {
    k.p1_exact = (uint32_t) best1;
    k.p2_exact = best2;
    k.n_sr = (uint32_t) best_cnt;
    cl[c] = k;
    voted[c] = 1;
  }
}

__device__ uint32_t base_depth_wave(const RecView &r, int32_t tid, unsigned long long pos, int maxspan)
{
  int beg = (int) (pos - 1ull), end = (int) pos;
  if (beg < 0) beg = 0;
  if (end < beg || tid < 0) return 0;
  Region rg;
  rg.tid = tid;
  rg.beg = beg;
  rg.end = end;
  rg.valid = true;
  const int lane = threadIdx.x & 63;
  uint64_t lo = rec_lower(r, tid, (long long) beg - maxspan), hi = rec_lower(r, tid, (long long) end);
  long long acc = 0;
  for (uint64_t i = lo + lane; i < hi; i += 64)
  {
    if (!in_region(rg, r.tid[i], r.pos[i], rec_endpos(r, i))) continue;
    uint16_t f = r.flag[i];
    if (r.mapq[i] > 0 && !(f & 0x400) && (f & 1)) ++acc;
  }
  return (uint32_t) wave_sum(acc);
}

__global__ __launch_bounds__(256) void k_bp_depth(RecView r, const bk_cluster *__restrict__ cl, uint32_t ncl, int maxspan, const uint32_t *__restrict__ voted,
                                                  uint32_t *__restrict__ depth)
{
  const uint32_t c = blockIdx.x * 4 + (threadIdx.x >> 6);
  if (c >= ncl) return;
  uint32_t d1 = 0, d2 = 0;
  if (voted[c])
  {
    const bk_cluster k = cl[c];
    d1 = base_depth_wave(r, k.p1_tid, (unsigned long long) k.p1_exact, maxspan);
    d2 = base_depth_wave(r, k.p2_tid, (unsigned long long) (long long) k.p2_exact, maxspan);
  }
  if ((threadIdx.x & 63) == 0)
  {
    depth[2 * c] = d1;
    depth[2 * c + 1] = d2;
  }
}

__global__ __launch_bounds__(256) void k_base_depth_at(RecView r, const int32_t *__restrict__ tid, const uint32_t *__restrict__ pos, uint32_t n, int maxspan,
                                                       uint32_t *__restrict__ depth)
{
  const uint32_t j = blockIdx.x * 4 + (threadIdx.x >> 6);
  if (j >= n) return;
  const uint32_t d = base_depth_wave(r, tid[j], (unsigned long long) pos[j], maxspan);
  if ((threadIdx.x & 63) == 0) depth[j] = d;
}

__global__ __launch_bounds__(64) void k_debug_region(RecView r, const bk_split *__restrict__ sp, uint64_t nsp, int32_t tid, uint32_t start, uint32_t end, int maxspan,
                                                     unsigned long long depth_pos, bk_split *__restrict__ out, uint32_t cap, uint32_t *__restrict__ res)
{
  Region rg;
  rg.tid = tid;
  rg.beg = (int) start;
  rg.end = (int) end;
  if (rg.beg < 0) rg.beg = 0;
  rg.valid = !(rg.end < rg.beg || tid < 0);
  const int lane = threadIdx.x & 63;
  const uint32_t cov = region_cov(r, rg, maxspan);
  uint64_t tlo, thi;
  bool poison = false;
  const bool ok = side_verdict(sp, nsp, rg, maxspan, cov, tlo, thi, poison);
  const uint32_t depth = base_depth_wave(r, tid, depth_pos, maxspan);
  if (lane == 0)
  {
    uint32_t n = 0;
    if (ok)
      for (uint64_t t = tlo; t < thi; ++t)
        if (in_region(rg, sp[t].tid, sp[t].pos, sp[t].endpos))
        {
          if (n < cap) out[n] = sp[t];
          ++n;
        }
    res[0] = n;
    res[1] = cov;
    res[2] = depth;
    res[3] = poison ? 1u : 0u;
  }
}
__global__ __launch_bounds__(256) void k_bp_finish(bk_cluster *__restrict__ cl, uint32_t ncl, const uint32_t *__restrict__ voted, const uint32_t *__restrict__ depth)
{
  uint32_t c = blockIdx.x * blockDim.x + threadIdx.x;
  if (c >= ncl || !voted[c]) return;
  cl[c].depth1 = depth[2 * c];
  cl[c].depth2 = depth[2 * c + 1];
  cl[c].flags |= 2u;
}

__global__ __launch_bounds__(256) void k_split_keys(const bk_split *__restrict__ sp, uint64_t n, uint64_t *__restrict__ key, uint32_t *__restrict__ val, unsigned long long *__restrict__ max_rec)
{
  uint64_t i = (uint64_t) blockIdx.x * blockDim.x + threadIdx.x;
  unsigned long long r = 0;
  if (i < n)
  {
    r = sp[i].rec;
    key[i] = r;
    val[i] = (uint32_t) i;
  }
  if (max_rec)
  {
    for (int d = 32; d >= 1; d >>= 1)
    {
      const unsigned long long o = __shfl_xor(r, d, 64);
      r = o > r ? o : r;
    }
    if ((threadIdx.x & 63) == 0 && r) atomicMax(max_rec, r);
  }
}
__global__ __launch_bounds__(256) void k_split_gather(const bk_split *__restrict__ in, const uint32_t *__restrict__ perm, uint64_t n, bk_split *__restrict__ out)
{
  uint64_t i = (uint64_t) blockIdx.x * blockDim.x + threadIdx.x;
  if (i < n) out[i] = in[perm[i]];
}
}

static inline unsigned nb(uint64_t n) { return cdiv(n ? n : 1, 256); }

void sort_splits(bk_split *unsorted, uint64_t n, bk_split *sorted, BpBufs &b, hipStream_t st, int rec_bits)
{
  if (n == 0) return;
  uint64_t *key = b.key.as<uint64_t>(n);
  uint32_t *val = b.val.as<uint32_t>(n);
  unsigned long long *mx = nullptr;
  if (rec_bits <= 0)
  {
    mx = b.maxrec.as<unsigned long long>(2);
    HIP_CHECK(hipMemsetAsync(mx, 0, 8, st));
  }
  hipLaunchKernelGGL(k_split_keys, dim3(nb(n)), dim3(256), 0, st, unsorted, n, key, val, mx);
  if (mx)
  {
    unsigned long long h = 0;
    HIP_CHECK(hipMemcpyAsync(&h, mx, 8, hipMemcpyDeviceToHost, st));
    HIP_CHECK(hipStreamSynchronize(st));
    rec_bits = 1;
    while (rec_bits < 64 && (h >> rec_bits) != 0ull) ++rec_bits;
  }
  uint64_t *ks;
  uint32_t *vs;
  prims::radix_sort_pairs(key, val, n, 0, rec_bits, b.radix, st, &ks, &vs);
  hipLaunchKernelGGL(k_split_gather, dim3(nb(n)), dim3(256), 0, st, unsorted, vs, n, sorted);
}

uint64_t cluster_summary(const bk_pair *pairs, const uint32_t *idx, const uint32_t *gof, const uint32_t *cl, uint64_t n, uint32_t ng, const uint32_t *gkey,
                         const uint32_t *glex, const uint32_t *lex_to_num, int32_t nt, double w, DevBuf &clusters_out, BpBufs &b, hipStream_t st)
{
  if (n == 0 || ng == 0) return 0;
  uint32_t *kmax = b.kmax.as<uint32_t>((uint64_t) ng + 1);
  HIP_CHECK(hipMemsetAsync(kmax, 0, ((uint64_t) ng + 1) * 4, st));
  hipLaunchKernelGGL(k_group_kmax, dim3(nb(n)), dim3(256), 0, st, gof, cl, n, kmax);
  uint32_t *slotbase = b.slotbase.as<uint32_t>((uint64_t) ng + 1), *lexbase = b.lexbase.as<uint32_t>((uint64_t) ng + 1);
  hipLaunchKernelGGL(k_slot_bases, dim3(1), dim3(prims::BLOCK), 0, st, kmax, lex_to_num, ng, lexbase, slotbase);
  uint32_t nslots = 0;
  HIP_CHECK(hipMemcpyAsync(&nslots, lexbase + ng, 4, hipMemcpyDeviceToHost, st));
  HIP_CHECK(hipStreamSynchronize(st));
  if (nslots == 0) return 0;
  ClusterAcc acc;
  acc.n = b.an.as<uint32_t>(nslots);
  acc.sum1 = b.as1.as<unsigned long long>(nslots);
  acc.sum2 = b.as2.as<unsigned long long>(nslots);
  acc.min1 = b.amin1.as<uint32_t>(nslots);
  acc.max1 = b.amax1.as<uint32_t>(nslots);
  acc.min2 = b.amin2.as<uint32_t>(nslots);
  acc.max2 = b.amax2.as<uint32_t>(nslots);
  acc.type = b.atype.as<uint32_t>(nslots);
  HIP_CHECK(hipMemsetAsync(acc.n, 0, (size_t) nslots * 4, st));
  HIP_CHECK(hipMemsetAsync(acc.sum1, 0, (size_t) nslots * 8, st));
  HIP_CHECK(hipMemsetAsync(acc.sum2, 0, (size_t) nslots * 8, st));
  HIP_CHECK(hipMemsetAsync(acc.min1, 0xFF, (size_t) nslots * 4, st));
  HIP_CHECK(hipMemsetAsync(acc.max1, 0, (size_t) nslots * 4, st));
  HIP_CHECK(hipMemsetAsync(acc.min2, 0xFF, (size_t) nslots * 4, st));
  HIP_CHECK(hipMemsetAsync(acc.max2, 0, (size_t) nslots * 4, st));
  HIP_CHECK(hipMemsetAsync(acc.type, 0, (size_t) nslots * 4, st));
  hipLaunchKernelGGL(k_accumulate, dim3(nb(n)), dim3(256), 0, st, pairs, idx, gof, cl, slotbase, n, acc);
  uint32_t *keep = b.keep.as<uint32_t>((uint64_t) nslots + 1), *off = b.off.as<uint32_t>((uint64_t) nslots + 1);
  bk_cluster *tmp = b.tmpc.as<bk_cluster>(nslots);
  hipLaunchKernelGGL(k_finalize, dim3(nb(nslots)), dim3(256), 0, st, acc, lexbase, lex_to_num, ng, nslots, gkey, glex, nt, w, keep, tmp);
  prims::exclusive_scan<uint32_t>(keep, off, nslots, b.scan_tmp, st);
  uint32_t nk = 0;
  HIP_CHECK(hipMemcpyAsync(&nk, off + nslots, 4, hipMemcpyDeviceToHost, st));
  HIP_CHECK(hipStreamSynchronize(st));
  bk_cluster *out = clusters_out.as<bk_cluster>((uint64_t) nk + 1);
  if (nk) hipLaunchKernelGGL(k_compact_clusters, dim3(nb(nslots)), dim3(256), 0, st, keep, off, nslots, tmp, out);
  return nk;
}

RecView rec_sampled(const RecView &r, DevBuf &samp, hipStream_t st)
{
  RecView v = r;
  v.n_samp = (r.n + (1ull << REC_SAMPLE_SHIFT) - 1) >> REC_SAMPLE_SHIFT;
  v.samp = nullptr;
  if (r.n >= (64ull << REC_SAMPLE_SHIFT))
  {
    unsigned long long *sp = samp.as<unsigned long long>(v.n_samp + 1);
    hipLaunchKernelGGL(k_rec_sample, dim3(cdiv(v.n_samp, 256)), dim3(256), 0, st, r.tid, r.pos, v.n_samp, sp);
    v.samp = sp;
  }
  return v;
}
static RecView sampled(const RecView &r, BpBufs &b, hipStream_t st) { return rec_sampled(r, b.samp, st); }

uint32_t *bp_cov_partial(const RecView &r0, const bk_cluster *cl, uint64_t ncl, double w, int maxspan, BpBufs &b, hipStream_t st)
{
  const RecView r = sampled(r0, b, st);
  uint32_t *cov = b.cov.as<uint32_t>(2 * ncl + 2);
  if (ncl) hipLaunchKernelGGL(k_bp_cov, dim3(cdiv(ncl, 4)), dim3(256), 0, st, r, cl, (uint32_t) ncl, (int) w, maxspan, cov);
  return cov;
}

void bp_vote(const bk_split *sp, uint64_t nsp, bk_cluster *cl, uint64_t ncl, double w, int maxspan, const uint32_t *cov, const int32_t *hdr_id, BpBufs &b, hipStream_t st)
{
  uint32_t *voted = b.voted.as<uint32_t>(ncl + 1);
  if (ncl == 0) return;
  if (ncl > 0x7FFFFFFFull) throw bk_error(BK_ERR_LIMIT, "too many clusters");
  const int wi = (int) w;
  BpWork *work = b.work.as<BpWork>(ncl);
  uint32_t *nmatch = b.nmatch.as<uint32_t>(ncl + 1), *moff = b.moff.as<uint32_t>(ncl + 1);
  uint32_t *err = b.err.as<uint32_t>(4);
  HIP_CHECK(hipMemsetAsync(err, 0, 16, st));
  hipLaunchKernelGGL(k_bp_regions, dim3(cdiv(ncl, 4)), dim3(256), 0, st, sp, nsp, cl, (uint32_t) ncl, wi, maxspan, cov, work, nmatch, err);
  prims::exclusive_scan<uint32_t>(nmatch, moff, ncl, b.scan_tmp, st);
  uint32_t host[2] = {0, 0};
  HIP_CHECK(hipMemcpyAsync(&host[0], moff + ncl, 4, hipMemcpyDeviceToHost, st));
  HIP_CHECK(hipMemcpyAsync(&host[1], err, 4, hipMemcpyDeviceToHost, st));
  HIP_CHECK(hipStreamSynchronize(st));
  if (host[1] & 2u)
    throw bk_error(BK_ERR_COLLISION, "two different read names share one 64-bit name hash (their second hashes differ): the breakpoint vote would not be the reference's");
  if (host[1] & 1u) throw bk_error(BK_ERR_CIGAR, "error cigar: ");
  if (bk_debug("bp"))
  {
    std::vector<uint32_t> nm(ncl);
    std::vector<BpWork> wk(ncl);
    HIP_CHECK(hipMemcpy(nm.data(), nmatch, ncl * 4, hipMemcpyDeviceToHost));
    HIP_CHECK(hipMemcpy(wk.data(), work, ncl * sizeof(BpWork), hipMemcpyDeviceToHost));
    uint64_t okc = 0, kmax = 0, ksum = 0, pmax = 0, psum = 0, k0 = 0;
    for (uint64_t i = 0; i < ncl; ++i)
    {
      if (!wk[i].ok) continue;
      ++okc;
      const uint64_t pr = (wk[i].t1hi - wk[i].t1lo) * (wk[i].t2hi - wk[i].t2lo);
      kmax = std::max<uint64_t>(kmax, nm[i]);
      ksum += nm[i];
      pmax = std::max(pmax, pr);
      psum += pr;
      k0 += nm[i] == 0;
    }
    fprintf(stderr, "[bp] %llu clusters, %llu with both regions ok (%llu of them without a match): matches total %llu max %llu; tuple combinations total %llu max %llu\n",
            (unsigned long long) ncl, (unsigned long long) okc, (unsigned long long) k0, (unsigned long long) ksum, (unsigned long long) kmax, (unsigned long long) psum, (unsigned long long) pmax);
  }
  int2 *emit = b.emit.as<int2>((uint64_t) host[0] + 1);
  uint32_t *ecount = b.ecount.as<uint32_t>(ncl + 1);
  HIP_CHECK(hipMemsetAsync(ecount, 0, (ncl + 1) * 4, st));
  hipLaunchKernelGGL(k_bp_vote, dim3(cdiv(ncl, 4)), dim3(256), 0, st, sp, cl, (uint32_t) ncl, wi, work, moff, emit, ecount, hdr_id, voted);
}

uint32_t *bp_depth_partial(const RecView &r0, const bk_cluster *cl, uint64_t ncl, int maxspan, BpBufs &b, hipStream_t st)
{
  const RecView r = sampled(r0, b, st);
  uint32_t *depth = b.depth.as<uint32_t>(2 * ncl + 2);
  if (ncl) hipLaunchKernelGGL(k_bp_depth, dim3(cdiv(ncl, 4)), dim3(256), 0, st, r, cl, (uint32_t) ncl, maxspan, b.voted.get<uint32_t>(), depth);
  return depth;
}

void base_depth_at(const RecView &r0, const int32_t *tid, const uint32_t *pos, uint64_t n, int maxspan, DevBuf &samp, hipStream_t st, uint32_t *depth)
{
  if (n == 0) return;
  if (n > 0x3FFFFFFFull) throw bk_error(BK_ERR_LIMIT, "too many positions");
  const RecView r = rec_sampled(r0, samp, st);
  hipLaunchKernelGGL(k_base_depth_at, dim3(cdiv(n, 4)), dim3(256), 0, st, r, tid, pos, (uint32_t) n, maxspan, depth);
}

void bp_finish(bk_cluster *cl, uint64_t ncl, const uint32_t *depth, BpBufs &b, hipStream_t st)
{
  if (ncl) hipLaunchKernelGGL(k_bp_finish, dim3(cdiv(ncl, 256)), dim3(256), 0, st, cl, (uint32_t) ncl, b.voted.get<uint32_t>(), depth);
}

__global__ __launch_bounds__(256) void k_count_valid(const bk_cluster *__restrict__ cl, uint32_t ncl, unsigned long long *__restrict__ out)
{
  const uint32_t c = blockIdx.x * blockDim.x + threadIdx.x;
  const bool v = c < ncl && (cl[c].flags & 2u);
  const unsigned long long b = __ballot(v);
  if ((threadIdx.x & 63) == 0 && b) atomicAdd(out, (unsigned long long) __popcll(b));
}
uint64_t count_valid_clusters(const bk_cluster *cl, uint64_t ncl, BpBufs &b, hipStream_t st)
{
  if (ncl == 0) return 0;
  unsigned long long *d = b.nvalid.as<unsigned long long>(1), h = 0;
  HIP_CHECK(hipMemsetAsync(d, 0, 8, st));
  hipLaunchKernelGGL(k_count_valid, dim3(cdiv(ncl, 256)), dim3(256), 0, st, cl, (uint32_t) ncl, d);
  HIP_CHECK(hipMemcpyAsync(&h, d, 8, hipMemcpyDeviceToHost, st));
  HIP_CHECK(hipStreamSynchronize(st));
  return h;
}

void split_breakpoints(const RecView &r, const bk_split *sp, uint64_t nsp, bk_cluster *cl, uint64_t ncl, double w, int maxspan, const int32_t *hdr_id, BpBufs &b,
                       hipStream_t st)
{
  if (ncl == 0) return;
  const uint32_t *cov = bp_cov_partial(r, cl, ncl, w, maxspan, b, st);
  bp_vote(sp, nsp, cl, ncl, w, maxspan, cov, hdr_id, b, st);
  const uint32_t *depth = bp_depth_partial(r, cl, ncl, maxspan, b, st);
  bp_finish(cl, ncl, depth, b, st);
}

void debug_region(const RecView &r, const bk_split *sp, uint64_t nsp, int32_t tid, uint32_t start, uint32_t end, int maxspan, unsigned long long depth_pos, bk_split *out,
                  uint32_t cap, uint32_t *res, hipStream_t st)
{
  hipLaunchKernelGGL(k_debug_region, dim3(1), dim3(64), 0, st, r, sp, nsp, tid, start, end, maxspan, depth_pos, out, cap, res);
}
```

Before: 11690.

## Reorder breakpoint stages: split evidence first, skip coverage for hopeless clusters

Adds a split-evidence kernel that binary-searches precomputed split position keys and counts in-region splits per side before any read coverage is computed. The coverage kernel then skips clusters or sides that cannot pass the evidence test, and it scans both sides together with multi-key wave searches. It also records the lower bounds it finds so the depth kernel can start from them. The valid-cluster count is now accumulated in the finish kernel, which removes a separate count kernel. The cost is extra kernels and buffers and a more complicated ordering of stages. Clusters that are skipped get zero coverage, which has to agree with the old verdict logic.

Result: faster. 11950 (median of 6 runs) (+2.2%).

```diff
diff --git a/breakid_amd/csrc/api.hip b/breakid_amd/csrc/api.hip
--- a/breakid_amd/csrc/api.hip
+++ b/breakid_amd/csrc/api.hip
@@ -782,11 +782,11 @@
     r.cigar_off = ctx->rec.cigar_off; r.cigar = ctx->rec.cigar;
     {
       Scope s(ctx, "split_breakpoints");
-      split_breakpoints(r, ctx->d_split.get<bk_split>(), ctx->hc.n_split, ctx->clusters_ptr(), ctx->n_clusters, w, (int) ctx->hc.max_span,
-                        ctx->d_hdr.get<int32_t>(), ctx->bb, ctx->st);
+      split_breakpoints(r, ctx->d_split.get<bk_split>(), ctx->bb.tkey.get<unsigned long long>(), ctx->hc.n_split, ctx->clusters_ptr(), ctx->n_clusters, w,
+                        (int) ctx->hc.max_span, ctx->d_hdr.get<int32_t>(), ctx->bb, ctx->st);
     }
     ctx->bp_done = true;
-    if (n_valid) *n_valid = count_valid_clusters(ctx->clusters_ptr(), ctx->n_clusters, ctx->bb, ctx->st);
+    if (n_valid) *n_valid = bp_valid_count(ctx->n_clusters, ctx->bb, ctx->st);
   });
 }
 
@@ -1787,7 +1787,7 @@
 {
   return guarded(ctx, [&] {
     ensure_splits_sorted(ctx);
-    bp_vote(ctx->d_split.get<bk_split>(), ctx->hc.n_split, ctx->clusters_ptr(), ctx->n_clusters, w, (int) ctx->hc.max_span, (const uint32_t *) cov_total_dev,
+    bp_vote(ctx->d_split.get<bk_split>(), ctx->bb.tkey.get<unsigned long long>(), ctx->hc.n_split, ctx->clusters_ptr(), ctx->n_clusters, w, (int) ctx->hc.max_span, (const uint32_t *) cov_total_dev,
             ctx->d_hdr.get<int32_t>(), ctx->bb, ctx->st);
     HIP_CHECK(hipStreamSynchronize(ctx->st));
   });
@@ -1798,7 +1798,7 @@
   return guarded(ctx, [&] {
     if (lo > hi || hi > ctx->n_clusters || !clusters_dev || !voted_dev) throw bk_error(BK_ERR_ARG, "bk_shard_bp_vote_slice: bad range");
     ensure_splits_sorted(ctx);
-    bp_vote(ctx->d_split.get<bk_split>(), ctx->hc.n_split, ctx->clusters_ptr() + lo, hi - lo, w, (int) ctx->hc.max_span,
+    bp_vote(ctx->d_split.get<bk_split>(), ctx->bb.tkey.get<unsigned long long>(), ctx->hc.n_split, ctx->clusters_ptr() + lo, hi - lo, w, (int) ctx->hc.max_span,
             cov_total_dev ? (const uint32_t *) cov_total_dev + 2 * lo : nullptr, ctx->d_hdr.get<int32_t>(), ctx->bb, ctx->st);
     HIP_CHECK(hipStreamSynchronize(ctx->st));
     *clusters_dev = ctx->clusters_ptr() + lo;
@@ -2237,7 +2237,7 @@
     HIP_CHECK(hipMemcpy(dc.as<bk_cluster>(2), &c, sizeof c, hipMemcpyHostToDevice));
     const uint32_t cov[2] = {5, 5};
     HIP_CHECK(hipMemcpy(dcov.as<uint32_t>(4), cov, 8, hipMemcpyHostToDevice));
-    bp_vote(dt.get<bk_split>(), t.size(), dc.get<bk_cluster>(), 1, 1000.0, 200, dcov.get<uint32_t>(), ctx->d_hdr.get<int32_t>(), ctx->bb, ctx->st);
+    bp_vote(dt.get<bk_split>(), nullptr, t.size(), dc.get<bk_cluster>(), 1, 1000.0, 200, dcov.get<uint32_t>(), ctx->d_hdr.get<int32_t>(), ctx->bb, ctx->st);
     uint32_t voted = 0;
     HIP_CHECK(hipMemcpyAsync(&voted, ctx->bb.voted.get<uint32_t>(), 4, hipMemcpyDeviceToHost, ctx->st));
     HIP_CHECK(hipMemcpyAsync(&c, dc.get<bk_cluster>(), sizeof c, hipMemcpyDeviceToHost, ctx->st));
diff --git a/breakid_amd/csrc/bp.h b/breakid_amd/csrc/bp.h
--- a/breakid_amd/csrc/bp.h
+++ b/breakid_amd/csrc/bp.h
@@ -17,6 +17,40 @@
   }
   const uint64_t i = lo + lane;
   return lo + (uint64_t) __popcll(__ballot(i < hi && less(i)));
+}
+template <int N, class Key> __device__ __forceinline__ void wave_lower_keys(uint64_t (&lo)[N], uint64_t (&hi)[N], const unsigned long long (&want)[N], Key key)
+{
+  const uint32_t lane = threadIdx.x & 63;
+  for (;;)
+  {
+    bool any = false;
+#pragma unroll
+    for (int k = 0; k < N; ++k) any |= hi[k] - lo[k] > 64;
+    if (!any) break;
+    unsigned long long v[N];
+#pragma unroll
+    for (int k = 0; k < N; ++k)
+    {
+      const uint64_t width = hi[k] - lo[k];
+      v[k] = width > 64 ? key(lo[k] + width * (lane + 1) / 65) : ~0ull;
+    }
+#pragma unroll
+    for (int k = 0; k < N; ++k)
+    {
+      const uint64_t width = hi[k] - lo[k];
+      if (width <= 64) continue;
+      const uint32_t c = (uint32_t) __popcll(__ballot(v[k] < want[k]));
+      const uint64_t nlo = c ? lo[k] + width * c / 65 + 1 : lo[k];
+      const uint64_t nhi = c < 64 ? lo[k] + width * (c + 1) / 65 : hi[k];
+      lo[k] = nlo;
+      hi[k] = nhi;
+    }
+  }
+  unsigned long long v[N];
+#pragma unroll
+  for (int k = 0; k < N; ++k) v[k] = lo[k] + lane < hi[k] ? key(lo[k] + lane) : ~0ull;
+#pragma unroll
+  for (int k = 0; k < N; ++k) lo[k] += (uint64_t) __popcll(__ballot(lo[k] + lane < hi[k] && v[k] < want[k]));
 }
 __device__ __forceinline__ uint32_t wave_sum_u32(uint32_t v)
 {
@@ -64,15 +98,44 @@
   });
 }
 
+__device__ __forceinline__ unsigned long long rec_want(int32_t T, long long P) { return rec_key(T, P < -0x80000000ll ? -0x80000000ll : P); }
+template <int N> __device__ __forceinline__ void rec_lower_keys(const RecView &r, const unsigned long long (&want)[N], const bool (&on)[N], uint64_t (&out)[N])
+{
+  uint64_t hi[N];
+#pragma unroll
+  for (int k = 0; k < N; ++k)
+  {
+    out[k] = 0;
+    hi[k] = on[k] ? r.n : 0;
+  }
+  if (r.samp)
+  {
+    const unsigned long long *__restrict__ samp = r.samp;
+#pragma unroll
+    for (int k = 0; k < N; ++k) hi[k] = on[k] ? r.n_samp : 0;
+    wave_lower_keys<N>(out, hi, want, [&](uint64_t m) { return samp[m]; });
+#pragma unroll
+    for (int k = 0; k < N; ++k)
+    {
+      const uint64_t a = out[k];
+      out[k] = on[k] && a ? ((a - 1) << REC_SAMPLE_SHIFT) + 1 : 0;
+      hi[k] = !on[k] ? 0 : a < r.n_samp ? (a << REC_SAMPLE_SHIFT) : r.n;
+    }
+  }
+  const int32_t *__restrict__ tid = r.tid, *__restrict__ pos = r.pos;
+  wave_lower_keys<N>(out, hi, want, [&](uint64_t m) { return rec_key(tid[m], (long long) pos[m]); });
+}
+
+constexpr uint32_t BP_EV1_OK = 1u, BP_EV1_BAD = 2u, BP_EV2_OK = 4u, BP_EV2_BAD = 8u;
 struct BpWork
 {
   uint64_t t1lo, t1hi, t2lo, t2hi;
-  uint32_t ok, pad;
+  uint32_t ok, ev;
 };
 
 struct BpBufs
 {
-  DevBuf samp, key, val, kmax, lexbase, slotbase, an, as1, as2, amin1, amax1, amin2, amax2, atype, keep, off, tmpc, work, nmatch, moff, err, emit, ecount, scan_tmp, cov, depth, voted, nvalid, maxrec;
+  DevBuf samp, key, val, kmax, lexbase, slotbase, an, as1, as2, amin1, amax1, amin2, amax2, atype, keep, off, tmpc, work, nmatch, moff, err, emit, ecount, scan_tmp, cov, depth, voted, nvalid, maxrec, tkey, tkey_tmp, lb;
   prims::RadixBufs radix;
 };
 
@@ -82,11 +145,13 @@
                          const uint32_t *glex, const uint32_t *lex_to_num, int32_t nt, double w, DevBuf &clusters_out, BpBufs &b, hipStream_t st);
 RecView rec_sampled(const RecView &r, DevBuf &samp, hipStream_t st);
 uint32_t *bp_cov_partial(const RecView &r, const bk_cluster *cl, uint64_t ncl, double w, int maxspan, BpBufs &b, hipStream_t st);
-void bp_vote(const bk_split *sp, uint64_t nsp, bk_cluster *cl, uint64_t ncl, double w, int maxspan, const uint32_t *cov, const int32_t *hdr_id, BpBufs &b, hipStream_t st);
+void bp_vote(const bk_split *sp, const unsigned long long *tkey, uint64_t nsp, bk_cluster *cl, uint64_t ncl, double w, int maxspan, const uint32_t *cov, const int32_t *hdr_id,
+             BpBufs &b, hipStream_t st);
 uint32_t *bp_depth_partial(const RecView &r, const bk_cluster *cl, uint64_t ncl, int maxspan, BpBufs &b, hipStream_t st);
 void base_depth_at(const RecView &r, const int32_t *tid, const uint32_t *pos, uint64_t n, int maxspan, DevBuf &samp, hipStream_t st, uint32_t *depth);
 void bp_finish(bk_cluster *cl, uint64_t ncl, const uint32_t *depth, BpBufs &b, hipStream_t st);
-void split_breakpoints(const RecView &r, const bk_split *sp, uint64_t nsp, bk_cluster *cl, uint64_t ncl, double w, int maxspan, const int32_t *hdr_id, BpBufs &b,
-                       hipStream_t st);
+void split_breakpoints(const RecView &r, const bk_split *sp, const unsigned long long *tkey, uint64_t nsp, bk_cluster *cl, uint64_t ncl, double w, int maxspan,
+                       const int32_t *hdr_id, BpBufs &b, hipStream_t st);
+uint64_t bp_valid_count(uint64_t ncl, BpBufs &b, hipStream_t st);
 void debug_region(const RecView &r, const bk_split *sp, uint64_t nsp, int32_t tid, uint32_t start, uint32_t end, int maxspan, unsigned long long depth_pos, bk_split *out,
                   uint32_t cap, uint32_t *res, hipStream_t st);
diff --git a/breakid_amd/csrc/bp.hip b/breakid_amd/csrc/bp.hip
--- a/breakid_amd/csrc/bp.hip
+++ b/breakid_amd/csrc/bp.hip
@@ -239,17 +239,121 @@
   return cov < COV_ENOUGH ? cov : COV_ENOUGH;
 }
 
-__global__ __launch_bounds__(256) void k_bp_cov(RecView r, const bk_cluster *__restrict__ cl, uint32_t ncl, int wi, int maxspan, uint32_t *__restrict__ cov)
-{
-  const uint32_t c = blockIdx.x * 4 + (threadIdx.x >> 6);
+__device__ __forceinline__ uint32_t wave_cluster() { return (uint32_t) __builtin_amdgcn_readfirstlane((int) (blockIdx.x * 4 + (threadIdx.x >> 6))); }
+
+__global__ __launch_bounds__(256) void k_bp_ev(const bk_split *__restrict__ sp, const unsigned long long *__restrict__ tkey, uint64_t nsp, const bk_cluster *__restrict__ cl,
+                                               uint32_t ncl, int wi, int maxspan, BpWork *__restrict__ work)
+{
+  const uint32_t c = wave_cluster();
+  const int lane = threadIdx.x & 63;
   if (c >= ncl) return;
-  const bk_cluster k = cl[c];
-  uint32_t c1 = region_cov(r, make_region(k.p1_tid, k.p1_mean, wi), maxspan);
-  uint32_t c2 = region_cov(r, make_region(k.p2_tid, k.p2_mean, wi), maxspan);
-  if ((threadIdx.x & 63) == 0)
-  {
-    cov[2 * c] = c1;
-    cov[2 * c + 1] = c2;
+  const int32_t tid1 = cl[c].p1_tid, tid2 = cl[c].p2_tid;
+  const Region r1 = make_region(tid1, cl[c].p1_mean, wi), r2 = make_region(tid2, cl[c].p2_mean, wi);
+  const unsigned long long want[4] = {rec_want(r1.tid, (long long) r1.beg - maxspan), rec_want(r1.tid, (long long) r1.end), rec_want(r2.tid, (long long) r2.beg - maxspan),
+                                      rec_want(r2.tid, (long long) r2.end)};
+  uint64_t lo[4] = {0, 0, 0, 0}, hi[4] = {r1.valid ? nsp : 0, r1.valid ? nsp : 0, r2.valid ? nsp : 0, r2.valid ? nsp : 0};
+  wave_lower_keys<4>(lo, hi, want, [&](uint64_t m) { return tkey[m]; });
+  unsigned long long n1 = 0, n2 = 0;
+  for (uint64_t t1 = lo[0] + lane, t2 = lo[2] + lane; t1 < lo[1] || t2 < lo[3]; t1 += 64, t2 += 64)
+  {
+    const bool on1 = t1 < lo[1], on2 = t2 < lo[3];
+    const bk_split *a = sp + (on1 ? t1 : 0), *b = sp + (on2 ? t2 : 0);
+    int32_t at = 0, ap = 0, ae = 0, bt = 0, bp = 0, be = 0;
+    uint32_t af = 0, bf = 0;
+    if (on1) at = a->tid, ap = a->pos, ae = a->endpos, af = a->flags;
+    if (on2) bt = b->tid, bp = b->pos, be = b->endpos, bf = b->flags;
+    if (on1 && in_region(r1, at, ap, ae)) n1 += 1ull + ((af & 2u) ? 1ull << 32 : 0ull);
+    if (on2 && in_region(r2, bt, bp, be)) n2 += 1ull + ((bf & 2u) ? 1ull << 32 : 0ull);
+  }
+  n1 = (unsigned long long) wave_sum((long long) n1);
+  n2 = (unsigned long long) wave_sum((long long) n2);
+  if (lane == 0)
+  {
+    BpWork wk;
+    wk.t1lo = lo[0];
+    wk.t1hi = lo[1];
+    wk.t2lo = lo[2];
+    wk.t2hi = lo[3];
+    wk.ok = 0;
+    wk.ev = ((uint32_t) n1 >= 2u ? BP_EV1_OK : 0u) | (n1 >> 32 ? BP_EV1_BAD : 0u) | ((uint32_t) n2 >= 2u ? BP_EV2_OK : 0u) | (n2 >> 32 ? BP_EV2_BAD : 0u);
+    work[c] = wk;
+  }
+}
+
+constexpr unsigned long long NO_LB = ~0ull;
+__global__ __launch_bounds__(256) void k_bp_cov(RecView r, const bk_cluster *__restrict__ cl, uint32_t ncl, int wi, int maxspan, const BpWork *__restrict__ work,
+                                                uint32_t *__restrict__ cov, unsigned long long *__restrict__ lb)
+{
+  const uint32_t c = wave_cluster();
+  const int lane = threadIdx.x & 63;
+  if (c >= ncl) return;
+  const uint32_t ev = work ? work[c].ev : (BP_EV1_OK | BP_EV2_OK);
+  bool on[2] = {(ev & BP_EV1_OK) != 0, (ev & BP_EV1_OK) && (ev & BP_EV2_OK)};
+  uint32_t n[2] = {0, 0};
+  uint64_t lo[2] = {NO_LB, NO_LB};
+  if (on[0] || !work)
+  {
+    const Region rg[2] = {make_region(cl[c].p1_tid, cl[c].p1_mean, wi), make_region(cl[c].p2_tid, cl[c].p2_mean, wi)};
+    on[0] = on[0] && rg[0].valid;
+    on[1] = on[1] && rg[1].valid;
+    const unsigned long long want[2] = {rec_want(rg[0].tid, (long long) rg[0].beg - maxspan), rec_want(rg[1].tid, (long long) rg[1].beg - maxspan)};
+    uint64_t base[2];
+    rec_lower_keys<2>(r, want, on, base);
+    bool act[2];
+#pragma unroll
+    for (int s = 0; s < 2; ++s)
+    {
+      if (on[s]) lo[s] = base[s];
+      act[s] = on[s] && base[s] < r.n;
+    }
+    while (act[0] || act[1])
+    {
+      int32_t t[2], p[2];
+      uint32_t c0[2], c1[2];
+      uint16_t f[2];
+      bool live[2];
+#pragma unroll
+      for (int s = 0; s < 2; ++s)
+      {
+        const uint64_t i = base[s] + lane;
+        live[s] = act[s] && i < r.n;
+        t[s] = p[s] = 0;
+        c0[s] = c1[s] = 0;
+        f[s] = 0;
+        if (live[s])
+        {
+          t[s] = r.tid[i];
+          p[s] = r.pos[i];
+          f[s] = r.flag[i];
+          c0[s] = r.cigar_off[i];
+          c1[s] = r.cigar_off[i + 1];
+        }
+      }
+#pragma unroll
+      for (int s = 0; s < 2; ++s)
+      {
+        if (!act[s]) continue;
+        bool hit = false, past = true;
+        if (live[s])
+        {
+          past = t[s] != rg[s].tid || p[s] >= rg[s].end;
+          hit = !past && in_region(rg[s], t[s], p[s], bam_endpos_hts(f[s], p[s], r.cigar, c0[s], c1[s]));
+        }
+        n[s] += (uint32_t) __popcll(__ballot(hit));
+        base[s] += 64;
+        if (__ballot(past) || n[s] >= COV_ENOUGH || base[s] >= r.n) act[s] = false;
+      }
+    }
+  }
+  if (lane == 0)
+  {
+    cov[2 * c] = n[0] < COV_ENOUGH ? n[0] : COV_ENOUGH;
+    cov[2 * c + 1] = n[1] < COV_ENOUGH ? n[1] : COV_ENOUGH;
+    if (lb)
+    {
+      lb[2 * c] = lo[0];
+      lb[2 * c + 1] = lo[1];
+    }
   }
 }
 
@@ -296,26 +400,21 @@
          a.prim_bp == b.prim_bp && a.sec_bp == b.sec_bp;
 }
 
-__global__ __launch_bounds__(256) void k_bp_regions(const bk_split *__restrict__ sp, uint64_t nsp, const bk_cluster *__restrict__ cl, uint32_t ncl, int wi, int maxspan,
-                                                    const uint32_t *__restrict__ cov, BpWork *__restrict__ work, uint32_t *__restrict__ nmatch, uint32_t *__restrict__ err)
-{
-  const uint32_t c = blockIdx.x * 4 + (threadIdx.x >> 6);
+__global__ __launch_bounds__(256) void k_bp_match(const bk_split *__restrict__ sp, const bk_cluster *__restrict__ cl, uint32_t ncl, int wi, const uint32_t *__restrict__ cov,
+                                                  BpWork *__restrict__ work, uint32_t *__restrict__ nmatch, uint32_t *__restrict__ err)
+{
+  const uint32_t c = wave_cluster();
   const int lane = threadIdx.x & 63;
   if (c >= ncl) return;
-  const bk_cluster k = cl[c];
-  BpWork wk;
-  wk.ok = 0;
-  wk.pad = 0;
-  wk.t1lo = wk.t1hi = wk.t2lo = wk.t2hi = 0;
-  bool poison = false;
-  Region r1 = make_region(k.p1_tid, k.p1_mean, wi), r2 = make_region(k.p2_tid, k.p2_mean, wi);
-  bool ok1 = side_verdict(sp, nsp, r1, maxspan, cov[2 * c], wk.t1lo, wk.t1hi, poison);
-  bool ok2 = false;
-  if (ok1) ok2 = side_verdict(sp, nsp, r2, maxspan, cov[2 * c + 1], wk.t2lo, wk.t2hi, poison);
+  const uint32_t ev = work[c].ev;
+  const bool ok1 = cov[2 * c] >= 5 && (ev & BP_EV1_OK);
+  const bool ok2 = ok1 && cov[2 * c + 1] >= 5 && (ev & BP_EV2_OK);
+  const bool poison = (ev & BP_EV1_BAD) || (ok1 && (ev & BP_EV2_BAD));
   long long m = 0;
   if (ok1 && ok2)
   {
-    wk.ok = 1;
+    BpWork wk = work[c];
+    const Region r1 = make_region(cl[c].p1_tid, cl[c].p1_mean, wi), r2 = make_region(cl[c].p2_tid, cl[c].p2_mean, wi);
     const uint64_t n2 = wk.t2hi - wk.t2lo, total = (wk.t1hi - wk.t1lo) * n2;
     for (uint64_t q = lane; q < total; q += 64)
     {
@@ -328,7 +427,7 @@
   }
   if (lane == 0)
   {
-    work[c] = wk;
+    work[c].ok = ok1 && ok2 ? 1u : 0u;
     nmatch[c] = (uint32_t) m;
     if (poison) atomicOr(err, 1u);
   }
@@ -513,22 +612,133 @@
   return (uint32_t) wave_sum(acc);
 }
 
+template <int N> __device__ __forceinline__ void rec_lower_from(const RecView &r, const unsigned long long (&want)[N], const bool (&on)[N], const uint64_t (&start)[N],
+                                                                uint64_t (&out)[N])
+{
+  const uint32_t lane = threadIdx.x & 63;
+  const int32_t *__restrict__ tid = r.tid, *__restrict__ pos = r.pos;
+  uint64_t from[N], hi[N];
+  bool open[N];
+#pragma unroll
+  for (int k = 0; k < N; ++k)
+  {
+    const bool hinted = on[k] && start[k] <= r.n;
+    open[k] = hinted;
+    from[k] = hinted ? start[k] : 0;
+    out[k] = 0;
+    hi[k] = on[k] && !hinted ? r.n : 0;
+  }
+  for (uint64_t step = 8;; step *= 8)
+  {
+    bool any = false;
+#pragma unroll
+    for (int k = 0; k < N; ++k) any |= open[k];
+    if (!any) break;
+    bool less[N];
+#pragma unroll
+    for (int k = 0; k < N; ++k)
+    {
+      const uint64_t q = from[k] + (uint64_t) lane * step;
+      less[k] = open[k] && (q == 0 || (q - 1 < r.n && rec_key(tid[q - 1], (long long) pos[q - 1]) < want[k]));
+    }
+#pragma unroll
+    for (int k = 0; k < N; ++k)
+    {
+      if (!open[k]) continue;
+      const uint32_t c = (uint32_t) __popcll(__ballot(less[k]));
+      if (c == 64)
+        from[k] += 63 * step;
+      else
+      {
+        open[k] = false;
+        if (c == 0)
+          hi[k] = from[k] - 1;
+        else
+        {
+          out[k] = from[k] + (uint64_t) (c - 1) * step;
+          const uint64_t e = from[k] - 1 + (uint64_t) c * step;
+          hi[k] = e < r.n ? e : r.n;
+        }
+      }
+    }
+  }
+  wave_lower_keys<N>(out, hi, want, [&](uint64_t m) { return rec_key(tid[m], (long long) pos[m]); });
+}
+
+__device__ __forceinline__ bool depth_region(int32_t tid, unsigned long long pos, Region &rg)
+{
+  int beg = (int) (pos - 1ull), end = (int) pos;
+  if (beg < 0) beg = 0;
+  rg.tid = tid;
+  rg.beg = beg;
+  rg.end = end;
+  rg.valid = !(end < beg || tid < 0);
+  return rg.valid;
+}
+
 __global__ __launch_bounds__(256) void k_bp_depth(RecView r, const bk_cluster *__restrict__ cl, uint32_t ncl, int maxspan, const uint32_t *__restrict__ voted,
-                                                  uint32_t *__restrict__ depth)
-{
-  const uint32_t c = blockIdx.x * 4 + (threadIdx.x >> 6);
+                                                  const unsigned long long *__restrict__ lb, uint32_t *__restrict__ depth)
+{
+  const uint32_t c = wave_cluster();
+  const int lane = threadIdx.x & 63;
   if (c >= ncl) return;
-  uint32_t d1 = 0, d2 = 0;
+  long long acc[2] = {0, 0};
   if (voted[c])
   {
-    const bk_cluster k = cl[c];
-    d1 = base_depth_wave(r, k.p1_tid, (unsigned long long) k.p1_exact, maxspan);
-    d2 = base_depth_wave(r, k.p2_tid, (unsigned long long) (long long) k.p2_exact, maxspan);
-  }
-  if ((threadIdx.x & 63) == 0)
-  {
-    depth[2 * c] = d1;
-    depth[2 * c + 1] = d2;
+    Region rg[2];
+    const bool v1 = depth_region(cl[c].p1_tid, (unsigned long long) cl[c].p1_exact, rg[0]);
+    const bool v2 = depth_region(cl[c].p2_tid, (unsigned long long) (long long) cl[c].p2_exact, rg[1]);
+    const uint64_t h1 = lb ? lb[2 * c] : NO_LB, h2 = lb ? lb[2 * c + 1] : NO_LB;
+    const unsigned long long want[2] = {rec_want(rg[0].tid, (long long) rg[0].beg - maxspan), rec_want(rg[1].tid, (long long) rg[1].beg - maxspan)};
+    const bool on[2] = {v1, v2};
+    uint64_t base[2];
+    if (lb)
+    {
+      const uint64_t start[2] = {h1, h2};
+      rec_lower_from<2>(r, want, on, start, base);
+    }
+    else
+      rec_lower_keys<2>(r, want, on, base);
+    bool act[2] = {on[0] && base[0] < r.n, on[1] && base[1] < r.n};
+    while (act[0] || act[1])
+    {
+      int32_t t[2] = {0, 0}, p[2] = {0, 0};
+      uint32_t c0[2] = {0, 0}, c1[2] = {0, 0};
+      uint16_t f[2] = {0, 0};
+      uint8_t q[2] = {0, 0};
+      bool live[2];
+#pragma unroll
+      for (int s = 0; s < 2; ++s)
+      {
+        const uint64_t i = base[s] + lane;
+        live[s] = act[s] && i < r.n;
+        if (live[s])
+        {
+          t[s] = r.tid[i];
+          p[s] = r.pos[i];
+          f[s] = r.flag[i];
+          q[s] = r.mapq[i];
+          c0[s] = r.cigar_off[i];
+          c1[s] = r.cigar_off[i + 1];
+        }
+      }
+#pragma unroll
+      for (int s = 0; s < 2; ++s)
+      {
+        if (!act[s]) continue;
+        const bool past = !live[s] || ((uint32_t) t[s] != (uint32_t) rg[s].tid ? (uint32_t) t[s] > (uint32_t) rg[s].tid : p[s] >= rg[s].end);
+        if (!past && in_region(rg[s], t[s], p[s], bam_endpos_hts(f[s], p[s], r.cigar, c0[s], c1[s])) && q[s] > 0 && !(f[s] & 0x400) && (f[s] & 1)) ++acc[s];
+        base[s] += 64;
+        if (__ballot(past)) act[s] = false;
+      }
+    }
+    acc[0] = wave_sum(acc[0]);
+    acc[1] = wave_sum(acc[1]);
+  }
+  if (lane == 0)
+  {
+    depth[2 * c] = (uint32_t) acc[0];
+    depth[2 * c + 1] = (uint32_t) acc[1];
   }
 }
 
@@ -572,13 +782,28 @@
     res[3] = poison ? 1u : 0u;
   }
 }
-__global__ __launch_bounds__(256) void k_bp_finish(bk_cluster *__restrict__ cl, uint32_t ncl, const uint32_t *__restrict__ voted, const uint32_t *__restrict__ depth)
-{
-  uint32_t c = blockIdx.x * blockDim.x + threadIdx.x;
-  if (c >= ncl || !voted[c]) return;
-  cl[c].depth1 = depth[2 * c];
-  cl[c].depth2 = depth[2 * c + 1];
-  cl[c].flags |= 2u;
+__global__ __launch_bounds__(256) void k_bp_finish(bk_cluster *__restrict__ cl, uint32_t ncl, const uint32_t *__restrict__ voted, const uint32_t *__restrict__ depth,
+                                                   uint32_t *__restrict__ nvalid)
+{
+  __shared__ uint32_t s_n[4];
+  const uint32_t c = blockIdx.x * blockDim.x + threadIdx.x;
+  bool valid = false;
+  if (c < ncl)
+  {
+    uint32_t f = cl[c].flags;
+    if (voted[c])
+    {
+      cl[c].depth1 = depth[2 * c];
+      cl[c].depth2 = depth[2 * c + 1];
+      cl[c].flags = f |= 2u;
+    }
+    valid = (f & 2u) != 0;
+  }
+  if (!nvalid) return;
+  const uint32_t n = (uint32_t) __popcll(__ballot(valid));
+  if ((threadIdx.x & 63) == 0) s_n[threadIdx.x >> 6] = n;
+  __syncthreads();
+  if (threadIdx.x == 0 && s_n[0] + s_n[1] + s_n[2] + s_n[3]) atomicAdd(nvalid, s_n[0] + s_n[1] + s_n[2] + s_n[3]);
 }
 
 __global__ __launch_bounds__(256) void k_split_keys(const bk_split *__restrict__ sp, uint64_t n, uint64_t *__restrict__ key, uint32_t *__restrict__ val, unsigned long long *__restrict__ max_rec)
@@ -601,10 +826,19 @@
     if ((threadIdx.x & 63) == 0 && r) atomicMax(max_rec, r);
   }
 }
-__global__ __launch_bounds__(256) void k_split_gather(const bk_split *__restrict__ in, const uint32_t *__restrict__ perm, uint64_t n, bk_split *__restrict__ out)
+__global__ __launch_bounds__(256) void k_split_gather(const bk_split *__restrict__ in, const uint32_t *__restrict__ perm, uint64_t n, bk_split *__restrict__ out,
+                                                      unsigned long long *__restrict__ tkey)
 {
   uint64_t i = (uint64_t) blockIdx.x * blockDim.x + threadIdx.x;
-  if (i < n) out[i] = in[perm[i]];
+  if (i >= n) return;
+  const bk_split s = in[perm[i]];
+  out[i] = s;
+  tkey[i] = rec_key(s.tid, (long long) s.pos);
+}
+__global__ __launch_bounds__(256) void k_split_poskeys(const bk_split *__restrict__ sp, uint64_t n, unsigned long long *__restrict__ tkey)
+{
+  uint64_t i = (uint64_t) blockIdx.x * blockDim.x + threadIdx.x;
+  if (i < n) tkey[i] = rec_key(sp[i].tid, (long long) sp[i].pos);
 }
 }
 
@@ -633,7 +867,7 @@
   uint64_t *ks;
   uint32_t *vs;
   prims::radix_sort_pairs(key, val, n, 0, rec_bits, b.radix, st, &ks, &vs);
-  hipLaunchKernelGGL(k_split_gather, dim3(nb(n)), dim3(256), 0, st, unsorted, vs, n, sorted);
+  hipLaunchKernelGGL(k_split_gather, dim3(nb(n)), dim3(256), 0, st, unsorted, vs, n, sorted, b.tkey.as<unsigned long long>(n + 1));
 }
 
 uint64_t cluster_summary(const bk_pair *pairs, const uint32_t *idx, const uint32_t *gof, const uint32_t *cl, uint64_t n, uint32_t ng, const uint32_t *gkey,
@@ -694,25 +928,44 @@
 }
 static RecView sampled(const RecView &r, BpBufs &b, hipStream_t st) { return rec_sampled(r, b.samp, st); }
 
+static uint32_t *bp_cov_phase(const RecView &r, const bk_cluster *cl, uint64_t ncl, double w, int maxspan, const BpWork *skip, bool keep_lb, BpBufs &b, hipStream_t st)
+{
+  uint32_t *cov = b.cov.as<uint32_t>(2 * ncl + 2);
+  unsigned long long *lb = keep_lb ? b.lb.as<unsigned long long>(2 * ncl + 2) : nullptr;
+  if (ncl) hipLaunchKernelGGL(k_bp_cov, dim3(cdiv(ncl, 4)), dim3(256), 0, st, r, cl, (uint32_t) ncl, (int) w, maxspan, skip, cov, lb);
+  return cov;
+}
 uint32_t *bp_cov_partial(const RecView &r0, const bk_cluster *cl, uint64_t ncl, double w, int maxspan, BpBufs &b, hipStream_t st)
 {
-  const RecView r = sampled(r0, b, st);
-  uint32_t *cov = b.cov.as<uint32_t>(2 * ncl + 2);
-  if (ncl) hipLaunchKernelGGL(k_bp_cov, dim3(cdiv(ncl, 4)), dim3(256), 0, st, r, cl, (uint32_t) ncl, (int) w, maxspan, cov);
-  return cov;
-}
-
-void bp_vote(const bk_split *sp, uint64_t nsp, bk_cluster *cl, uint64_t ncl, double w, int maxspan, const uint32_t *cov, const int32_t *hdr_id, BpBufs &b, hipStream_t st)
+  return bp_cov_phase(sampled(r0, b, st), cl, ncl, w, maxspan, nullptr, false, b, st);
+}
+
+static const BpWork *bp_evidence(const bk_split *sp, const unsigned long long *tkey, uint64_t nsp, const bk_cluster *cl, uint64_t ncl, double w, int maxspan, BpBufs &b,
+                                 hipStream_t st)
+{
+  if (ncl > 0x7FFFFFFFull) throw bk_error(BK_ERR_LIMIT, "too many clusters");
+  BpWork *work = b.work.as<BpWork>(ncl + 1);
+  if (ncl == 0) return work;
+  if (!tkey)
+  {
+    unsigned long long *t = b.tkey_tmp.as<unsigned long long>(nsp + 1);
+    hipLaunchKernelGGL(k_split_poskeys, dim3(nb(nsp)), dim3(256), 0, st, sp, nsp, t);
+    tkey = t;
+  }
+  hipLaunchKernelGGL(k_bp_ev, dim3(cdiv(ncl, 4)), dim3(256), 0, st, sp, tkey, nsp, cl, (uint32_t) ncl, (int) w, maxspan, work);
+  return work;
+}
+
+static void bp_vote_phase(const bk_split *sp, uint64_t nsp, bk_cluster *cl, uint64_t ncl, double w, const uint32_t *cov, const int32_t *hdr_id, BpBufs &b, hipStream_t st)
 {
   uint32_t *voted = b.voted.as<uint32_t>(ncl + 1);
   if (ncl == 0) return;
-  if (ncl > 0x7FFFFFFFull) throw bk_error(BK_ERR_LIMIT, "too many clusters");
   const int wi = (int) w;
-  BpWork *work = b.work.as<BpWork>(ncl);
+  BpWork *work = b.work.get<BpWork>();
   uint32_t *nmatch = b.nmatch.as<uint32_t>(ncl + 1), *moff = b.moff.as<uint32_t>(ncl + 1);
   uint32_t *err = b.err.as<uint32_t>(4);
   HIP_CHECK(hipMemsetAsync(err, 0, 16, st));
-  hipLaunchKernelGGL(k_bp_regions, dim3(cdiv(ncl, 4)), dim3(256), 0, st, sp, nsp, cl, (uint32_t) ncl, wi, maxspan, cov, work, nmatch, err);
+  hipLaunchKernelGGL(k_bp_match, dim3(cdiv(ncl, 4)), dim3(256), 0, st, sp, cl, (uint32_t) ncl, wi, cov, work, nmatch, err);
   prims::exclusive_scan<uint32_t>(nmatch, moff, ncl, b.scan_tmp, st);
   uint32_t host[2] = {0, 0};
   HIP_CHECK(hipMemcpyAsync(&host[0], moff + ncl, 4, hipMemcpyDeviceToHost, st));
@@ -727,9 +980,12 @@
     std::vector<BpWork> wk(ncl);
     HIP_CHECK(hipMemcpy(nm.data(), nmatch, ncl * 4, hipMemcpyDeviceToHost));
     HIP_CHECK(hipMemcpy(wk.data(), work, ncl * sizeof(BpWork), hipMemcpyDeviceToHost));
-    uint64_t okc = 0, kmax = 0, ksum = 0, pmax = 0, psum = 0, k0 = 0;
+    uint64_t okc = 0, kmax = 0, ksum = 0, pmax = 0, psum = 0, k0 = 0, few_sides = 0, few1 = 0, few2 = 0;
     for (uint64_t i = 0; i < ncl; ++i)
     {
+      few_sides += !(wk[i].ev & BP_EV1_OK) + !(wk[i].ev & BP_EV2_OK);
+      few1 += !(wk[i].ev & BP_EV1_OK);
+      few2 += (wk[i].ev & BP_EV1_OK) && !(wk[i].ev & BP_EV2_OK);
       if (!wk[i].ok) continue;
       ++okc;
       const uint64_t pr = (wk[i].t1hi - wk[i].t1lo) * (wk[i].t2hi - wk[i].t2lo);
@@ -741,19 +997,30 @@
     }
     fprintf(stderr, "[bp] %llu clusters, %llu with both regions ok (%llu of them without a match): matches total %llu max %llu; tuple combinations total %llu max %llu\n",
             (unsigned long long) ncl, (unsigned long long) okc, (unsigned long long) k0, (unsigned long long) ksum, (unsigned long long) kmax, (unsigned long long) psum, (unsigned long long) pmax);
+    fprintf(stderr, "[bp] evidence first: %llu of %llu sides with ev < 2; %llu clusters with ev1 < 2 (no side counted), %llu with ev1 >= 2 and ev2 < 2 (side 1 counted alone)\n",
+            (unsigned long long) few_sides, (unsigned long long) (2 * ncl), (unsigned long long) few1, (unsigned long long) few2);
   }
   int2 *emit = b.emit.as<int2>((uint64_t) host[0] + 1);
   uint32_t *ecount = b.ecount.as<uint32_t>(ncl + 1);
   HIP_CHECK(hipMemsetAsync(ecount, 0, (ncl + 1) * 4, st));
   hipLaunchKernelGGL(k_bp_vote, dim3(cdiv(ncl, 4)), dim3(256), 0, st, sp, cl, (uint32_t) ncl, wi, work, moff, emit, ecount, hdr_id, voted);
 }
-
+void bp_vote(const bk_split *sp, const unsigned long long *tkey, uint64_t nsp, bk_cluster *cl, uint64_t ncl, double w, int maxspan, const uint32_t *cov, const int32_t *hdr_id,
+             BpBufs &b, hipStream_t st)
+{
+  bp_evidence(sp, tkey, nsp, cl, ncl, w, maxspan, b, st);
+  bp_vote_phase(sp, nsp, cl, ncl, w, cov, hdr_id, b, st);
+}
+
+static uint32_t *bp_depth_phase(const RecView &r, const bk_cluster *cl, uint64_t ncl, int maxspan, const unsigned long long *lb, BpBufs &b, hipStream_t st)
+{
+  uint32_t *depth = b.depth.as<uint32_t>(2 * ncl + 2);
+  if (ncl) hipLaunchKernelGGL(k_bp_depth, dim3(cdiv(ncl, 4)), dim3(256), 0, st, r, cl, (uint32_t) ncl, maxspan, b.voted.get<uint32_t>(), lb, depth);
+  return depth;
+}
 uint32_t *bp_depth_partial(const RecView &r0, const bk_cluster *cl, uint64_t ncl, int maxspan, BpBufs &b, hipStream_t st)
 {
-  const RecView r = sampled(r0, b, st);
-  uint32_t *depth = b.depth.as<uint32_t>(2 * ncl + 2);
-  if (ncl) hipLaunchKernelGGL(k_bp_depth, dim3(cdiv(ncl, 4)), dim3(256), 0, st, r, cl, (uint32_t) ncl, maxspan, b.voted.get<uint32_t>(), depth);
-  return depth;
+  return bp_depth_phase(sampled(r0, b, st), cl, ncl, maxspan, nullptr, b, st);
 }
 
 void base_depth_at(const RecView &r0, const int32_t *tid, const uint32_t *pos, uint64_t n, int maxspan, DevBuf &samp, hipStream_t st, uint32_t *depth)
@@ -766,7 +1033,7 @@
 
 void bp_finish(bk_cluster *cl, uint64_t ncl, const uint32_t *depth, BpBufs &b, hipStream_t st)
 {
-  if (ncl) hipLaunchKernelGGL(k_bp_finish, dim3(cdiv(ncl, 256)), dim3(256), 0, st, cl, (uint32_t) ncl, b.voted.get<uint32_t>(), depth);
+  if (ncl) hipLaunchKernelGGL(k_bp_finish, dim3(cdiv(ncl, 256)), dim3(256), 0, st, cl, (uint32_t) ncl, b.voted.get<uint32_t>(), depth, (uint32_t *) nullptr);
 }
 
 __global__ __launch_bounds__(256) void k_count_valid(const bk_cluster *__restrict__ cl, uint32_t ncl, unsigned long long *__restrict__ out)
@@ -787,14 +1054,24 @@
   return h;
 }
 
-void split_breakpoints(const RecView &r, const bk_split *sp, uint64_t nsp, bk_cluster *cl, uint64_t ncl, double w, int maxspan, const int32_t *hdr_id, BpBufs &b,
-                       hipStream_t st)
+void split_breakpoints(const RecView &r0, const bk_split *sp, const unsigned long long *tkey, uint64_t nsp, bk_cluster *cl, uint64_t ncl, double w, int maxspan,
+                       const int32_t *hdr_id, BpBufs &b, hipStream_t st)
 {
   if (ncl == 0) return;
-  const uint32_t *cov = bp_cov_partial(r, cl, ncl, w, maxspan, b, st);
-  bp_vote(sp, nsp, cl, ncl, w, maxspan, cov, hdr_id, b, st);
-  const uint32_t *depth = bp_depth_partial(r, cl, ncl, maxspan, b, st);
-  bp_finish(cl, ncl, depth, b, st);
+  const BpWork *work = bp_evidence(sp, tkey, nsp, cl, ncl, w, maxspan, b, st);
+  const RecView r = sampled(r0, b, st);
+  const uint32_t *cov = bp_cov_phase(r, cl, ncl, w, maxspan, work, true, b, st);
+  bp_vote_phase(sp, nsp, cl, ncl, w, cov, hdr_id, b, st);
+  const uint32_t *depth = bp_depth_phase(r, cl, ncl, maxspan, b.lb.get<unsigned long long>(), b, st);
+  hipLaunchKernelGGL(k_bp_finish, dim3(cdiv(ncl, 256)), dim3(256), 0, st, cl, (uint32_t) ncl, b.voted.get<uint32_t>(), depth, b.err.get<uint32_t>() + 1);
+}
+uint64_t bp_valid_count(uint64_t ncl, BpBufs &b, hipStream_t st)
+{
+  if (ncl == 0) return 0;
+  uint32_t h = 0;
+  HIP_CHECK(hipMemcpyAsync(&h, b.err.get<uint32_t>() + 1, 4, hipMemcpyDeviceToHost, st));
+  HIP_CHECK(hipStreamSynchronize(st));
+  return h;
 }
 
 void debug_region(const RecView &r, const bk_split *sp, uint64_t nsp, int32_t tid, uint32_t start, uint32_t end, int maxspan, unsigned long long depth_pos, bk_split *out,
```
